# sashashura/h2o-3

Hardware: AMD Instinct MI355X
Metric: gbm_trees_per_sec (higher is better)
Workload: dtype fp32; 1 GPU; model=GBM binomial 100Mx100 ntrees=500 max_depth=8, rows=100000000, cols=100, max_depth=8, histogram_type=QuantilesGlobal, nbins=255, global_batch=100000000, parallelism=dp1

## Files before the change

h2o3_amd/models/tree/devtree.py:

```python
from __future__ import annotations

import ctypes
import os

import numpy as np
import torch

from ...ops import tree_ops
from ...ops.tree_ops import _ptr, _stream
from ...parallel import cloud
from ...parallel import collectives as coll
from ...utils import graphs
from .engine import _TreeBuf

RS = 16
(GAIN, FEAT, T, OPT, L0, L1, R0, R1, T0, T1, OK, NL, NAW, ST, CT, VAL) = range(16)
MAX_DEPTH = 11
_cv, _ci, _cll, _cd, _cf = ctypes.c_void_p, ctypes.c_int, ctypes.c_longlong, ctypes.c_double, ctypes.c_float


def _libs():
    from ...ops import _native
    lh = tree_ops._lib()
    ls = _native.get_lib("tree_split")
    if not getattr(lh, "_typed_dt", False):
        lh.h2o_dt_items.argtypes = [_ci, _cv, _ci, _ci, _ci, _ci, _ci, _cv, _cv, _cv, _cv]
        lh.h2o_dt_offsets.argtypes = [_cv, _cv, _cv, _cv, _ci, _cv, _cv, _cv, _cv]
        lh.h2o_dt_sibling.argtypes = [_cv, _cv, _cv, _ci, _ci, _ci, _ci, _ci, _ci, _cv, _cv, _cv, _cv, _cv]
        lh.h2o_dt_leaf_vals.argtypes = [_cv, _cv, _ci, _ci, _cv, _cd, _cv, _cv]
        lh.h2o_dt_root.argtypes = [_cv, _cll, _cv]
        lh.h2o_part_flags_dev.argtypes = [_cv, _ci, _cll, _cll, _cv, _cv, _cv, _ci, _cv, _cv, _ci, _cv, _cv, _cv, _cv]
        lh.h2o_part_compact_dev.argtypes = [_cv, _cv, _cv, _ci, _cv, _cv, _cv, _cv, _cv, _cv, _cv, _cv]
        lh.h2o_leaf_pos_dev.argtypes = [_cv, _cv, _ci, _ci, _cv, _cv, _cv]
        lh.h2o_leaf_scatter_dev.argtypes = [_cv, _cv, _ci, _cv, _cv, _cv, _cv]
        lh.h2o_hist_bm.argtypes = [_cv, _ci, _cv, _cv, _cv, _cv, _ci, _ci, _ci, _ci, _cf, _cf, _cv, _ci, _ci, _cv,
                                   _ci, _cll, _ci, _cv, _cv, _cv, _cv]
        lh.h2o_gbm_grad.argtypes = [_cv, _cv, _cv, _ci, _cll, _cv, _cv, _cv]
        lh.h2o_iota_i32.argtypes = [_cv, _cll, _cv]
        lh.h2o_dt_colmask.argtypes = [_ci, _cv, _cv, _cv, _cv, _cv, _ci, _ci, _cv, _cv]
        lh.h2o_dt_items2.argtypes = [_ci, _cv, _ci, _ci, _ci, _ci, _ci, _cv, _cv, _cv, _cv, _cv]
        lh.h2o_leaf_flag_sums_dev.argtypes = [_cv, _cv, _cv, _ci, _cv, _cv, _ci, _ci, _cv, _cv, _cv]
        lh.h2o_leaf_gather_lds.argtypes = [_ci, _ci]
        lh.h2o_leaf_gather_items.argtypes = [_cll, _ci]
        lh.h2o_leaf_gather_dev.argtypes = [_cv, _ci, _ci, _ci, _cv, _cv, _cv, _cv, _cll, _ci, _ci, _cv, _cv, _cv, _cv,
                                           _cv, _cv]
        lh._typed_dt = True
    if not getattr(ls, "_typed_dt", False):
        ls.h2o_split_find_b.argtypes = [_cv, _ci, _ci, _ci, _cv, _cv, _cv] + [_cd] * 5 + [_ci, _cv, _cv, _ci, _cv]
        ls.h2o_split_select2.argtypes = [_cv, _cv, _ci, _ci, _ci, _ci, _cd, _ci, _cv, _cv, _cv, _cv]
        ls._typed_dt = True
    return lh, ls


def _ck(rc, what):
    if rc != 0:
        raise RuntimeError(f"{what} failed: error {rc}")


def supported(drv) -> str | None:
    if os.environ.get("H2O3_DEV_TREE", "1") != "1":
        return "disabled (H2O3_DEV_TREE=0)"
    bd, gp, p = drv.bd, drv.gp, drv.est._parms
    if drv.dev.type != "cuda":
        return "no GPU"
    if drv.K != 1 or drv.dist.family not in ("bernoulli", "gaussian") or drv.dist.link not in ("logit", "identity"):
        return "distribution"
    if drv.mono_on or drv.noise_bw != 0 or gp.interaction_sets:
        return "constraints / prediction noise"
    if not drv._base_unit:
        return "row weights other than 0/1"
    if any(bd.is_cat) or bd.code_bytes != 1 or bd.Bs > 256 or bd.Bs % 4 or bd.Fp % 16:
        return "categorical features / wide codes"
    if getattr(bd, "hist_type", "auto") in ("uniformadaptive", "random", "roundrobin"):
        return "adaptive histogram type"
    if gp.max_depth > MAX_DEPTH or gp.max_depth < 1:
        return "max_depth"
    if (gp.mtries or -1) > 0:
        return "mtries"
    if gp.max_leaves:
        return "max_leaves"
    if tree_ops.bm_groups(bd.F, bd.Fp, bd.Bs, True) is None:
        return "histogram layout"
    if drv.offset is not None or getattr(drv.dist, "huber_delta", None) is not None:
        return "offset"
    if not drv.grower.pos_payload_ok():
        return "payload path"
    return None


def gather_rows(n):
    ev = tree_ops.env("H2O3_LEAF_GATHER_R")
    return int(ev) if ev else 8192


class LeafGather:

    def __init__(self, lh, N, D, dev, R=None):
        self.lh, self.N, self.D = lh, int(N), int(D)
        self.nh = (1 << (D + 1)) - 1
        self.R = int(R) if R else gather_rows(N)
        self.scap = 1 << D
        nb = -(-self.N // self.R)
        self.segs = torch.zeros(self.scap * 4, dtype=torch.int32, device=dev)
        self.items = torch.zeros(2 * lh.h2o_leaf_gather_items(self.N, self.scap), dtype=torch.int32, device=dev)
        self.nseg = torch.zeros(2, dtype=torch.int32, device=dev)
        self.T = torch.zeros((nb + 1) * self.scap, dtype=torch.int32, device=dev)

    def run(self, rec, ridx, vals, dbuf, flags=None, slot_wb=None):
        last = 0 if slot_wb is None else 1
        _ck(self.lh.h2o_leaf_gather_dev(_ptr(rec), self.nh, self.D, last, _ptr(slot_wb), _ptr(ridx), _ptr(flags),
                                        _ptr(vals), self.N, self.R, self.scap, _ptr(self.segs), _ptr(self.items),
                                        _ptr(self.nseg), _ptr(self.T), _ptr(dbuf), _stream()), "leaf_gather_dev")


class DevTreeGBM:

    def __init__(self, drv):
        self.drv = drv
        bd, gp = drv.bd, drv.gp
        self.bd, self.gp = bd, gp
        self.lh, self.ls = _libs()
        g = drv.grower
        self.W, self.rank = g.W, g.rank
        self.F, self.Fl, self.Fpad, self.f0 = bd.F, g.Fl, g.Fpad, g.f0
        self.N = N = bd.nrows_local
        self.D = D = int(gp.max_depth)
        self.nh = (1 << (D + 1)) - 1
        self.Bs = Bs = bd.Bs
        self.C = C = 2
        self.bern = drv.dist.family == "bernoulli"
        self.maxabs = float(drv.est._parms.get("max_abs_leafnode_pred", 1.79e308))
        dev = drv.dev
        self.dev = dev
        self.pack = tree_ops.env("H2O3_HIST_PACK", "1") == "1"
        n_fg, G = tree_ops.bm_groups(bd.F, bd.Fp, Bs, self.pack)
        self.n_fg, self.G = n_fg, G
        self.chunk_r = tree_ops.hist_chunk(N, n_fg)
        self.chunk_c = tree_ops.hist_chunk((N + 1) // 2, n_fg)
        if self.pack and max(self.chunk_r, self.chunk_c) >= (1 << 23):
            raise RuntimeError("devtree: histogram chunk too large for the packed path")
        self.chunk_p = tree_ops._part_chunk(N)
        self.chunk_l = 65536
        self.vmax = [1.0, 1.0]
        self._scales()
        n_lvl_max = 1 << (D - 1) if D >= 1 else 1
        self.cap_r = 1 + N // self.chunk_r + 1
        self.cap_c = n_lvl_max + ((N + 1) // 2) // self.chunk_c + 2
        self.cap_p = (1 << D) + N // self.chunk_p + 1
        self.cap_l = self.nh + N // self.chunk_l + 1
        cap_h = max(self.cap_r, self.cap_c)
        i32, f64 = torch.int32, torch.float64
        self.rec = torch.zeros(self.nh * RS, dtype=f64, device=dev)
        self.sums = torch.zeros(self.nh * 2, dtype=f64, device=dev)
        self.vals = torch.zeros(self.nh, dtype=torch.float32, device=dev)
        self.lr_t = torch.zeros(1, dtype=torch.float32, device=dev)
        self.ridx = [g.ridx, g.ridx2]
        self.pos = [torch.empty(N, dtype=torch.float32, device=dev) for _ in range(2)]
        self.dbuf = torch.zeros(N, dtype=torch.float32, device=dev)
        lvl = self.Fl * n_lvl_max * Bs * C
        self.Hbuf = [torch.zeros(lvl, dtype=f64, device=dev) for _ in range(2)]
        self.wyybuf = [torch.zeros(n_lvl_max, dtype=f64, device=dev) for _ in range(2)]
        npar_max = max(1, n_lvl_max // 2)
        self.Hb = torch.zeros(bd.F * npar_max * Bs * C + npar_max, dtype=f64, device=dev)
        self.Hroot = torch.zeros(bd.F * Bs * C + 1, dtype=f64, device=dev)
        self.hwork = torch.zeros(cap_h * 4, dtype=i32, device=dev)
        self.pwork = torch.zeros(self.cap_p * 4, dtype=i32, device=dev)
        self.fbase = torch.zeros(self.cap_p, dtype=i32, device=dev)
        self.lwork = torch.zeros(self.cap_l * 4, dtype=i32, device=dev)
        self.counts = torch.zeros(2, dtype=i32, device=dev)
        self.cnt = torch.zeros(self.cap_p, dtype=i32, device=dev)
        self.loff = torch.zeros(self.cap_p, dtype=i32, device=dev)
        self.roff = torch.zeros(self.cap_p, dtype=i32, device=dev)
        self.flags = torch.zeros(N // 64 + self.cap_p + 1, dtype=torch.int64, device=dev)
        self.part = tree_ops.bm_part(cap_h, n_fg, Bs, G, self.pack, dev)
        self.split_out = torch.zeros(n_lvl_max * max(self.Fl, 1) * 4, dtype=f64, device=dev)
        self.mask = torch.zeros(n_lvl_max * Bs, dtype=torch.uint8, device=dev)
        self.feat_i = torch.zeros(n_lvl_max, dtype=i32, device=dev)
        self.okm = torch.ones((n_lvl_max, max(self.Fl, 1)), dtype=torch.uint8, device=dev)
        if self.f0 + self.Fl > self.F:
            self.okm[:, max(0, self.F - self.f0):] = 0
        self._okm_col = None
        self.mono = torch.zeros(max(self.Fl, 1), dtype=torch.float32, device=dev)
        if bd.codes_col is not None:
            self.pcodes, self.prs, self.pfs = bd.codes_col, 1, bd.nrows_local
        else:
            self.pcodes, self.prs, self.pfs = bd.codes, bd.Fp, 1
        self.cutmat = g._cut_matrix()
        self.sampled = not drv._unit_weights
        self.wbuf = torch.ones(N, dtype=torch.float32, device=dev) if self.sampled else None
        self.colsamp = gp.col_sample_rate < 1.0 or gp.col_sample_rate_change_per_level != 1.0
        if self.colsamp:
            self.cs_elig = torch.zeros(max(self.F, 1), dtype=torch.int64, device=dev)
            self.cs_m = torch.zeros(1, dtype=torch.int32, device=dev)
            self.cs_k = torch.zeros(max(D, 1), dtype=torch.int32, device=dev)
            self.cs_seed = torch.zeros(max(D, 1), dtype=torch.int64, device=dev)
        self.gather = os.environ.get("H2O3_LEAF_GATHER", "1") != "0" and N > 0
        self.last_level = self.gather and os.environ.get("H2O3_DEV_LAST_LEVEL", "1") != "0"
        self.lg = LeafGather(self.lh, N, D, dev) if self.gather else None
        self.slot_wb = torch.zeros(n_lvl_max, dtype=i32, device=dev)
        self.graph = None
        self._hv = [None, None]
        self._k = 0

    def _scales(self):
        vm = self.vmax
        self.s_r = [tree_ops.fixed_point_scale(m, self.chunk_r) for m in vm]
        self.s_c = [tree_ops.fixed_point_scale(m, self.chunk_c) for m in vm]
        self.bq_r = self.bq_c = -1
        if self.pack:
            self.s_r[1], self.bq_r = tree_ops._pack_scale(vm[1], self.chunk_r)
            self.s_c[1], self.bq_c = tree_ops._pack_scale(vm[1], self.chunk_c)

    def set_tree_cols(self, mask):
        key = None if mask is None else mask.tobytes()
        if key == self._okm_col:
            return
        self._okm_col = key
        m = np.ones(self.Fpad, dtype=np.uint8)
        if mask is not None:
            m[:self.F] = np.asarray(mask, dtype=np.uint8)
        m[self.F:] = 0
        row = self._upload([m[self.f0:self.f0 + self.Fl].copy()])[0]
        self.okm.copy_(row.view(1, -1).expand_as(self.okm))

    def _upload(self, arrays):
        offs, n = [], 0
        for a in arrays:
            offs.append(n)
            n += (a.nbytes + 7) & ~7
        n = max(n, 8)
        if getattr(self, "_stg", None) is None or self._stg[0].numel() < n:
            self._stg = [torch.empty(n, dtype=torch.uint8, pin_memory=True) for _ in range(2)]
            self._stg_ev = [None, None]
            self._dstg = torch.empty(n, dtype=torch.uint8, device=self.dev)
            self._stg_i = 0
        i = self._stg_i
        self._stg_i ^= 1
        if self._stg_ev[i] is not None:
            self._stg_ev[i].synchronize()
        buf = self._stg[i].numpy()
        for a, o in zip(arrays, offs):
            buf[o:o + a.nbytes] = np.ascontiguousarray(a).view(np.uint8).reshape(-1)
        self._dstg[:n].copy_(self._stg[i][:n], non_blocking=True)
        ev = torch.cuda.Event()
        ev.record()
        self._stg_ev[i] = ev
        out = []
        for a, o in zip(arrays, offs):
            out.append(self._dstg[o:o + a.nbytes].view(torch.from_numpy(a[:0]).dtype)
                       if a.nbytes else torch.empty(0, dtype=torch.from_numpy(a[:0]).dtype, device=self.dev))
        return out

    def _rec_lvl(self, d):
        off = (1 << d) - 1
        return self.rec[off * RS:]

    def _hist(self, d, cur):
        lh = self.lh
        bd, Bs, C = self.bd, self.Bs, self.C
        n = 1 << d
        H = self.Hbuf[d % 2][:self.Fl * n * Bs * C]
        wyy = self.wyybuf[d % 2][:n]
        s = _stream()
        if d == 0:
            _ck(lh.h2o_dt_items(0, _ptr(self.rec), 1, self.D, 0, self.chunk_r, self.cap_r, _ptr(self.hwork), None,
                                _ptr(self.counts), s), "dt_items(root)")
            nh = bd.F * Bs * C
            buf = self.Hroot
            buf.zero_()
            _ck(lh.h2o_hist_bm(_ptr(bd.codes), bd.Fp, _ptr(self.ridx[cur]), _ptr(self.pos[cur]), None,
                               _ptr(self.hwork), self.cap_r, bd.F, 0, Bs, self.s_r[0], self.s_r[1], _ptr(buf), 1, 0,
                               _ptr(buf[nh:]), 1, self.bq_r, self.G, None, _ptr(self.counts), _ptr(self.part), s),
                "hist_bm(root)")
            Hl, wl = buf[:nh].view(bd.F, 1, Bs, C), buf[nh:]
            if self.W > 1:
                Hl, wl = self.drv.grower._rs_hist_wyy(Hl, wl)
            H.view(self.Fl, 1, Bs, C).copy_(Hl)
            wyy.copy_(wl)
            return H, wyy
        npar = n // 2
        rp = self._rec_lvl(d - 1)
        _ck(lh.h2o_dt_items(1, _ptr(rp), npar, self.D, 0, self.chunk_c, self.cap_c, _ptr(self.hwork), None,
                            _ptr(self.counts), s), "dt_items(child)")
        nhb = bd.F * npar * Bs * C
        buf = self.Hb[:nhb + npar]
        buf.zero_()
        _ck(lh.h2o_hist_bm(_ptr(bd.codes), bd.Fp, _ptr(self.ridx[cur]), _ptr(self.pos[cur]), None, _ptr(self.hwork),
                           self.cap_c, bd.F, 0, Bs, self.s_c[0], self.s_c[1], _ptr(buf), npar, 0, _ptr(buf[nhb:]), 1,
                           self.bq_c, self.G, None, _ptr(self.counts), _ptr(self.part), s), "hist_bm(child)")
        Hb, wb = buf[:nhb].view(bd.F, npar, Bs, C), buf[nhb:]
        if self.W > 1:
            Hb, wb = self.drv.grower._rs_hist_wyy(Hb, wb)
            Hb, wb = Hb.contiguous(), wb.contiguous()
        Hp = self.Hbuf[(d - 1) % 2]
        wp = self.wyybuf[(d - 1) % 2]
        _ck(lh.h2o_dt_sibling(_ptr(Hb), _ptr(Hp), _ptr(rp), npar, self.Fl, Bs * C, C, 0b1, 0, _ptr(H), _ptr(wb),
                              _ptr(wp), _ptr(wyy), _stream()), "dt_sibling")
        return H, wyy

    def _merge(self, recl, n):
        W, Bs = self.W, self.Bs
        rows = recl[:n * RS].view(n, RS)
        rb = 13 * 8
        buf = torch.cat([rows[:, :13].contiguous().view(torch.uint8).view(n, rb), self.mask[:n * Bs].view(n, Bs)], 1)
        g = coll.all_gather_dim0(buf).view(W, n, rb + Bs)
        gains = g[:, :, :8].contiguous().view(torch.float64).view(W, n)
        best = torch.argmax(gains, 0)
        win = g[best, torch.arange(n, device=buf.device)]
        pk = win[:, :rb].contiguous().view(torch.float64).view(n, 13)
        rows[:, :13].copy_(pk)
        self.mask[:n * Bs].view(n, Bs).copy_(win[:, rb:])
        okf = pk[:, OK] > 0
        self.feat_i[:n].copy_(torch.where(okf, pk[:, FEAT], torch.zeros_like(pk[:, FEAT])).to(torch.int32))

    def _level(self, d, cur):
        lh, ls, gp = self.lh, self.ls, self.gp
        n = 1 << d
        Bs = self.Bs
        H, wyy = self._hist(d, cur)
        recl = self._rec_lvl(d)
        s = _stream()
        if self.colsamp:
            rp = self._rec_lvl(d - 1) if d > 0 else None
            _ck(lh.h2o_dt_colmask(d, _ptr(rp), _ptr(self.cs_elig), _ptr(self.cs_m), _ptr(self.cs_k),
                                  _ptr(self.cs_seed), self.f0, self.Fl, _ptr(self.okm), s), "dt_colmask")
        _ck(ls.h2o_split_find_b(_ptr(H), self.Fl, n, Bs, _ptr(wyy), _ptr(self.okm), _ptr(self.mono),
                                float(gp.min_rows), float(gp.min_split_improvement), float(gp.reg_lambda),
                                float(gp.reg_alpha), float(gp.gamma), 0, _ptr(self.split_out), None, 0, s),
            "split_find")
        _ck(ls.h2o_split_select2(_ptr(self.split_out), _ptr(H), self.Fl, n, Bs, self.f0, 2.0 * float(gp.min_rows), RS,
                                 _ptr(recl), _ptr(self.mask), _ptr(self.feat_i), s), "split_select2")
        if self.W > 1:
            self._merge(recl, n)
        s = _stream()
        skip = self.last_level and d == self.D - 1
        _ck(lh.h2o_dt_items2(0, _ptr(recl), n, self.D, 0, self.chunk_p, self.cap_p, _ptr(self.pwork),
                             _ptr(self.fbase), _ptr(self.slot_wb) if skip else None, _ptr(self.counts), s),
            "dt_items(part)")
        _ck(lh.h2o_part_flags_dev(_ptr(self.pcodes), 1, self.prs, self.pfs, _ptr(self.ridx[cur]), _ptr(self.pwork),
                                  _ptr(self.fbase), self.cap_p, _ptr(self.feat_i), _ptr(self.mask), Bs,
                                  _ptr(self.flags), _ptr(self.cnt), _ptr(self.counts), s), "part_flags_dev")
        _ck(lh.h2o_dt_offsets(_ptr(self.cnt), _ptr(self.pwork), _ptr(self.counts), _ptr(recl), n,
                              _ptr(self._rec_lvl(d + 1)), _ptr(self.loff), _ptr(self.roff), s), "dt_offsets")
        if skip:
            _ck(lh.h2o_leaf_flag_sums_dev(_ptr(self.pos[cur]), _ptr(self.pwork), _ptr(self.fbase), self.cap_p,
                                          _ptr(self.flags), _ptr(recl), self.D, 1 if self.bern else 0,
                                          _ptr(self.sums), _ptr(self.counts), s), "leaf_flag_sums_dev")
            return cur
        nxt = cur ^ 1
        _ck(lh.h2o_part_compact_dev(_ptr(self.ridx[cur]), _ptr(self.pwork), _ptr(self.fbase), self.cap_p,
                                    _ptr(self.flags), _ptr(self.loff), _ptr(self.roff), _ptr(self.ridx[nxt]),
                                    _ptr(self.pos[cur]), _ptr(self.pos[nxt]), _ptr(self.counts), s),
            "part_compact_dev")
        return nxt

    def _sequence(self):
        lh, drv = self.lh, self.drv
        s = _stream()
        y = drv.yb if self.bern else torch.nan_to_num(drv.yf)
        if not hasattr(self, "_y"):
            self._y = y.contiguous().to(torch.float32)
        f = drv._f[:, 0]
        _ck(lh.h2o_gbm_grad(_ptr(self._y), _ptr(f), _ptr(self.wbuf) if self.sampled else None,
                            1 if self.bern else 0, self.N, _ptr(self.pos[0]), _ptr(self.dbuf), s), "gbm_grad")
        _ck(lh.h2o_iota_i32(_ptr(self.ridx[0]), self.N, s), "iota")
        self.rec.zero_()
        self.sums.zero_()
        _ck(lh.h2o_dt_root(_ptr(self.rec), self.N, _stream()), "dt_root")
        cur = 0
        for d in range(self.D):
            cur = self._level(d, cur)
        s = _stream()
        _ck(lh.h2o_dt_items(3 if self.last_level else 2, _ptr(self.rec), self.nh, self.D, 0, self.chunk_l, self.cap_l,
                            _ptr(self.lwork), None, _ptr(self.counts), s), "dt_items(leaf)")
        _ck(lh.h2o_leaf_pos_dev(_ptr(self.pos[cur]), _ptr(self.lwork), self.cap_l, 1 if self.bern else 0,
                                _ptr(self.sums), _ptr(self.counts), s), "leaf_pos_dev")
        if self.W > 1:
            coll.allreduce_(self.sums)
        s = _stream()
        _ck(lh.h2o_dt_leaf_vals(_ptr(self.rec), _ptr(self.sums), self.nh, self.D, _ptr(self.lr_t), self.maxabs,
                                _ptr(self.vals), s), "dt_leaf_vals")
        if self.gather:
            self.lg.run(self.rec, self.ridx[cur], self.vals, self.dbuf, self.flags if self.last_level else None,
                        self.slot_wb if self.last_level else None)
        else:
            _ck(lh.h2o_leaf_scatter_dev(_ptr(self.ridx[cur]), _ptr(self.lwork), self.cap_l, _ptr(self.vals),
                                        _ptr(self.dbuf), _ptr(self.counts), s), "leaf_scatter_dev")
        self.cur = cur

    def set_col_sampling(self, tree_mask):
        if not self.colsamp:
            return
        g, gp, F, D = self.drv.grower, self.gp, self.F, self.D
        base = np.ones(F, dtype=bool) if tree_mask is None else np.asarray(tree_mask, dtype=bool)
        elig = np.nonzero(base)[0]
        m = int(elig.size)
        ks = np.zeros(D, dtype=np.int32)
        seeds = np.zeros(D, dtype=np.int64)
        for d in range(D):
            rate = gp.col_sample_rate * (gp.col_sample_rate_change_per_level ** d)
            k = max(1, int(np.floor(rate * m + 0.5))) if rate < 1.0 else m
            if k >= m:
                ks[d] = m
            else:
                ks[d] = k
                seeds[d] = int(g.rng.randint(0, 2 ** 31 - 1))
        e = np.zeros(max(F, 1), dtype=np.int64)
        e[:m] = elig
        de, dm, dk, dsd = self._upload([e, np.array([m], dtype=np.int32), ks, seeds])
        self.cs_elig.copy_(de)
        self.cs_m.copy_(dm)
        self.cs_k.copy_(dk)
        self.cs_seed.copy_(dsd)

    def run(self, lr, pending, w=None):
        if not pending:
            self.dbuf.zero_()
        if self.sampled:
            self.wbuf.copy_(w)
        self.lr_t.fill_(float(lr))
        if not self.bern:
            f = self.drv._f[:, 0]
            z = (torch.nan_to_num(self.drv.yf) - (f + self.dbuf))
            self.vmax = [1.0, float(z.abs().max())]
            self._scales()
            self._sequence()
        elif self.W == 1 and os.environ.get("H2O3_DEV_TREE_GRAPH", "1") == "1":
            if self.graph is None:
                self._sequence()
                torch.cuda.synchronize()
                g = torch.cuda.CUDAGraph()
                with graphs.capture(g):
                    self._sequence()
                self.graph = g
            else:
                self.graph.replay()
        else:
            self._sequence()
        return self._copy_out()

    def _copy_out(self):
        k = self._k
        self._k ^= 1
        h = self._hv[k]
        if h is None:
            h = self._hv[k] = torch.empty(self.nh * RS, dtype=torch.float64, pin_memory=True)
        h.copy_(self.rec, non_blocking=True)
        ev = torch.cuda.Event()
        ev.record()
        return h, ev

    def decode(self, rec_h, criterion="se"):
        D, nh = self.D, self.nh
        R = np.asarray(rec_h, dtype=np.float64).reshape(nh, RS)
        lv = np.floor(np.log2(np.arange(nh) + 1)).astype(np.int64)
        ok = R[:, OK] > 0
        exists = np.zeros(nh, dtype=bool)
        exists[0] = True
        for d in range(1, D + 1):
            a, b = (1 << d) - 1, (1 << (d + 1)) - 1
            par = (np.arange(a, b) - 1) >> 1
            exists[a:b] = exists[par] & ok[par]
        split = exists & ok & (lv < D)
        ids = np.nonzero(exists)[0]
        bfs = np.full(nh, -1, dtype=np.int64)
        bfs[ids] = np.arange(ids.size)
        n = ids.size
        tb = _TreeBuf(cap=max(n, 1))
        tb.n = n
        par = np.maximum((ids - 1) >> 1, 0)
        is_left = (ids % 2) == 1
        w_own = R[ids, T0]
        w_par = np.where(is_left, R[par, L0], R[par, R0])
        tb.weight[:n] = np.where(lv[ids] < D, w_own, w_par)
        tb.depth[:n] = lv[ids]
        sp = split[ids]
        hs = ids[sp]
        bi = bfs[hs]
        f = R[hs, FEAT].astype(np.int64)
        t = R[hs, T].astype(np.int64)
        opt = R[hs, OPT].astype(np.int64)
        tb.feat[bi] = f
        tb.left[bi] = bfs[2 * hs + 1]
        tb.right[bi] = bfs[2 * hs + 2]
        tb.gain[bi] = R[hs, GAIN]
        tb.split_code[bi] = t
        cm = self.cutmat
        tb.thr[bi] = np.where(opt == 2, np.inf, cm[f, np.minimum(t, cm.shape[1] - 1)])
        na = opt == 1
        if criterion != "xgb":
            free = (R[hs, NAW] == 0) & (opt != 2)
            na = np.where(free, R[hs, L0] > R[hs, R0], na)
        tb.na_left[bi] = na
        lf = ~sp
        tb.value[bfs[ids[lf]]] = R[ids[lf], VAL]
        return tb.to_tree()
```

h2o3_amd/ops/csrc/tree_hist.hip:

```cpp
#include "common.h"
#include <stdlib.h>
#include <algorithm>

template <int MODE> struct Chan { static constexpr int C = MODE == 2 ? 1 : 2; };

template <typename CodeT, int MODE, bool HAS_VB, bool POSV, bool PACK = false>
__global__ __launch_bounds__(512) void hist_build_kernel(
    const CodeT* __restrict__ codes, int Fp, const int* __restrict__ ridx,
    const float* __restrict__ va, const float* __restrict__ vb,
    const int4* __restrict__ work, int F, int Bs, int FGL, float s0, float s1,
    double* __restrict__ hist, int n_slots, double* __restrict__ wyy_out, const uint8_t* __restrict__ need,
    long long bq = 0) {
  constexpr int C = Chan<MODE>::C;
  constexpr int CL = PACK ? 1 : C;
  const int RPW = 64 / FGL;
  extern __shared__ __attribute__((aligned(16))) unsigned long long ldsq[];
  const int4 wk = work[blockIdx.x];
  if (need != nullptr && need[(size_t)wk.x * gridDim.y + blockIdx.y] == 0) return;
  const int fg0 = blockIdx.y * FGL;
  const int nf = min(FGL, F - fg0);
  const int stride_f = Bs * CL;
  const int total = FGL * stride_f;
  for (int i = threadIdx.x; i < total; i += blockDim.x) ldsq[i] = 0ull;
  __syncthreads();
  const unsigned long long pk_off = (1ull << 40) + (unsigned long long)bq;

  const int lane = threadIdx.x & 63;
  const int fl = lane % FGL;
  const int rs = lane / FGL;
  const bool lane_ok = rs < RPW;
  const bool fok = fl < nf && lane_ok;
  const int nwaves = blockDim.x >> 6;
  const int wv = threadIdx.x >> 6;
  unsigned long long* hbase = ldsq + fl * stride_f;
  const bool do_wyy = (MODE == 0) && wyy_out != nullptr && blockIdx.y == 0 && fl == 0 && lane_ok;
  double wyy = 0.0;
  const int pend = wk.y + wk.z;
  const int step = nwaves * RPW;
  constexpr int U = 8;
  const int fcl = min(fl, max(nf - 1, 0));
  const CodeT* cbase = codes + fg0 + fcl;
  for (int p0 = wk.y + wv * RPW + (lane_ok ? rs : 0); p0 < pend; p0 += U * step) {
    int rr[U];
    float c0[U], c1[U], yv[U];
    int code[U];
#pragma unroll
    for (int u = 0; u < U; ++u) rr[u] = ridx[min(p0 + u * step, pend - 1)];
#pragma unroll
    for (int u = 0; u < U; ++u) {
      const int r = rr[u];
      const int vi = POSV ? min(p0 + u * step, pend - 1) : r;
      if (MODE == 0) {
        const float y = va[vi];
        const float w = HAS_VB ? vb[vi] : 1.f;
        c0[u] = w; c1[u] = w * y;
        yv[u] = y;
      } else if (MODE == 1) {
        c0[u] = va[vi]; c1[u] = vb[vi];
      } else {
        c0[u] = HAS_VB ? vb[vi] : 1.f; c1[u] = 0.f;
      }
      code[u] = (int)cbase[(size_t)r * Fp];
    }
#pragma unroll
    for (int u = 0; u < U; ++u) {
      const bool inr = p0 + u * step < pend;
      if (MODE == 0 && do_wyy && inr) wyy += (double)c1[u] * (double)yv[u];
      if (PACK) {
        if (fok && inr && c0[u] != 0.f)
          __hip_atomic_fetch_add(hbase + code[u], pk_off + (unsigned long long)__float2ll_rn(c1[u] * s1),
                                 __ATOMIC_RELAXED, __HIP_MEMORY_SCOPE_WORKGROUP);
        continue;
      }
      const bool ok = fok && inr && (c0[u] != 0.f || c1[u] != 0.f);
      if (ok) {
        unsigned long long* h = hbase + code[u] * C;
        __hip_atomic_fetch_add(h, (unsigned long long)__float2ll_rn(c0[u] * s0), __ATOMIC_RELAXED,
                               __HIP_MEMORY_SCOPE_WORKGROUP);
        if (C > 1)
          __hip_atomic_fetch_add(h + 1, (unsigned long long)__float2ll_rn(c1[u] * s1), __ATOMIC_RELAXED,
                                 __HIP_MEMORY_SCOPE_WORKGROUP);
      }
    }
  }
  __syncthreads();
  if (MODE == 0 && wyy_out != nullptr && blockIdx.y == 0) {
    wyy = wave_sum(wyy);
    if (lane == 0) gbl_add(wyy_out + wk.x, wyy);
  }
  const double inv0 = 1.0 / (double)s0, inv1 = 1.0 / (double)s1;
  if (PACK) {
    const int tot = nf * Bs;
    for (int i = threadIdx.x; i < tot; i += blockDim.x) {
      const unsigned long long v = ldsq[i];
      if (v != 0) {
        const int j = i / Bs, b = i - (i / Bs) * Bs;
        const long long cnt = (long long)(v >> 40);
        const long long low = (long long)(v & ((1ull << 40) - 1));
        double* o = hist + ((size_t)(fg0 + j) * n_slots + wk.x) * (Bs * 2) + 2 * b;
        gbl_add(o, (double)cnt);
        gbl_add(o + 1, (double)(low - cnt * bq) * inv1);
      }
    }
    return;
  }
  const int tot_real = nf * stride_f;
  for (int i = threadIdx.x; i < tot_real; i += blockDim.x) {
    const long long q = (long long)ldsq[i];
    if (q != 0) {
      const int j = i / stride_f;
      const int rem = i - j * stride_f;
      const double v = (double)q * ((C == 1 || (rem & 1) == 0) ? inv0 : inv1);
      gbl_add(hist + ((size_t)(fg0 + j) * n_slots + wk.x) * stride_f + rem, v);
    }
  }
}

template <int LW> struct CodeW { using T = unsigned int; };
template <> struct CodeW<2> { using T = uint2; };
__device__ __forceinline__ unsigned int code_at(unsigned int w, int hi, int sh) { return (w >> sh) & 0xffu; }
__device__ __forceinline__ unsigned int code_at(uint2 w, int hi, int sh) { return ((hi ? w.y : w.x) >> sh) & 0xffu; }

template <int MODE, bool HAS_VB, bool POSV, bool PACK, bool PIPE = true, int LW = 1>
__global__ __launch_bounds__(1024) void hist_quad_kernel(
    const uint8_t* __restrict__ codes, int Fp, const int* __restrict__ ridx,
    const float* __restrict__ va, const float* __restrict__ vb,
    const int4* __restrict__ work, int n_work, int n_fg, int fgw, int F, int foff, int Bs, float s0, float s1,
    double* __restrict__ hist, int n_slots, double* __restrict__ wyy_out, long long bq,
    const uint8_t* __restrict__ need, const int* __restrict__ n_work_dev) {
  using CT = typename CodeW<LW>::T;
  constexpr int C = Chan<MODE>::C;
  constexpr int CL = PACK ? 1 : C;
  constexpr int NK = 4 * LW;
  constexpr int U = 4;
  extern __shared__ __attribute__((aligned(16))) unsigned long long ldsq[];
  const int nwg = n_work_dev != nullptr ? n_work_dev[1] * n_fg : n_work * n_fg;
  if ((int)blockIdx.x >= nwg) return;
  const int lb = xcd_remap(blockIdx.x, nwg);
  const int fgi = lb % n_fg;
  const int4 wk = work[lb / n_fg];
  if (need != nullptr && need[(size_t)wk.x * n_fg + fgi] == 0) return;
  const int fg0 = foff + fgi * fgw;
  const int nf = min(fgw, F - fg0);
  const int LPR = fgw / NK;
  const int RPW = 64 / LPR;
  const int stride_f = Bs * CL + CL;
  const int total = fgw * stride_f;
  for (int i = threadIdx.x; i < total; i += blockDim.x) ldsq[i] = 0ull;
  __syncthreads();
  const int lane = threadIdx.x & 63;
  const int q = lane % LPR;
  const int rs = lane / LPR;
  const bool lane_ok = rs < RPW;
  const int wv = threadIdx.x >> 6;
  const int nwaves = blockDim.x >> 6;
  const bool do_wyy = (MODE == 0) && wyy_out != nullptr && fgi == 0 && q == 0 && lane_ok;
  double wyy = 0.0;
  const int pend = wk.y + wk.z;
  const int step = nwaves * RPW;
  const uint8_t* cbase = codes + fg0 + NK * q;
  unsigned long long* hb[NK];
  bool fk[NK];
#pragma unroll
  for (int k = 0; k < NK; ++k) {
    hb[k] = ldsq + (NK * q + k) * stride_f;
    fk[k] = lane_ok && NK * q + k < nf;
  }
  const int p_first = wk.y + wv * RPW + (lane_ok ? rs : 0);
  int rA[U], rB[U];
  CT cwA[U];
  float xaA[U], xbA[U];
  auto load_r = [&](int p, int (&r)[U]) {
#pragma unroll
    for (int u = 0; u < U; ++u) r[u] = ridx[min(p + u * step, pend - 1)];
  };
  auto load_v = [&](int p, const int (&r)[U], CT (&cw)[U], float (&xa)[U], float (&xb)[U]) {
#pragma unroll
    for (int u = 0; u < U; ++u) {
      const int vi = POSV ? min(p + u * step, pend - 1) : r[u];
      xa[u] = (MODE == 2) ? 0.f : va[vi];
      xb[u] = (HAS_VB || MODE == 1) ? vb[vi] : 1.f;
      cw[u] = *reinterpret_cast<const CT*>(cbase + (size_t)r[u] * Fp);
    }
  };
  if (PIPE) {
    load_r(p_first, rA);
    load_v(p_first, rA, cwA, xaA, xbA);
    load_r(p_first + U * step, rB);
  }
  for (int p0 = p_first; p0 < pend; p0 += U * step) {
    CT cw[U];
    float c0[U], c1[U], yv[U], xa[U], xb[U];
    if (PIPE) {
#pragma unroll
      for (int u = 0; u < U; ++u) { cw[u] = cwA[u]; xa[u] = xaA[u]; xb[u] = xbA[u]; }
      load_v(p0 + U * step, rB, cwA, xaA, xbA);
      load_r(p0 + 2 * U * step, rB);
    } else {
      int rr[U];
      load_r(p0, rr);
      load_v(p0, rr, cw, xa, xb);
    }
#pragma unroll
    for (int u = 0; u < U; ++u) {
      if (MODE == 0) {
        const float y = xa[u];
        const float w = HAS_VB ? xb[u] : (y == y ? 1.f : 0.f);
        c0[u] = w; c1[u] = w != 0.f ? w * y : 0.f; yv[u] = w != 0.f ? y : 0.f;
      } else if (MODE == 1) {
        c0[u] = xa[u]; c1[u] = xb[u]; yv[u] = 0.f;
      } else {
        c0[u] = xb[u]; c1[u] = 0.f; yv[u] = 0.f;
      }
    }
#pragma unroll
    for (int u = 0; u < U; ++u) {
      const bool inr = p0 + u * step < pend;
      if (MODE == 0 && do_wyy && inr) wyy += (double)c1[u] * (double)yv[u];
      if (!inr || (c0[u] == 0.f && c1[u] == 0.f)) continue;
      if (PACK) {
        const unsigned long long a = (1ull << 40) + (unsigned long long)(__float2ll_rn(yv[u] * s1) + bq);
#pragma unroll
        for (int k = 0; k < NK; ++k) {
          if (!fk[k]) continue;
          __hip_atomic_fetch_add(hb[k] + code_at(cw[u], k >> 2, 8 * (k & 3)), a, __ATOMIC_RELAXED,
                                 __HIP_MEMORY_SCOPE_WORKGROUP);
        }
        continue;
      }
      const unsigned long long a0 = (unsigned long long)__float2ll_rn(c0[u] * s0);
      const unsigned long long a1 = (unsigned long long)__float2ll_rn(c1[u] * s1);
#pragma unroll
      for (int k = 0; k < NK; ++k) {
        if (!fk[k]) continue;
        unsigned long long* h = hb[k] + code_at(cw[u], k >> 2, 8 * (k & 3)) * CL;
        __hip_atomic_fetch_add(h, a0, __ATOMIC_RELAXED, __HIP_MEMORY_SCOPE_WORKGROUP);
        if (C > 1) __hip_atomic_fetch_add(h + 1, a1, __ATOMIC_RELAXED, __HIP_MEMORY_SCOPE_WORKGROUP);
      }
    }
  }
  __syncthreads();
  if (MODE == 0 && wyy_out != nullptr && fgi == 0) {
    wyy = wave_sum(wyy);
    if (lane == 0) gbl_add(wyy_out + wk.x, wyy);
  }
  const double inv0 = 1.0 / (double)s0, inv1 = 1.0 / (double)s1;
  const int per_f = Bs * C;
  if (PACK) {
    const int tot = nf * Bs;
    for (int i = threadIdx.x; i < tot; i += blockDim.x) {
      const int j = i / Bs;
      const int b = i - j * Bs;
      const unsigned long long v = ldsq[j * stride_f + b];
      if (v != 0) {
        const long long cnt = (long long)(v >> 40);
        const long long low = (long long)(v & ((1ull << 40) - 1));
        double* o = hist + ((size_t)(fg0 + j) * n_slots + wk.x) * per_f + 2 * b;
        gbl_add(o, (double)cnt);
        gbl_add(o + 1, (double)(low - cnt * bq) * inv1);
      }
    }
    return;
  }
  const int tot_real = nf * per_f;
  for (int i = threadIdx.x; i < tot_real; i += blockDim.x) {
    const int j = i / per_f;
    const int rem = i - j * per_f;
    const long long v = (long long)ldsq[j * stride_f + rem];
    if (v != 0) {
      const double d = (double)v * ((C == 1 || (rem & 1) == 0) ? inv0 : inv1);
      gbl_add(hist + ((size_t)(fg0 + j) * n_slots + wk.x) * per_f + rem, d);
    }
  }
}

struct QuadArgs {
  dim3 grid; int threads; size_t lds; hipStream_t s;
  const uint8_t* cc; int Fp; const int* ridx; const float* va; const float* vb; const int4* wk;
  int n_work, n_fg, fgw, F, foff, Bs; float s0, s1; double* hist; int n_slots; double* wyy; long long bq;
  const uint8_t* need; const int* n_work_dev; unsigned long long* part = nullptr;
};

template <int M, bool V, bool PV, bool PK, bool PIPE = true, int LW = 1>
static void lq(const QuadArgs& a) {
  hipLaunchKernelGGL((hist_quad_kernel<M, V, PV, PK, PIPE, LW>), a.grid, dim3(a.threads), a.lds, a.s, a.cc, a.Fp,
                     a.ridx, a.va, a.vb, a.wk, a.n_work, a.n_fg, a.fgw, a.F, a.foff, a.Bs, a.s0, a.s1, a.hist,
                     a.n_slots, a.wyy, a.bq, a.need, a.n_work_dev);
}

static int env_int(const char* k, int d) {
  const char* v = getenv(k);
  return v ? atoi(v) : d;
}

template <int M, bool V, bool PV, bool PK>
static void lq_var(int lw, const QuadArgs& a) {
  static const int pipe = env_int("H2O3_HIST_PIPE", 1);
  if (!pipe) lq<M, V, PV, PK, false>(a);
  else if (lw == 2) lq<M, V, PV, PK, true, 2>(a);
  else lq<M, V, PV, PK>(a);
}

template <int M, bool V>
static void lq_pv(int posv, int pack, int lw, const QuadArgs& a) {
  if (pack) { if (posv) lq_var<M, V, true, true>(lw, a); else lq_var<M, V, false, true>(lw, a); }
  else { if (posv) lq_var<M, V, true, false>(lw, a); else lq_var<M, V, false, false>(lw, a); }
}

extern "C" int h2o_hist_quad4(const void* codes, int Fp, const int* ridx, const float* va, const float* vb,
                              const int* work, int n_work, int F, int foff, int Bs, float s0, float s1,
                              double* hist, int n_slots, int mode, int threads, double* wyy, int posv,
                              long long pack_bq, int fgw, const uint8_t* need, const int* n_work_dev,
                              hipStream_t s);
extern "C" int h2o_hist_quad3(const void* codes, int Fp, const int* ridx, const float* va, const float* vb,
                              const int* work, int n_work, int F, int foff, int Bs, float s0, float s1,
                              double* hist, int n_slots, int mode, int threads, double* wyy, int posv,
                              long long pack_bq, int fgw, const uint8_t* need, hipStream_t s) {
  return h2o_hist_quad4(codes, Fp, ridx, va, vb, work, n_work, F, foff, Bs, s0, s1, hist, n_slots, mode, threads,
                        wyy, posv, pack_bq, fgw, need, nullptr, s);
}

extern "C" int h2o_hist_quad4(const void* codes, int Fp, const int* ridx, const float* va, const float* vb,
                              const int* work, int n_work, int F, int foff, int Bs, float s0, float s1,
                              double* hist, int n_slots, int mode, int threads, double* wyy, int posv,
                              long long pack_bq, int fgw, const uint8_t* need, const int* n_work_dev,
                              hipStream_t s) {
  if (n_work <= 0 || foff >= F) return 0;
  if (Fp % 4 != 0 || foff % 4 != 0 || Bs > 256 || mode < 0 || mode > 2) return -1;
  if (fgw < 4 || fgw > 64 || fgw % 4 != 0) return -2;
  const bool pack = pack_bq >= 0 && mode == 0;
  const int n_fg = (F - foff + fgw - 1) / fgw;
  if (foff + n_fg * fgw > Fp) return -3;
  static const int lw_env = env_int("H2O3_HIST_LW", 1);
  const int lw = (lw_env == 2 && fgw % 8 == 0 && foff % 8 == 0 && Fp % 8 == 0) ? 2 : 1;
  const int C = mode == 2 ? 1 : 2;
  const int CL = pack ? 1 : C;
  QuadArgs a;
  a.grid = dim3(n_work * n_fg); a.threads = threads;
  a.lds = (size_t)fgw * (Bs * CL + CL) * sizeof(unsigned long long); a.s = s;
  if (a.lds > 160 * 1024) return -4;
  a.cc = (const uint8_t*)codes; a.Fp = Fp; a.ridx = ridx; a.va = va; a.vb = vb; a.wk = (const int4*)work;
  a.n_work = n_work; a.n_fg = n_fg; a.fgw = fgw; a.F = F; a.foff = foff; a.Bs = Bs; a.s0 = s0; a.s1 = s1;
  a.hist = hist; a.n_slots = n_slots; a.wyy = wyy; a.bq = pack_bq; a.need = need; a.n_work_dev = n_work_dev;
  switch (mode) {
    case 0: if (vb) lq_pv<0, true>(posv, pack, lw, a); else lq_pv<0, false>(posv, pack, lw, a); break;
    case 1: lq_pv<1, true>(posv, 0, lw, a); break;
    default: if (vb) lq_pv<2, true>(posv, 0, lw, a); else lq_pv<2, false>(posv, 0, lw, a); break;
  }
  return (int)hipGetLastError();
}

__device__ __forceinline__ unsigned long long fx_signed(float v, float s) {
  const double d = __fma_rn((double)v, (double)s, 6755399441055744.0);
  return (unsigned long long)(__double_as_longlong(d) - 0x4338000000000000LL);
}

template <int G, int CL, int MODE, bool HAS_VB, bool POSV, bool PACK, int LW = 2>
__global__ __launch_bounds__(1024) void hist_bm_kernel(
    const uint8_t* __restrict__ codes, int Fp, const int* __restrict__ ridx,
    const float* __restrict__ va, const float* __restrict__ vb,
    const int4* __restrict__ work, int n_work, int n_fg, int F, int foff, int Bs, float s0, float s1,
    double* __restrict__ hist, int n_slots, double* __restrict__ wyy_out, long long bq,
    const uint8_t* __restrict__ need, const int* __restrict__ n_work_dev, unsigned long long* __restrict__ part,
    int dbg) {
  constexpr int C = Chan<MODE>::C;
  constexpr int NK = 4 * LW;
  constexpr int LPR = G / NK;
  constexpr int RPW = 64 / LPR;
  constexpr int PITCH = G * CL;
  constexpr int U = 4;
  constexpr int PD = 2;
  using CT = typename CodeW<LW>::T;
  static_assert(CL == 1 || C == 2, "two LDS channels need a two-channel mode");
  static_assert(LPR >= 1, "group narrower than one lane's codes");
  extern __shared__ __attribute__((aligned(16))) unsigned long long ldsq[];
  const int nwg = n_work_dev != nullptr ? n_work_dev[1] * n_fg : n_work * n_fg;
  if ((int)blockIdx.x >= nwg) return;
  const int lb = xcd_remap(blockIdx.x, nwg);
  const int fgi = lb % n_fg;
  int4 wk = work[lb / n_fg];
  wk.x = __builtin_amdgcn_readfirstlane(wk.x);
  wk.y = __builtin_amdgcn_readfirstlane(wk.y);
  wk.z = __builtin_amdgcn_readfirstlane(wk.z);
  if (need != nullptr && need[(size_t)wk.x * n_fg + fgi] == 0) return;
  const int fg0 = foff + fgi * G;
  const int nf = min(G, F - fg0);
  {
    const int n2 = Bs * PITCH / 2;
    ulonglong2* z = reinterpret_cast<ulonglong2*>(ldsq);
    for (int i = threadIdx.x; i < n2; i += blockDim.x) z[i] = make_ulonglong2(0ull, 0ull);
  }
  __syncthreads();
  const int lane = threadIdx.x & 63;
  const int q = lane % LPR;
  const int rs = lane / LPR;
  const int wv = threadIdx.x >> 6;
  const int nwaves = __builtin_amdgcn_readfirstlane((int)(blockDim.x >> 6));
  unsigned sh[NK], sb[NK];
#pragma unroll
  for (int k = 0; k < NK; ++k) {
    const int kk = (k & ~3) | ((k + rs) & 3);
    sh[k] = 8u * kk;
    sb[k] = (unsigned)((kk * LPR + q) * 8);
  }
  const bool blk_wyy = MODE == 0 && wyy_out != nullptr && fgi == 0;
  double wyyd = 0.0;
  const int pend = wk.y + wk.z;
  const int step = nwaves * RPW;
  const uint8_t* cbase = codes + fg0 + NK * q;
  const int p_first = wk.y + wv * RPW + rs;
  const unsigned long long pk_off = (1ull << 40) + (unsigned long long)bq;
  const __amdgpu_buffer_rsrc_t rr = __builtin_amdgcn_make_buffer_rsrc((void*)ridx, (short)0, pend * 4, 0x00020000);
  const __amdgpu_buffer_rsrc_t ra = __builtin_amdgcn_make_buffer_rsrc((void*)va, (short)0, POSV ? pend * 4 : 0,
                                                                      0x00020000);
  const __amdgpu_buffer_rsrc_t rb = __builtin_amdgcn_make_buffer_rsrc((void*)vb, (short)0,
                                                                      (POSV && vb) ? pend * 4 : 0, 0x00020000);
  int R[PD][U];
  CT CW[PD][U];
  float XA[PD][U], XB[PD][U];
  auto load_r = [&](int p, int (&r)[U]) {
#pragma unroll
    for (int u = 0; u < U; ++u) r[u] = __builtin_amdgcn_raw_buffer_load_b32(rr, p * 4, u * step * 4, 0);
  };
  auto load_v = [&](int p, const int (&r)[U], CT (&cw)[U], float (&xa)[U], float (&xb)[U]) {
#pragma unroll
    for (int u = 0; u < U; ++u) {
      if (POSV) {
        xa[u] = (MODE == 2) ? 0.f : __int_as_float(__builtin_amdgcn_raw_buffer_load_b32(ra, p * 4, u * step * 4, 0));
        xb[u] = (HAS_VB || MODE == 1) ? __int_as_float(__builtin_amdgcn_raw_buffer_load_b32(rb, p * 4, u * step * 4, 0))
                                      : 1.f;
      } else {
        xa[u] = (MODE == 2) ? 0.f : va[r[u]];
        xb[u] = (HAS_VB || MODE == 1) ? vb[r[u]] : 1.f;
      }
      cw[u] = *reinterpret_cast<const CT*>(cbase + (size_t)(unsigned)r[u] * (unsigned)Fp);
    }
  };
  const int IT = U * step;
#pragma unroll
  for (int d = 0; d < PD; ++d) load_r(p_first + d * IT, R[d]);
#pragma unroll
  for (int d = 0; d < PD; ++d) {
    load_v(p_first + d * IT, R[d], CW[d], XA[d], XB[d]);
    load_r(p_first + (PD + d) * IT, R[d]);
  }
  for (int p0r = p_first; p0r < pend; p0r += PD * IT) {
#pragma unroll
    for (int d = 0; d < PD; ++d) {
      const int p0 = p0r + d * IT;
#pragma unroll
      for (int u = 0; u < U; ++u) {
        const bool inr = p0 + u * step < pend;
        float c0, c1, yv = 0.f;
        if (MODE == 0) {
          const float y = XA[d][u];
          const float w = HAS_VB ? XB[d][u] : (y == y ? 1.f : 0.f);
          c0 = w;
          c1 = w != 0.f ? w * y : 0.f;
          yv = w != 0.f ? y : 0.f;
          if (blk_wyy && inr) wyyd += (double)c1 * (double)yv;
        } else if (MODE == 1) {
          c0 = XA[d][u]; c1 = XB[d][u];
        } else {
          c0 = XB[d][u]; c1 = 0.f;
        }
        if (!inr || (c0 == 0.f && c1 == 0.f) || (dbg & 2)) continue;
        unsigned long long a0, a1 = 0ull;
        if (PACK) {
          a0 = fx_signed(yv, s1) + pk_off;
        } else {
          a0 = fx_signed(c0, s0);
          if (CL == 2) a1 = fx_signed(c1, s1);
        }
#pragma unroll
        for (int k = 0; k < NK; ++k) {
          unsigned word;
          if constexpr (LW == 2) word = (k & 4) ? CW[d][u].y : CW[d][u].x;
          else word = CW[d][u];
          const unsigned code = __builtin_amdgcn_ubfe(word, sh[k] & 31u, 8);
          unsigned long long* h = reinterpret_cast<unsigned long long*>(
              reinterpret_cast<char*>(ldsq) + code * (unsigned)(PITCH * 8) + sb[k]);
          __hip_atomic_fetch_add(h, a0, __ATOMIC_RELAXED, __HIP_MEMORY_SCOPE_WORKGROUP);
          if (CL == 2) __hip_atomic_fetch_add(h + G, a1, __ATOMIC_RELAXED, __HIP_MEMORY_SCOPE_WORKGROUP);
        }
      }
      load_v(p0 + PD * IT, R[d], CW[d], XA[d], XB[d]);
      load_r(p0 + 2 * PD * IT, R[d]);
    }
  }
  __syncthreads();
  if (blk_wyy) {
    double v = q == 0 ? wyyd : 0.0;
    v = wave_sum(v);
    if (lane == 0) gbl_add(wyy_out + wk.x, v);
  }
  if (part != nullptr) {
    if (dbg & 1) return;
    const int n2 = Bs * PITCH / 2;
    const ulonglong2* src = reinterpret_cast<const ulonglong2*>(ldsq);
    ulonglong2* dst = reinterpret_cast<ulonglong2*>(part + ((size_t)(lb / n_fg) * n_fg + fgi) * (size_t)(Bs * PITCH));
    for (int i2 = threadIdx.x; i2 < n2; i2 += blockDim.x) dst[i2] = src[i2];
    return;
  }
  const double inv0 = 1.0 / (double)s0, inv1 = 1.0 / (double)s1;
  const int si = lane & 15, bi = lane >> 4;
  constexpr int NSG = G / 16;
  const int nbq = (dbg & 1) ? 0 : (Bs + 3) >> 2;
  for (int e = wv; e < nbq * NSG; e += nwaves) {
    const int b = (e / NSG) * 4 + bi;
    const int slot = (e % NSG) * 16 + si;
    const int fl = NK * (slot % LPR) + slot / LPR;
    if (b >= Bs || fl >= nf) continue;
    double* o = hist + ((size_t)(fg0 + fl) * n_slots + wk.x) * (size_t)(Bs * C) + (size_t)b * C;
    const unsigned long long v = ldsq[b * PITCH + slot];
    if (PACK) {
      if (v != 0ull) {
        const long long cnt = (long long)(v >> 40);
        const long long low = (long long)(v & ((1ull << 40) - 1));
        if (dbg & 4) {
          unsigned long long* ou = reinterpret_cast<unsigned long long*>(o);
          __hip_atomic_fetch_add(ou, (unsigned long long)cnt, __ATOMIC_RELAXED, __HIP_MEMORY_SCOPE_AGENT);
          __hip_atomic_fetch_add(ou + 1, (unsigned long long)(low - cnt * bq), __ATOMIC_RELAXED,
                                 __HIP_MEMORY_SCOPE_AGENT);
        } else {
          gbl_add(o, (double)cnt);
          gbl_add(o + 1, (double)(low - cnt * bq) * inv1);
        }
      }
    } else {
      if (v != 0ull) gbl_add(o, (double)(long long)v * inv0);
      if (CL == 2) {
        const unsigned long long v1 = ldsq[b * PITCH + G + slot];
        if (v1 != 0ull) gbl_add(o + 1, (double)(long long)v1 * inv1);
      }
    }
  }
}

static int g_bm_dbg = 0;
extern "C" void h2o_hist_bm_set_debug(int flags) { g_bm_dbg = flags; }

template <int G, int CL, int M, bool V, bool PV, bool PK, int LW>
static int lbm_u(const QuadArgs& a) {
  auto kern = hist_bm_kernel<G, CL, M, V, PV, PK, LW>;
  static bool attr = false;
  if (!attr) {
    hipError_t e = hipFuncSetAttribute((const void*)kern, hipFuncAttributeMaxDynamicSharedMemorySize, 160 * 1024);
    if (e != hipSuccess) return (int)e;
    attr = true;
  }
  hipLaunchKernelGGL(kern, a.grid, dim3(a.threads), a.lds, a.s, a.cc, a.Fp, a.ridx, a.va, a.vb, a.wk, a.n_work,
                     a.n_fg, a.F, a.foff, a.Bs, a.s0, a.s1, a.hist, a.n_slots, a.wyy, a.bq, a.need, a.n_work_dev,
                     a.part, g_bm_dbg);
  return (int)hipGetLastError();
}

template <int G, int CL, int M, bool V, bool PV, bool PK>
static int lbm(const QuadArgs& a) {
  static const int lw = env_int("H2O3_HIST_BM_LW", 2);
  return (lw == 1 || G == 16) ? lbm_u<G, CL, M, V, PV, PK, 1>(a) : lbm_u<G, CL, M, V, PV, PK, 2>(a);
}

template <int G, int CL, int M, bool PK>
static int lbm_v(bool vb, bool posv, const QuadArgs& a) {
  if (M == 1) return posv ? lbm<G, CL, M, true, true, PK>(a) : lbm<G, CL, M, true, false, PK>(a);
  if (vb) return posv ? lbm<G, CL, M, true, true, PK>(a) : lbm<G, CL, M, true, false, PK>(a);
  return posv ? lbm<G, CL, M, false, true, PK>(a) : lbm<G, CL, M, false, false, PK>(a);
}

template <int G>
static int lbm_g(int mode, bool pack, bool vb, bool posv, const QuadArgs& a) {
  if (pack) return lbm_v<G, 1, 0, true>(vb, posv, a);
  if (mode == 2) return lbm_v<G, 1, 2, false>(vb, posv, a);
  if constexpr (G <= 32) {
    if (mode == 0) return lbm_v<G, 2, 0, false>(vb, posv, a);
    return lbm_v<G, 2, 1, false>(vb, posv, a);
  }
  return (int)hipErrorInvalidValue;
}

#define BM_RED 32
__global__ __launch_bounds__(256) void hist_bm_reduce_kernel(
    const unsigned long long* __restrict__ part, const int4* __restrict__ work, int n_work,
    const int* __restrict__ n_work_dev, int n_fg, int F, int foff, int G, int CL, int lpr, int nk, int Bs, int C,
    int pack, long long bq, float s0, float s1, const uint8_t* __restrict__ need, double* __restrict__ hist,
    int n_slots) {
  const int nw = n_work_dev != nullptr ? n_work_dev[1] : n_work;
  const int i0 = blockIdx.z * BM_RED;
  if (i0 >= nw) return;
  const int i1 = min(nw, i0 + BM_RED);
  const int g = blockIdx.y;
  const int PITCH = G * CL;
  const int nbt = (Bs + 15) / 16;
  const int b = (blockIdx.x % nbt) * 16 + (threadIdx.x >> 4);
  if (b >= Bs) return;
  const int sl = (blockIdx.x / nbt) * 16 + (threadIdx.x & 15);
  const int ch = sl / G, slot = sl - ch * G;
  const int fg0 = foff + g * G;
  const int fl = nk * (slot % lpr) + slot / lpr;
  const bool live = fl < min(G, F - fg0);
  const double inv0 = 1.0 / (double)s0, inv1 = 1.0 / (double)s1;
  const size_t E = (size_t)Bs * PITCH;
  const size_t eoff = (size_t)b * PITCH + sl;
  long long a0 = 0, a1 = 0;
  int cur = -1;
  auto flush = [&]() {
    if (cur < 0 || !live || (a0 == 0 && a1 == 0)) return;
    double* o = hist + ((size_t)(fg0 + fl) * n_slots + cur) * (size_t)(Bs * C) + (size_t)b * C;
    if (pack) {
      gbl_add(o, (double)a0);
      gbl_add(o + 1, (double)a1 * inv1);
    } else {
      gbl_add(o + ch, (double)a0 * (ch == 0 ? inv0 : inv1));
    }
  };
  for (int i = i0; i < i1; ++i) {
    const int s = work[i].x;
    if (need != nullptr && need[(size_t)s * n_fg + g] == 0) continue;
    if (s != cur) {
      flush();
      cur = s; a0 = 0; a1 = 0;
    }
    const unsigned long long v = part[((size_t)i * n_fg + g) * E + eoff];
    if (pack) {
      const long long cnt = (long long)(v >> 40);
      a0 += cnt;
      a1 += (long long)(v & ((1ull << 40) - 1)) - cnt * bq;
    } else {
      a0 += (long long)v;
    }
  }
  flush();
}

extern "C" int h2o_hist_bm(const void* codes, int Fp, const int* ridx, const float* va, const float* vb,
                           const int* work, int n_work, int F, int foff, int Bs, float s0, float s1,
                           double* hist, int n_slots, int mode, double* wyy, int posv, long long pack_bq, int G,
                           const uint8_t* need, const int* n_work_dev, unsigned long long* part, hipStream_t s) {
  if (n_work <= 0 || foff >= F) return 0;
  if (Fp % 4 != 0 || foff % 4 != 0 || Bs > 256 || Bs % 4 != 0 || mode < 0 || mode > 2) return -1;
  const bool pack = pack_bq >= 0 && mode == 0;
  const int CL = (pack || mode == 2) ? 1 : 2;
  if (!(G == 16 || G == 32 || G == 64) || (CL == 2 && G == 64)) return -2;
  const int n_fg = (F - foff + G - 1) / G;
  if (foff + n_fg * G > Fp) return -3;
  QuadArgs a;
  a.grid = dim3(n_work * n_fg); a.threads = 1024;
  a.lds = (size_t)Bs * G * CL * sizeof(unsigned long long); a.s = s;
  if (a.lds > 160 * 1024) return -4;
  a.cc = (const uint8_t*)codes; a.Fp = Fp; a.ridx = ridx; a.va = va; a.vb = vb; a.wk = (const int4*)work;
  a.n_work = n_work; a.n_fg = n_fg; a.fgw = G; a.F = F; a.foff = foff; a.Bs = Bs; a.s0 = s0; a.s1 = s1;
  a.hist = hist; a.n_slots = n_slots; a.wyy = wyy; a.bq = pack_bq; a.need = need; a.n_work_dev = n_work_dev;
  a.part = part;
  const int rc = G == 64 ? lbm_g<64>(mode, pack, vb != nullptr, posv != 0, a)
               : G == 32 ? lbm_g<32>(mode, pack, vb != nullptr, posv != 0, a)
                         : lbm_g<16>(mode, pack, vb != nullptr, posv != 0, a);
  if (rc != 0 || part == nullptr || (g_bm_dbg & 1)) return rc;
  static const int lw_env = env_int("H2O3_HIST_BM_LW", 2);
  const int lw = (lw_env == 1 || G == 16) ? 1 : 2;
  const int nk = 4 * lw, lpr = G / nk;
  const int C = mode == 2 ? 1 : 2;
  dim3 rg(((Bs + 15) / 16) * (G * CL / 16), n_fg, (n_work + BM_RED - 1) / BM_RED);
  hipLaunchKernelGGL(hist_bm_reduce_kernel, rg, dim3(256), 0, s, part, (const int4*)work, n_work, n_work_dev, n_fg,
                     F, foff, G, CL, lpr, nk, Bs, C, pack ? 1 : 0, pack_bq, s0, s1, need, hist, n_slots);
  return (int)hipGetLastError();
}

template <typename CodeT>
static int launch_hist(const void* codes, int Fp, const int* ridx, const float* va, const float* vb,
                       const int4* work, int n_work, int F, int FG, int Bs, float s0, float s1, double* hist,
                       int n_slots, int mode, int threads, double* wyy, int posv, const uint8_t* need,
                       hipStream_t s, long long pack_bq = -1) {
  const int n_fg = (F + FG - 1) / FG;
  dim3 grid(n_work, n_fg);
  const int C = mode == 2 ? 1 : 2;
  const CodeT* cc = (const CodeT*)codes;
  if (pack_bq >= 0 && mode == 0) {
    const size_t lds = (size_t)FG * Bs * sizeof(unsigned long long);
    if (lds > 160 * 1024) return (int)hipErrorInvalidValue;
#define H2O_PK(V, PV)                                                                                        \
  {                                                                                                          \
    auto kern = hist_build_kernel<CodeT, 0, V, PV, true>;                                                    \
    if (hipFuncSetAttribute((const void*)kern, hipFuncAttributeMaxDynamicSharedMemorySize, (int)lds) !=      \
        hipSuccess)                                                                                          \
      return (int)hipErrorInvalidValue;                                                                      \
    hipLaunchKernelGGL(kern, grid, dim3(threads), lds, s, cc, Fp, ridx, va, vb, work, F, Bs, FG, s0, s1,     \
                       hist, n_slots, wyy, need, pack_bq);                                                   \
  }
    if (vb) {
      if (posv) H2O_PK(true, true) else H2O_PK(true, false)
    } else {
      if (posv) H2O_PK(false, true) else H2O_PK(false, false)
    }
#undef H2O_PK
    return (int)hipGetLastError();
  }
  size_t lds = (size_t)FG * Bs * C * sizeof(unsigned long long);
  switch (mode) {
#define H2O_LH(M, V) if (posv) H2O_LH2(M, V, true); else H2O_LH2(M, V, false)
#define H2O_LH2(M, V, PV) hipLaunchKernelGGL((hist_build_kernel<CodeT, M, V, PV>), grid, dim3(threads), lds, s, cc, Fp, ridx, va, vb, work, F, Bs, FG, s0, s1, hist, n_slots, wyy, need)
    case 0: if (vb) H2O_LH(0, true); else H2O_LH(0, false); break;
    case 1: H2O_LH(1, true); break;
    default: if (vb) H2O_LH(2, true); else H2O_LH(2, false); break;
#undef H2O_LH
#undef H2O_LH2
  }
  return (int)hipGetLastError();
}

template <typename CodeT>
__device__ __forceinline__ void load_items(const CodeT* __restrict__ codes, long long rs, long long fs, int f,
                                           const int* __restrict__ ridx, int p0, int end, int (&r)[16],
                                           int (&c)[16]) {
  if (p0 + 16 <= end && (p0 & 3) == 0) {
    const int4* v = reinterpret_cast<const int4*>(ridx + p0);
#pragma unroll
    for (int q = 0; q < 4; ++q) {
      const int4 x = v[q];
      r[4 * q] = x.x; r[4 * q + 1] = x.y; r[4 * q + 2] = x.z; r[4 * q + 3] = x.w;
    }
  } else {
#pragma unroll
    for (int k = 0; k < 16; ++k) r[k] = ridx[min(p0 + k, end - 1)];
  }
#pragma unroll
  for (int k = 0; k < 16; ++k) c[k] = (int)codes[(size_t)r[k] * rs + (size_t)f * fs];
}

template <typename CodeT>
__global__ __launch_bounds__(256) void part_count_kernel(
    const CodeT* __restrict__ codes, long long rs, long long fs, const int* __restrict__ ridx,
    const int4* __restrict__ work, const int* __restrict__ feat, const uint8_t* __restrict__ masks,
    int Bs, int* __restrict__ cnt) {
  __shared__ uint8_t m[4096];
  __shared__ int red[4];
  const int4 wk = work[blockIdx.x];
  const int f = feat[wk.x];
  for (int i = threadIdx.x; i < Bs; i += blockDim.x) m[i] = masks[(size_t)wk.x * Bs + i];
  __syncthreads();
  const int end = wk.y + wk.z;
  int local = 0;
  for (int base = wk.y; base < end; base += 256 * 16) {
    const int p0 = base + threadIdx.x * 16;
    if (p0 >= end) continue;
    int r[16], c[16];
    load_items<CodeT>(codes, rs, fs, f, ridx, p0, end, r, c);
#pragma unroll
    for (int k = 0; k < 16; ++k) local += (p0 + k < end && m[c[k]]) ? 1 : 0;
  }
  for (int o = 32; o > 0; o >>= 1) local += __shfl_xor(local, o, 64);
  if (lane_id() == 0) red[wave_id()] = local;
  __syncthreads();
  if (threadIdx.x == 0) cnt[blockIdx.x] = red[0] + red[1] + red[2] + red[3];
}

template <typename CodeT>
__global__ __launch_bounds__(256) void part_scatter_kernel(
    const CodeT* __restrict__ codes, long long rs, long long fs, const int* __restrict__ ridx,
    const int4* __restrict__ work, const int* __restrict__ feat, const uint8_t* __restrict__ masks,
    int Bs, const int* __restrict__ loff, const int* __restrict__ roff, int* __restrict__ out,
    const float* __restrict__ pa, const float* __restrict__ pb, float* __restrict__ pa_out,
    float* __restrict__ pb_out) {
  __shared__ uint8_t m[4096];
  __shared__ int wsum[4];
  const int4 wk = work[blockIdx.x];
  const int f = feat[wk.x];
  for (int i = threadIdx.x; i < Bs; i += blockDim.x) m[i] = masks[(size_t)wk.x * Bs + i];
  __syncthreads();
  int lbase = loff[blockIdx.x], rbase = roff[blockIdx.x];
  const int end = wk.y + wk.z;
  const int lane = lane_id(), wv = wave_id();
  for (int base = wk.y; base < end; base += 256 * 16) {
    const int p0 = base + threadIdx.x * 16;
    int r[16], c[16];
    unsigned bits = 0;
    int nl = 0, nv = 0;
    if (p0 < end) {
      load_items<CodeT>(codes, rs, fs, f, ridx, p0, end, r, c);
#pragma unroll
      for (int k = 0; k < 16; ++k) {
        const bool v = p0 + k < end;
        const bool L = v && m[c[k]];
        bits |= (L ? 1u : 0u) << k;
        nl += L ? 1 : 0;
        nv += v ? 1 : 0;
      }
    }
    int incl = nl;
#pragma unroll
    for (int d = 1; d < 64; d <<= 1) {
      const int u = __shfl_up(incl, d, 64);
      if (lane >= d) incl += u;
    }
    if (lane == 63) wsum[wv] = incl;
    __syncthreads();
    int wpre = 0, tot = 0;
#pragma unroll
    for (int w = 0; w < 4; ++w) {
      const int s = wsum[w];
      wpre += (w < wv) ? s : 0;
      tot += s;
    }
    const int lpre = wpre + incl - nl;
    const int tile_first = base;
    const int pos_before = max(0, min(p0, end) - tile_first);
    int li = lbase + lpre;
    int ri = rbase + (pos_before - lpre);
    if (p0 < end) {
#pragma unroll
      for (int k = 0; k < 16; ++k) {
        if (p0 + k < end) {
          const int dst = ((bits >> k) & 1u) ? li++ : ri++;
          out[dst] = r[k];
          if (pa) { pa_out[dst] = pa[p0 + k]; pb_out[dst] = pb[p0 + k]; }
        }
      }
    }
    const int tile_n = min(256 * 16, end - base);
    lbase += tot;
    rbase += tile_n - tot;
    __syncthreads();
  }
}
template <typename CodeT>
__global__ __launch_bounds__(256) void part_flags_kernel(
    const CodeT* __restrict__ codes, long long rs, long long fs, const int* __restrict__ ridx,
    const int4* __restrict__ work, const int* __restrict__ fbase, const int* __restrict__ feat,
    const uint8_t* __restrict__ masks, int Bs, unsigned long long* __restrict__ flags, int* __restrict__ cnt,
    const int* __restrict__ nw_dev) {
  __shared__ uint8_t m[4096];
  __shared__ int red[4];
  if (nw_dev != nullptr && (int)blockIdx.x >= nw_dev[1]) return;
  const int4 wk = work[blockIdx.x];
  const int f = feat[wk.x];
  for (int i = threadIdx.x; i < Bs; i += blockDim.x) m[i] = masks[(size_t)wk.x * Bs + i];
  __syncthreads();
  const int lane = threadIdx.x & 63, wv = threadIdx.x >> 6;
  const int end = wk.y + wk.z;
  const int fb = fbase[blockIdx.x];
  int local = 0;
  constexpr int U = 8;
  for (int base = wk.y; base < end; base += 256 * U) {
    int r[U], c[U];
#pragma unroll
    for (int u = 0; u < U; ++u) r[u] = ridx[min(base + u * 256 + (int)threadIdx.x, end - 1)];
#pragma unroll
    for (int u = 0; u < U; ++u) c[u] = (int)codes[(size_t)r[u] * rs + (size_t)f * fs];
#pragma unroll
    for (int u = 0; u < U; ++u) {
      const int p = base + u * 256 + (int)threadIdx.x;
      const bool L = p < end && m[c[u]];
      const unsigned long long bal = __ballot(L);
      const int w0 = base + u * 256 + wv * 64;
      if (lane == 0 && w0 < end) flags[fb + (w0 - wk.y) / 64] = bal;
      local += L ? 1 : 0;
    }
  }
  local = (int)wave_sum((float)local);
  if (lane == 0) red[wv] = local;
  __syncthreads();
  if (threadIdx.x == 0) cnt[blockIdx.x] = red[0] + red[1] + red[2] + red[3];
}

template <int U>
__global__ __launch_bounds__(256) void part_compact_kernel(
    const int* __restrict__ ridx, const int4* __restrict__ work, const int* __restrict__ fbase,
    const unsigned long long* __restrict__ flags, const int* __restrict__ loff, const int* __restrict__ roff,
    int* __restrict__ out, const float* __restrict__ pa, float* __restrict__ pa_out, const int* __restrict__ nw_dev) {
  __shared__ int wl[U][4], wr_[U][4];
  if (nw_dev != nullptr && (int)blockIdx.x >= nw_dev[1]) return;
  const int4 wk = work[blockIdx.x];
  const int lane = threadIdx.x & 63, wv = threadIdx.x >> 6;
  const int end = wk.y + wk.z;
  const int fb = fbase[blockIdx.x];
  int lbase = loff[blockIdx.x], rbase = roff[blockIdx.x];
  const unsigned long long below = (lane == 0) ? 0ull : (~0ull >> (64 - lane));
  for (int base = wk.y; base < end; base += 256 * U) {
    int r[U];
    float a[U];
    unsigned long long bal[U], valid[U];
#pragma unroll
    for (int u = 0; u < U; ++u) {
      const int p = base + u * 256 + (int)threadIdx.x;
      const int pc = min(p, end - 1);
      r[u] = ridx[pc];
      a[u] = pa ? pa[pc] : 0.f;
      const int w0 = base + u * 256 + wv * 64;
      bal[u] = (w0 < end) ? flags[fb + (w0 - wk.y) / 64] : 0ull;
    }
#pragma unroll
    for (int u = 0; u < U; ++u) {
      valid[u] = __ballot(base + u * 256 + (int)threadIdx.x < end);
      const int nl_w = __popcll(bal[u] & valid[u]);
      if (lane == 0) { wl[u][wv] = nl_w; wr_[u][wv] = __popcll(valid[u]) - nl_w; }
    }
    __syncthreads();
    int lrun = 0, rrun = 0;
#pragma unroll
    for (int u = 0; u < U; ++u) {
      int lpre = lrun, rpre = rrun;
#pragma unroll
      for (int w = 0; w < 4; ++w) {
        lpre += (w < wv) ? wl[u][w] : 0;
        rpre += (w < wv) ? wr_[u][w] : 0;
        lrun += wl[u][w];
        rrun += wr_[u][w];
      }
      if ((valid[u] >> lane) & 1ull) {
        const bool L = (bal[u] >> lane) & 1ull;
        const int dst = L ? (lbase + lpre + __popcll(bal[u] & valid[u] & below))
                          : (rbase + rpre + __popcll(~bal[u] & valid[u] & below));
        out[dst] = r[u];
        if (pa) pa_out[dst] = a[u];
      }
    }
    lbase += lrun;
    rbase += rrun;
    __syncthreads();
  }
}


__global__ __launch_bounds__(256) void hist_sibling_kernel(const double* __restrict__ Hb,
                                                           const double* __restrict__ Hp,
                                                           const int* __restrict__ slots, int nb, int np, int nf,
                                                           int BsC, int C, int clamp_mask,
                                                           double* __restrict__ H, const double* __restrict__ wyy_b,
                                                           const double* __restrict__ wyy_p,
                                                           double* __restrict__ wyy_out,
                                                           const int* __restrict__ nb_dev) {
  const int j = blockIdx.x;
  if (nb_dev != nullptr && j >= nb_dev[0]) return;
  const int f = blockIdx.y;
  const int bs = slots[j], ds = slots[nb + j], ps = slots[2 * nb + j];
  const double* hb = Hb + ((size_t)f * nb + j) * BsC;
  const double* hp = Hp + ((size_t)f * np + ps) * BsC;
  double* ob = H + ((size_t)f * nf + bs) * BsC;
  double* od = H + ((size_t)f * nf + ds) * BsC;
  for (int i = threadIdx.x; i < BsC; i += blockDim.x) {
    const double b = hb[i];
    double d = hp[i] - b;
    if ((clamp_mask >> (i % C)) & 1) d = fmax(d, 0.0);
    ob[i] = b;
    od[i] = d;
  }
  if (wyy_b != nullptr && f == 0 && threadIdx.x == 0) {
    wyy_out[bs] = wyy_b[j];
    wyy_out[ds] = wyy_p[ps] - wyy_b[j];
  }
}

__global__ __launch_bounds__(1024) void part_offsets_kernel(const int* __restrict__ cnt,
                                                            const long long* __restrict__ meta, int nw, int n,
                                                            int* __restrict__ loff, int* __restrict__ roff,
                                                            long long* __restrict__ nleft, double* __restrict__ pk,
                                                            int stride, int col) {
  __shared__ long long carry;
  const long long* slot = meta;
  const long long* first = meta + nw;
  const long long* st = meta + 2 * (long long)nw;
  const long long* pos = meta + 3 * (long long)nw;
  for (int s = threadIdx.x; s < n; s += blockDim.x) nleft[s] = 0;
  if (threadIdx.x == 0) carry = 0;
  __syncthreads();
  __shared__ long long wtot[16];
  const int lane = threadIdx.x & 63, wv = threadIdx.x >> 6, nwv = blockDim.x >> 6;
  for (int base = 0; base < nw; base += blockDim.x) {
    const int i = base + threadIdx.x;
    const long long v = i < nw ? (long long)cnt[i] : 0;
    long long x = v;
#pragma unroll
    for (int o = 1; o < 64; o <<= 1) {
      const long long t = __shfl_up(x, o, 64);
      if (lane >= o) x += t;
    }
    if (lane == 63) wtot[wv] = x;
    __syncthreads();
    if (wv == 0) {
      long long w = lane < nwv ? wtot[lane] : 0;
#pragma unroll
      for (int o = 1; o < 16; o <<= 1) {
        const long long t = __shfl_up(w, o, 64);
        if (lane >= o) w += t;
      }
      if (lane < nwv) wtot[lane] = w;
    }
    __syncthreads();
    const long long before = (wv > 0 ? wtot[wv - 1] : 0) + carry;
    if (i < nw) loff[i] = (int)(before + x - v);
    __syncthreads();
    if (threadIdx.x == 0) carry += wtot[nwv - 1];
    __syncthreads();
  }
  __syncthreads();
  for (int i = threadIdx.x; i < nw; i += blockDim.x)
    if (i == nw - 1 || first[i + 1] != first[i])
      nleft[slot[i]] = (long long)loff[i] + cnt[i] - (long long)loff[first[i]];
  for (int i = threadIdx.x; i < nw; i += blockDim.x) roff[i] = loff[first[i]];
  __syncthreads();
  for (int i = threadIdx.x; i < nw; i += blockDim.x) {
    const long long lpre = (long long)loff[i] - (long long)roff[i];
    const long long s = slot[i];
    loff[i] = (int)(st[i] + lpre);
    roff[i] = (int)(st[i] + nleft[s] + pos[i] - lpre);
  }
  __syncthreads();
  if (pk != nullptr)
    for (int s = threadIdx.x; s < n; s += blockDim.x) pk[(size_t)s * stride + col] = (double)nleft[s];
}


__global__ __launch_bounds__(256) void leaf_pos_kernel(const float* __restrict__ zp, const int4* __restrict__ work,
                                                       int mode, double* __restrict__ out,
                                                       const int* __restrict__ nw_dev) {
  if (nw_dev != nullptr && (int)blockIdx.x >= nw_dev[1]) return;
  const int4 wk = work[blockIdx.x];
  double sa = 0.0, sb = 0.0;
  const int end = wk.y + wk.z;
  for (int p = wk.y + threadIdx.x; p < end; p += 256) {
    const float z = zp[p];
    if (z == z) {
      sa += (double)z;
      if (mode == 1) {
        const double az = fabs((double)z);
        sb += az * (1.0 - az);
      } else {
        sb += 1.0;
      }
    }
  }
  sa = wave_sum(sa);
  sb = wave_sum(sb);
  __shared__ double red[2][4];
  if (lane_id() == 0) { red[0][wave_id()] = sa; red[1][wave_id()] = sb; }
  __syncthreads();
  if (threadIdx.x == 0) {
    gbl_add(out + 2 * wk.x, red[0][0] + red[0][1] + red[0][2] + red[0][3]);
    gbl_add(out + 2 * wk.x + 1, red[1][0] + red[1][1] + red[1][2] + red[1][3]);
  }
}

__global__ __launch_bounds__(256) void leaf_update_kernel(const int* __restrict__ ridx, const int4* __restrict__ work,
                                                          const float* __restrict__ val, float* __restrict__ f) {
  const int4 wk = work[blockIdx.x];
  const float v = val[wk.x];
  for (int p = wk.y + threadIdx.x; p < wk.y + wk.z; p += 256) f[ridx[p]] += v;
}

__global__ __launch_bounds__(256) void leaf_scatter_kernel(const int* __restrict__ ridx, const int4* __restrict__ work,
                                                           const float* __restrict__ val, float* __restrict__ d,
                                                           const int* __restrict__ nw_dev) {
  if (nw_dev != nullptr && (int)blockIdx.x >= nw_dev[1]) return;
  const int4 wk = work[blockIdx.x];
  const float v = val[wk.x];
  const int end = wk.y + wk.z;
  int p = wk.y + threadIdx.x;
  for (; p + 3 * 256 < end; p += 4 * 256) {
    const int r0 = ridx[p], r1 = ridx[p + 256], r2 = ridx[p + 512], r3 = ridx[p + 768];
    d[r0] = v; d[r1] = v; d[r2] = v; d[r3] = v;
  }
  for (; p < end; p += 256) d[ridx[p]] = v;
}

__device__ __forceinline__ unsigned long long smix64(unsigned long long x) {
  x += 0x9E3779B97F4A7C15ull;
  x = (x ^ (x >> 30)) * 0xBF58476D1CE4E5B9ull;
  x = (x ^ (x >> 27)) * 0x94D049BB133111EBull;
  return x ^ (x >> 31);
}

__global__ __launch_bounds__(256) void col_sample_kernel(int n, int m, const long long* __restrict__ elig, int k,
                                                         unsigned long long seed, long long* __restrict__ out) {
  const int node = blockIdx.x * blockDim.x + threadIdx.x;
  if (node >= n) return;
  const unsigned long long base = smix64(seed ^ ((unsigned long long)node * 0xD1B54A32D192ED03ull));
  long long* o = out + (size_t)node * k;
  int taken = 0;
  for (int j = 0; j < m && taken < k; ++j) {
    const double u = (double)(smix64(base + (unsigned long long)j) >> 11) * (1.0 / 9007199254740992.0);
    if (u * (double)(m - j) < (double)(k - taken)) o[taken++] = elig[j];
  }
}

__global__ __launch_bounds__(256) void fill_nid_kernel(const int* __restrict__ ridx, const int4* __restrict__ work,
                                                       int* __restrict__ nid) {
  const int4 wk = work[blockIdx.x];
  for (int p = wk.y + threadIdx.x; p < wk.y + wk.z; p += blockDim.x) nid[ridx[p]] = wk.x;
}

__global__ __launch_bounds__(256) void iota_i32_kernel(int* __restrict__ out, long long n) {
  const long long n4 = n >> 2;
  const long long stride = (long long)gridDim.x * blockDim.x;
  for (long long i = (long long)blockIdx.x * blockDim.x + threadIdx.x; i < n4; i += stride) {
    const int b = (int)(4 * i);
    reinterpret_cast<int4*>(out)[i] = make_int4(b, b + 1, b + 2, b + 3);
  }
  for (long long i = 4 * n4 + (long long)blockIdx.x * blockDim.x + threadIdx.x; i < n; i += stride) out[i] = (int)i;
}

extern "C" {

int h2o_iota_i32(int* out, long long n, hipStream_t s) {
  if (n <= 0) return 0;
  if (((uintptr_t)out & 15) != 0) return -1;
  const long long blocks = std::min<long long>((n / 4 + 255) / 256 + 1, 4096);
  hipLaunchKernelGGL(iota_i32_kernel, dim3((unsigned)blocks), dim3(256), 0, s, out, n);
  return (int)hipGetLastError();
}

int h2o_hist_build(const void* codes, int code_bytes, int Fp, const int* ridx, const float* va,
                   const float* vb, const int* work, int n_work, int F, int FG, int Bs, float s0, float s1,
                   double* hist, int n_slots, int mode, int threads, double* wyy, int posv, const uint8_t* need,
                   hipStream_t s) {
  if (n_work <= 0) return 0;
  if (code_bytes == 1)
    return launch_hist<uint8_t>(codes, Fp, ridx, va, vb, (const int4*)work, n_work, F, FG, Bs, s0, s1, hist, n_slots, mode, threads, wyy, posv, need, s);
  return launch_hist<uint16_t>(codes, Fp, ridx, va, vb, (const int4*)work, n_work, F, FG, Bs, s0, s1, hist, n_slots, mode, threads, wyy, posv, need, s);
}

int h2o_hist_build_pk(const void* codes, int code_bytes, int Fp, const int* ridx, const float* va,
                      const float* vb, const int* work, int n_work, int F, int FG, int Bs, float s1, long long bq,
                      double* hist, int n_slots, int threads, double* wyy, int posv, const uint8_t* need,
                      hipStream_t s) {
  if (n_work <= 0) return 0;
  if (bq < 0) return (int)hipErrorInvalidValue;
  if (code_bytes == 1)
    return launch_hist<uint8_t>(codes, Fp, ridx, va, vb, (const int4*)work, n_work, F, FG, Bs, 1.f, s1, hist, n_slots,
                                0, threads, wyy, posv, need, s, bq);
  return launch_hist<uint16_t>(codes, Fp, ridx, va, vb, (const int4*)work, n_work, F, FG, Bs, 1.f, s1, hist, n_slots,
                               0, threads, wyy, posv, need, s, bq);
}

int h2o_part_flags(const void* codes, int code_bytes, long long rs, long long fs, const int* ridx,
                   const int* work, const int* fbase, int n_work, const int* feat, const uint8_t* masks, int Bs,
                   unsigned long long* flags, int* cnt, hipStream_t s) {
  if (n_work <= 0) return 0;
  if (code_bytes == 1)
    hipLaunchKernelGGL(part_flags_kernel<uint8_t>, dim3(n_work), dim3(256), 0, s, (const uint8_t*)codes, rs, fs,
                       ridx, (const int4*)work, fbase, feat, masks, Bs, flags, cnt, nullptr);
  else
    hipLaunchKernelGGL(part_flags_kernel<uint16_t>, dim3(n_work), dim3(256), 0, s, (const uint16_t*)codes, rs, fs,
                       ridx, (const int4*)work, fbase, feat, masks, Bs, flags, cnt, nullptr);
  return (int)hipGetLastError();
}

int h2o_hist_sibling(const double* Hb, const double* Hp, const int* slots, int nb, int np, int nf, int F, int BsC,
                     int C, int clamp_mask, double* H, const double* wyy_b, const double* wyy_p, double* wyy_out,
                     hipStream_t s) {
  if (nb <= 0 || F <= 0) return 0;
  hipLaunchKernelGGL(hist_sibling_kernel, dim3(nb, F), dim3(256), 0, s, Hb, Hp, slots, nb, np, nf, BsC, C, clamp_mask,
                     H, wyy_b, wyy_p, wyy_out, nullptr);
  return (int)hipGetLastError();
}

int h2o_hist_sibling_dev(const double* Hb, const double* Hp, const int* slots, int nb, int np, int nf, int F,
                         int BsC, int C, int clamp_mask, double* H, const double* wyy_b, const double* wyy_p,
                         double* wyy_out, const int* counts, hipStream_t s) {
  if (nb <= 0 || F <= 0) return 0;
  hipLaunchKernelGGL(hist_sibling_kernel, dim3(nb, F), dim3(256), 0, s, Hb, Hp, slots, nb, np, nf, BsC, C, clamp_mask,
                     H, wyy_b, wyy_p, wyy_out, counts);
  return (int)hipGetLastError();
}

__global__ __launch_bounds__(1024) void child_work_kernel(const long long* __restrict__ st,
                                                          const long long* __restrict__ ct,
                                                          const double* __restrict__ rec, int stride, int ok_col,
                                                          int nl_col, int wl_col, int wr_col, int n, int chunk,
                                                          int cap, int4* __restrict__ work, int* __restrict__ slots,
                                                          int* __restrict__ counts) {
  __shared__ long long wtot[2][16];
  __shared__ long long carry[2];
  const int lane = threadIdx.x & 63, wv = threadIdx.x >> 6, nwv = blockDim.x >> 6;
  if (threadIdx.x == 0) carry[0] = carry[1] = 0;
  __syncthreads();
  for (int base = 0; base < n; base += blockDim.x) {
    const int i = base + threadIdx.x;
    long long sp = 0, nch = 0, start = 0, cnt = 0;
    bool bl = true;
    if (i < n && rec[(size_t)i * stride + ok_col] > 0) {
      const long long nl = (long long)rec[(size_t)i * stride + nl_col];
      bl = rec[(size_t)i * stride + wl_col] <= rec[(size_t)i * stride + wr_col];
      cnt = bl ? nl : ct[i] - nl;
      start = bl ? st[i] : st[i] + nl;
      sp = 1;
      nch = (cnt + chunk - 1) / chunk;
    }
    long long a = sp, b = nch;
#pragma unroll
// ... 441 lines not shown
}

template <typename CodeT, int MODE>
static void pair_hist_launch(bool has_vb, bool posv, int n_work, size_t lds, hipStream_t s, const void* codes_col,
                             long long ncol, const int* ridx, const float* va, const float* vb, const int4* work,
                             const int* pfeat, int Bs, float s0, float s1, double* Hp, double* pwyy) {
  const CodeT* cc = (const CodeT*)codes_col;
#define PHL(V, PV)                                                                                                \
  hipLaunchKernelGGL((pair_hist_kernel<CodeT, MODE, V, PV>), dim3(n_work), dim3(256), lds, s, cc, ncol, ridx, va, \
                     vb, work, pfeat, Bs, s0, s1, Hp, pwyy)
  if (has_vb) { if (posv) PHL(true, true); else PHL(true, false); }
  else { if (posv) PHL(false, true); else PHL(false, false); }
#undef PHL
}

extern "C" int h2o_pair_hist(const void* codes_col, int code_bytes, long long ncol, const int* ridx, const float* va,
                             const float* vb, const int* work, int n_work, const int* pfeat, int Bs, int mode,
                             int posv, float s0, float s1, double* Hp, double* pwyy, hipStream_t s) {
  if (n_work <= 0) return 0;
  if (Bs < 2 || Bs > 4096 || (mode != 0 && mode != 1) || (mode == 1 && vb == nullptr)) return -1;
  const size_t lds = (size_t)Bs * 2 * sizeof(unsigned long long);
  const int4* w = (const int4*)work;
  const bool hv = vb != nullptr;
  if (code_bytes == 1) {
    if (mode == 0) pair_hist_launch<uint8_t, 0>(hv, posv, n_work, lds, s, codes_col, ncol, ridx, va, vb, w, pfeat, Bs, s0, s1, Hp, pwyy);
    else pair_hist_launch<uint8_t, 1>(hv, posv, n_work, lds, s, codes_col, ncol, ridx, va, vb, w, pfeat, Bs, s0, s1, Hp, pwyy);
  } else {
    if (mode == 0) pair_hist_launch<uint16_t, 0>(hv, posv, n_work, lds, s, codes_col, ncol, ridx, va, vb, w, pfeat, Bs, s0, s1, Hp, pwyy);
    else pair_hist_launch<uint16_t, 1>(hv, posv, n_work, lds, s, codes_col, ncol, ridx, va, vb, w, pfeat, Bs, s0, s1, Hp, pwyy);
  }
  return (int)hipGetLastError();
}

__global__ __launch_bounds__(256) void gbm_grad_kernel(const float* __restrict__ y, float* __restrict__ f,
                                                       const float* __restrict__ w, int mode, long long n,
                                                       float* __restrict__ z, const float* __restrict__ d) {
  const long long stride = (long long)gridDim.x * 256;
  for (long long i = (long long)blockIdx.x * 256 + threadIdx.x; i < n; i += stride) {
    float fi = f[i];
    if (d != nullptr) {
      fi += d[i];
      f[i] = fi;
    }
    const float p = mode == 1 ? 1.f / (1.f + expf(-fi)) : fi;
    float v = y[i] - p;
    if (w != nullptr && !(w[i] > 0.f)) v = __builtin_nanf("");
    z[i] = v;
  }
}

extern "C" int h2o_gbm_grad(const float* y, float* f, const float* w, int mode, long long n, float* z,
                            const float* d, hipStream_t s) {
  if (n <= 0) return 0;
  const long long blocks = std::min<long long>((n + 255) / 256, 8192);
  hipLaunchKernelGGL(gbm_grad_kernel, dim3((unsigned)blocks), dim3(256), 0, s, y, f, w, mode, n, z, d);
  return (int)hipGetLastError();
}

__global__ __launch_bounds__(256) void part_items_kernel(const long long* __restrict__ seg, int n, int chunk, int nw,
                                                         int4* __restrict__ work, long long* __restrict__ meta,
                                                         int* __restrict__ fbase) {
  const long long* st = seg;
  const long long* ct = seg + n;
  const long long* cb = seg + 2 * (long long)n;
  const long long* wb = seg + 3 * (long long)n;
  for (int c = blockIdx.x * 256 + threadIdx.x; c < nw; c += gridDim.x * 256) {
    int lo = 0, hi = n - 1;
    while (lo < hi) {
      const int mid = (lo + hi + 1) >> 1;
      if (cb[mid] <= c) lo = mid;
      else hi = mid - 1;
    }
    const int s = lo;
    const long long k = c - cb[s];
    const long long start = st[s] + k * chunk;
    const long long cnt = min((long long)chunk, ct[s] - k * chunk);
    work[c] = make_int4(s, (int)start, (int)cnt, (int)k);
    meta[c] = s;
    meta[(long long)nw + c] = cb[s];
    meta[2 * (long long)nw + c] = st[s];
    meta[3 * (long long)nw + c] = k * chunk;
    fbase[c] = (int)(wb[s] + k * (chunk / 64));
  }
}

extern "C" int h2o_part_items(const long long* seg, int n, int chunk, int nw, int* work, long long* meta,
                              int* fbase, hipStream_t s) {
  if (nw <= 0) return 0;
  if (chunk % 64 != 0 || n <= 0) return -1;
  const int blocks = std::min((nw + 255) / 256, 1024);
  hipLaunchKernelGGL(part_items_kernel, dim3(blocks), dim3(256), 0, s, seg, n, chunk, nw, (int4*)work, meta, fbase);
  return (int)hipGetLastError();
}

#define DT_RS 16
enum {
  DT_GAIN = 0, DT_FEAT = 1, DT_T = 2, DT_OPT = 3, DT_L0 = 4, DT_L1 = 5, DT_R0 = 6, DT_R1 = 7, DT_T0 = 8, DT_T1 = 9,
  DT_OK = 10, DT_NL = 11, DT_NAW = 12, DT_ST = 13, DT_CT = 14, DT_VAL = 15
};
#define DT_MAXN 4096

__device__ __forceinline__ void dt_seg(int kind, const double* __restrict__ rec, int i, int D, int wch,
                                       long long& start, long long& cnt) {
  const double* r = rec + (size_t)i * DT_RS;
  start = 0;
  cnt = 0;
  const long long st = (long long)r[DT_ST], ct = (long long)r[DT_CT];
  if (kind == 0) {
    start = st; cnt = ct;
  } else if (kind == 1) {
    if (r[DT_OK] > 0.0) {
      const long long nl = (long long)r[DT_NL];
      const bool bl = r[DT_L0 + wch] <= r[DT_R0 + wch];
      cnt = bl ? nl : ct - nl;
      start = bl ? st : st + nl;
    }
  } else {
    const int lv = 31 - __clz(i + 1);
    if (ct > 0 && ((lv == D && kind == 2) || (lv < D && !(r[DT_OK] > 0.0)))) { start = st; cnt = ct; }
  }
}

__global__ __launch_bounds__(1024) void dt_items_kernel(int kind, const double* __restrict__ rec, int n, int D,
                                                        int wch, int chunk, int cap, int4* __restrict__ work,
                                                        int* __restrict__ fbase, int* __restrict__ slot_wb,
                                                        int* __restrict__ counts) {
  __shared__ int sb[DT_MAXN + 1];
  __shared__ int wb[DT_MAXN + 1];
  __shared__ long long wtot[2][16];
  __shared__ long long carry[2];
  const int lane = threadIdx.x & 63, wv = threadIdx.x >> 6, nwv = blockDim.x >> 6;
  if (threadIdx.x == 0) carry[0] = carry[1] = 0;
  __syncthreads();
  for (int base = 0; base < n; base += blockDim.x) {
    const int i = base + threadIdx.x;
    long long start = 0, cnt = 0;
    if (i < n) dt_seg(kind, rec, i, D, wch, start, cnt);
    const long long nch = cnt > 0 ? (cnt + chunk - 1) / chunk : 0;
    const long long nwd = cnt > 0 ? (cnt + 63) / 64 : 0;
    long long a = nch, b = nwd;
#pragma unroll
    for (int o = 1; o < 64; o <<= 1) {
      const long long ta = __shfl_up(a, o, 64), tb = __shfl_up(b, o, 64);
      if (lane >= o) { a += ta; b += tb; }
    }
    if (lane == 63) { wtot[0][wv] = a; wtot[1][wv] = b; }
    __syncthreads();
    if (wv == 0) {
      long long x = lane < nwv ? wtot[0][lane] : 0, y = lane < nwv ? wtot[1][lane] : 0;
#pragma unroll
      for (int o = 1; o < 16; o <<= 1) {
        const long long tx = __shfl_up(x, o, 64), ty = __shfl_up(y, o, 64);
        if (lane >= o) { x += tx; y += ty; }
      }
      if (lane < nwv) { wtot[0][lane] = x; wtot[1][lane] = y; }
    }
    __syncthreads();
    if (i < n) {
      sb[i] = (int)(carry[0] + (wv > 0 ? wtot[0][wv - 1] : 0) + a - nch);
      wb[i] = (int)(carry[1] + (wv > 0 ? wtot[1][wv - 1] : 0) + b - nwd);
    }
    __syncthreads();
    if (threadIdx.x == 0) { carry[0] += wtot[0][nwv - 1]; carry[1] += wtot[1][nwv - 1]; }
    __syncthreads();
  }
  const int total = (int)min(carry[0], (long long)cap);
  if (slot_wb != nullptr)
    for (int i = threadIdx.x; i < n; i += blockDim.x) slot_wb[i] = wb[i];
  for (int it = threadIdx.x; it < total; it += blockDim.x) {
    int lo = 0, hi = n - 1;
    while (lo < hi) {
      const int mid = (lo + hi + 1) >> 1;
      if (sb[mid] <= it) lo = mid; else hi = mid - 1;
    }
    long long start, cnt;
    dt_seg(kind, rec, lo, D, wch, start, cnt);
    const int k = it - sb[lo];
    const long long p = start + (long long)k * chunk;
    work[it] = make_int4(lo, (int)p, (int)min((long long)chunk, cnt - (long long)k * chunk), k);
    if (fbase != nullptr) fbase[it] = wb[lo] + k * (chunk / 64);
  }
  if (threadIdx.x == 0) { counts[0] = n; counts[1] = total; }
}

__global__ __launch_bounds__(1024) void dt_offsets_kernel(const int* __restrict__ cnt, const int4* __restrict__ work,
                                                          const int* __restrict__ counts, double* __restrict__ rec,
                                                          int n, double* __restrict__ rec_next,
                                                          int* __restrict__ loff, int* __restrict__ roff) {
  __shared__ long long nl_s[DT_MAXN];
  __shared__ long long wtot[16];
  __shared__ long long carry;
  const int nw = counts[1];
  const int lane = threadIdx.x & 63, wv = threadIdx.x >> 6, nwv = blockDim.x >> 6;
  for (int s = threadIdx.x; s < n; s += blockDim.x) nl_s[s] = 0;
  if (threadIdx.x == 0) carry = 0;
  __syncthreads();
  for (int base = 0; base < nw; base += blockDim.x) {
    const int i = base + threadIdx.x;
    const long long v = i < nw ? (long long)cnt[i] : 0;
    long long x = v;
#pragma unroll
    for (int o = 1; o < 64; o <<= 1) {
      const long long t = __shfl_up(x, o, 64);
      if (lane >= o) x += t;
    }
    if (lane == 63) wtot[wv] = x;
    __syncthreads();
    if (wv == 0) {
      long long w = lane < nwv ? wtot[lane] : 0;
#pragma unroll
      for (int o = 1; o < 16; o <<= 1) {
        const long long t = __shfl_up(w, o, 64);
        if (lane >= o) w += t;
      }
      if (lane < nwv) wtot[lane] = w;
    }
    __syncthreads();
    if (i < nw) loff[i] = (int)(carry + (wv > 0 ? wtot[wv - 1] : 0) + x - v);
    __syncthreads();
    if (threadIdx.x == 0) carry += wtot[nwv - 1];
    __syncthreads();
  }
  __syncthreads();
  for (int i = threadIdx.x; i < nw; i += blockDim.x) {
    const int4 wk = work[i];
    if (i == nw - 1 || work[i + 1].x != wk.x) nl_s[wk.x] = (long long)loff[i] + cnt[i] - (long long)loff[i - wk.w];
  }
  for (int i = threadIdx.x; i < nw; i += blockDim.x) roff[i] = loff[i - work[i].w];
  __syncthreads();
  for (int i = threadIdx.x; i < nw; i += blockDim.x) {
    const int4 wk = work[i];
    const long long st = (long long)rec[(size_t)wk.x * DT_RS + DT_ST];
    const long long lpre = (long long)loff[i] - (long long)roff[i];
    loff[i] = (int)(st + lpre);
    roff[i] = (int)(st + nl_s[wk.x] + ((long long)wk.y - st) - lpre);
  }
  for (int s = threadIdx.x; s < n; s += blockDim.x) {
    double* r = rec + (size_t)s * DT_RS;
    const long long nl = nl_s[s];
    r[DT_NL] = (double)nl;
    if (rec_next != nullptr) {
      double* c = rec_next + (size_t)(2 * s) * DT_RS;
      const bool ok = r[DT_OK] > 0.0;
      const double st = r[DT_ST], ct = r[DT_CT];
      c[DT_ST] = ok ? st : 0.0;
      c[DT_CT] = ok ? (double)nl : 0.0;
      c[DT_RS + DT_ST] = ok ? st + (double)nl : 0.0;
      c[DT_RS + DT_CT] = ok ? ct - (double)nl : 0.0;
    }
  }
}

__global__ __launch_bounds__(256) void dt_sibling_kernel(const double* __restrict__ Hb, const double* __restrict__ Hp,
                                                         const double* __restrict__ rec_par, int np, int BsC, int C,
                                                         int clamp_mask, int wch, double* __restrict__ H,
                                                         const double* __restrict__ wyy_b,
                                                         const double* __restrict__ wyy_p,
                                                         double* __restrict__ wyy_out) {
  const int i = blockIdx.x, f = blockIdx.y;
  const double* r = rec_par + (size_t)i * DT_RS;
  const bool ok = r[DT_OK] > 0.0;
  const bool bl = r[DT_L0 + wch] <= r[DT_R0 + wch];
  const int bs = 2 * i + (bl ? 0 : 1), ds = 2 * i + (bl ? 1 : 0);
  const double* hb = Hb + ((size_t)f * np + i) * BsC;
  const double* hp = Hp + ((size_t)f * np + i) * BsC;
  double* ob = H + ((size_t)f * 2 * np + bs) * BsC;
  double* od = H + ((size_t)f * 2 * np + ds) * BsC;
  for (int k = threadIdx.x; k < BsC; k += blockDim.x) {
    double b = 0.0, d = 0.0;
    if (ok) {
      b = hb[k];
      d = hp[k] - b;
      if ((clamp_mask >> (k % C)) & 1) d = fmax(d, 0.0);
    }
    ob[k] = b;
    od[k] = d;
  }
  if (wyy_out != nullptr && f == 0 && threadIdx.x == 0) {
    wyy_out[bs] = ok ? wyy_b[i] : 0.0;
    wyy_out[ds] = ok ? wyy_p[i] - wyy_b[i] : 0.0;
  }
}

__global__ __launch_bounds__(256) void dt_leaf_vals_kernel(double* __restrict__ rec, const double* __restrict__ sums,
                                                           int nh, int D, const float* __restrict__ lr, double maxabs,
                                                           float* __restrict__ vals) {
  const int h = blockIdx.x * blockDim.x + threadIdx.x;
  if (h >= nh) return;
  const int lv = 31 - __clz(h + 1);
  const bool exists = h == 0 || rec[(size_t)((h - 1) >> 1) * DT_RS + DT_OK] > 0.0;
  const bool leaf = exists && (lv == D || !(rec[(size_t)h * DT_RS + DT_OK] > 0.0));
  double v = 0.0;
  if (leaf) {
    const double den = sums[2 * h + 1];
    v = den != 0.0 ? sums[2 * h] / den : 0.0;
    v = fmin(fmax(v, -maxabs), maxabs) * (double)lr[0];
  }
  vals[h] = (float)v;
  rec[(size_t)h * DT_RS + DT_VAL] = v;
}

__global__ void dt_root_kernel(double* __restrict__ rec, long long N) {
  if (threadIdx.x == 0) { rec[DT_ST] = 0.0; rec[DT_CT] = (double)N; }
}

__global__ __launch_bounds__(256) void leaf_flag_sums_kernel(
    const float* __restrict__ zp, const int4* __restrict__ work, const int* __restrict__ fbase,
    const unsigned long long* __restrict__ flags, const double* __restrict__ rec_lvl, int heap0, int mode,
    double* __restrict__ out, const int* __restrict__ nw_dev) {
  if (nw_dev != nullptr && (int)blockIdx.x >= nw_dev[1]) return;
  const int4 wk = work[blockIdx.x];
  if (!(rec_lvl[(size_t)wk.x * DT_RS + DT_OK] > 0.0)) return;
  const int fb = fbase[blockIdx.x];
  const int end = wk.y + wk.z;
  double la = 0.0, lb = 0.0, ra = 0.0, rb = 0.0;
  constexpr int U = 4;
  for (int base = wk.y + (int)threadIdx.x; base < end; base += 256 * U) {
    float z[U];
    unsigned long long w[U];
#pragma unroll
    for (int u = 0; u < U; ++u) {
      const int pc = min(base + u * 256, end - 1);
      z[u] = zp[pc];
      w[u] = flags[fb + ((pc - wk.y) >> 6)];
    }
#pragma unroll
    for (int u = 0; u < U; ++u) {
      const int p = base + u * 256;
      const bool L = (w[u] >> ((p - wk.y) & 63)) & 1ull;
      if (p < end && z[u] == z[u]) {
        const double az = fabs((double)z[u]);
        const double b = mode == 1 ? az * (1.0 - az) : 1.0;
        if (L) { la += (double)z[u]; lb += b; } else { ra += (double)z[u]; rb += b; }
      }
    }
  }
  la = wave_sum(la); lb = wave_sum(lb); ra = wave_sum(ra); rb = wave_sum(rb);
  __shared__ double red[4][4];
  if (lane_id() == 0) { red[0][wave_id()] = la; red[1][wave_id()] = lb; red[2][wave_id()] = ra; red[3][wave_id()] = rb; }
  __syncthreads();
  if (threadIdx.x < 4) {
    const int c = threadIdx.x;
    double* o = out + 2 * (size_t)(2 * (heap0 + wk.x) + 1 + (c >> 1)) + (c & 1);
    gbl_add(o, red[c][0] + red[c][1] + red[c][2] + red[c][3]);
  }
}

#define LG_MAXSEG 2048
__global__ __launch_bounds__(1024) void lg_segs_kernel(const double* __restrict__ rec, int nh, int D, int last,
                                                       const int* __restrict__ slot_wb, int cap, long long N,
                                                       int chk, int icap, int4* __restrict__ segs,
                                                       int2* __restrict__ items, int* __restrict__ nseg) {
  __shared__ int wcnt[16];
  __shared__ int carry;
  const int lane = threadIdx.x & 63, wv = threadIdx.x >> 6, nwv = blockDim.x >> 6;
  const unsigned long long below = (lane == 0) ? 0ull : (~0ull >> (64 - lane));
  if (threadIdx.x == 0) carry = 0;
  __syncthreads();
  for (int base = 0; base < nh; base += blockDim.x) {
    const int i = base + threadIdx.x;
    bool is = false;
    int4 sg = make_int4(0, 0, 0, -1);
    if (i < nh) {
      const double* r = rec + (size_t)i * DT_RS;
      const int lv = 31 - __clz(i + 1);
      const long long st = min(max((long long)r[DT_ST], 0ll), N);
      const long long ct = min((long long)r[DT_CT], N - st);
      const bool ok = r[DT_OK] > 0.0;
      if (ct > 0) {
        if (last == 0) {
          is = lv == D || !ok;
        } else if (lv < D) {
          is = !ok || lv == D - 1;
          if (ok && lv == D - 1) sg.w = slot_wb[i - ((1 << (D - 1)) - 1)];
        }
      }
      sg.x = i; sg.y = (int)st; sg.z = (int)ct;
    }
    const unsigned long long bal = __ballot(is);
    if (lane == 0) wcnt[wv] = __popcll(bal);
    __syncthreads();
    int pre = carry, tot = 0;
    for (int w = 0; w < nwv; ++w) { pre += (w < wv) ? wcnt[w] : 0; tot += wcnt[w]; }
    const int pos = pre + __popcll(bal & below);
    if (is && pos < cap) segs[pos] = sg;
    __syncthreads();
    if (threadIdx.x == 0) carry += tot;
    __syncthreads();
  }
  const int S = min(carry, cap);
  __shared__ int ib[LG_MAXSEG + 1];
  __shared__ int icarry;
  if (threadIdx.x == 0) icarry = 0;
  __syncthreads();
  for (int base = 0; base < S; base += blockDim.x) {
    const int s = base + threadIdx.x;
    const int nch = s < S ? (segs[s].z + chk - 1) / chk : 0;
    int x = nch;
#pragma unroll
    for (int o = 1; o < 64; o <<= 1) {
      const int t = __shfl_up(x, o, 64);
      if (lane >= o) x += t;
    }
    if (lane == 63) wcnt[wv] = x;
    __syncthreads();
    int off = icarry, tot = 0;
    for (int w = 0; w < nwv; ++w) { off += (w < wv) ? wcnt[w] : 0; tot += wcnt[w]; }
    if (s < S) ib[s] = off + x - nch;
    __syncthreads();
    if (threadIdx.x == 0) icarry += tot;
    __syncthreads();
  }
  const int nit = min(icarry, icap);
  for (int it = threadIdx.x; it < nit; it += blockDim.x) {
    int a = 0, b = S - 1;
    while (a < b) {
      const int mid = (a + b + 1) >> 1;
      if (ib[mid] <= it) a = mid; else b = mid - 1;
    }
    items[it] = make_int2(a, it - ib[a]);
  }
  if (threadIdx.x == 0) { nseg[0] = S; nseg[1] = nit; }
}

__global__ __launch_bounds__(256) void lg_bounds_kernel(const int* __restrict__ ridx, const int4* __restrict__ segs,
                                                        const int* __restrict__ nseg, const int2* __restrict__ items,
                                                        int sh, int nb, int scap, int chk, int* __restrict__ T) {
  if ((int)blockIdx.x >= nseg[1]) return;
  const int2 it = items[blockIdx.x];
  const int s = it.x;
  const int4 sg = segs[s];
  const int send = sg.y + sg.z;
  const int beg = sg.y + it.y * chk, end = min(send, beg + chk);
  for (int p = beg + (int)threadIdx.x; p < end; p += 256) {
    const int bcur = min(ridx[p] >> sh, nb - 1);
    const int bprev = p > sg.y ? (ridx[p - 1] >> sh) : -1;
    for (int b = max(bprev + 1, 0); b <= bcur; ++b) T[(size_t)b * scap + s] = p;
    if (p == send - 1)
      for (int b = max(bcur + 1, 0); b <= nb; ++b) T[(size_t)b * scap + s] = send;
  }
}

#define LG_NONE 0xFFFFFFFFu
__global__ __launch_bounds__(1024) void lg_gather_kernel(const int* __restrict__ ridx, const int4* __restrict__ segs,
                                                        const int* __restrict__ nseg, const int* __restrict__ T,
                                                        int scap, const unsigned long long* __restrict__ flags,
                                                        const float* __restrict__ vals, long long N, int R,
                                                        float* __restrict__ d) {
  extern __shared__ __attribute__((aligned(16))) int lg_lds[];
  unsigned int* v = reinterpret_cast<unsigned int*>(lg_lds);
  int* pre = lg_lds + R;
  int* lo = pre + scap + 1;
  __shared__ int wtot[16];
  const int nt = blockDim.x, nwv = nt >> 6;
  const int S = nseg[0];
  const long long row0 = (long long)blockIdx.x * R;
  const int nrows = (int)min((long long)R, N - row0);
  const int lane = threadIdx.x & 63, wv = threadIdx.x >> 6;
  for (int i = threadIdx.x; i < R; i += nt) v[i] = LG_NONE;
  const int K = (S + nt - 1) / nt;
  const int s0 = threadIdx.x * K;
  const int* Ta = T + (size_t)blockIdx.x * scap;
  const int* Tb = Ta + scap;
  int sum = 0;
  for (int k = 0; k < K; ++k) {
    const int s = s0 + k;
    if (s < S) {
      const int a = Ta[s];
      lo[s] = a;
      pre[s] = sum;
      sum += max(Tb[s] - a, 0);
    }
  }
  int x = sum;
#pragma unroll
  for (int o = 1; o < 64; o <<= 1) {
    const int t = __shfl_up(x, o, 64);
    if (lane >= o) x += t;
  }
  if (lane == 63) wtot[wv] = x;
  __syncthreads();
  int off = x - sum;
  int total = 0;
  for (int w = 0; w < nwv; ++w) { off += (w < wv) ? wtot[w] : 0; total += wtot[w]; }
  for (int k = 0; k < K; ++k) {
    const int s = s0 + k;
    if (s < S) pre[s] += off;
  }
  if (threadIdx.x == 0) pre[S] = total;
  __syncthreads();
  constexpr int U = 4;
  for (int j0 = threadIdx.x; j0 < total; j0 += nt * U) {
    int sl[U], p[U], r[U];
#pragma unroll
    for (int u = 0; u < U; ++u) {
      const int j = min(j0 + u * nt, total - 1);
      int a = 0, b = S - 1;
      while (a < b) {
        const int mid = (a + b) >> 1;
        if (pre[mid + 1] > j) b = mid; else a = mid + 1;
      }
      sl[u] = a;
      p[u] = lo[a] + (j - pre[a]);
    }
#pragma unroll
    for (int u = 0; u < U; ++u) r[u] = ridx[p[u]];
#pragma unroll
    for (int u = 0; u < U; ++u) {
      const int4 sg = segs[sl[u]];
      int h = sg.x;
      if (sg.w >= 0) {
        const int q = p[u] - sg.y;
        h = 2 * h + (((flags[sg.w + (q >> 6)] >> (q & 63)) & 1ull) ? 1 : 2);
      }
      const long long li = (long long)r[u] - row0;
      if (j0 + u * nt < total && li >= 0 && li < nrows) v[li] = __float_as_uint(vals[h]);
    }
  }
  __syncthreads();
  float* dr = d + row0;
  for (int i = threadIdx.x * 4; i < nrows; i += nt * 4) {
    const uint4 q = *reinterpret_cast<const uint4*>(v + i);
    if (i + 3 < nrows && q.x != LG_NONE && q.y != LG_NONE && q.z != LG_NONE && q.w != LG_NONE) {
      *reinterpret_cast<uint4*>(dr + i) = q;
    } else {
      const unsigned int e[4] = {q.x, q.y, q.z, q.w};
#pragma unroll
      for (int k = 0; k < 4; ++k)
        if (i + k < nrows && e[k] != LG_NONE) dr[i + k] = __uint_as_float(e[k]);
    }
  }
}

extern "C" {

int h2o_dt_items2(int kind, const double* rec, int n, int D, int wch, int chunk, int cap, int* work, int* fbase,
                  int* slot_wb, int* counts, hipStream_t s) {
  if (n <= 0 || n > DT_MAXN || chunk <= 0 || (fbase != nullptr && chunk % 64 != 0)) return -1;
  hipLaunchKernelGGL(dt_items_kernel, dim3(1), dim3(1024), 0, s, kind, rec, n, D, wch, chunk, cap, (int4*)work, fbase,
                     slot_wb, counts);
  return (int)hipGetLastError();
}

int h2o_dt_items(int kind, const double* rec, int n, int D, int wch, int chunk, int cap, int* work, int* fbase,
                 int* counts, hipStream_t s) {
  return h2o_dt_items2(kind, rec, n, D, wch, chunk, cap, work, fbase, nullptr, counts, s);
}

int h2o_dt_offsets(const int* cnt, const int* work, const int* counts, double* rec, int n, double* rec_next, int* loff,
                   int* roff, hipStream_t s) {
  if (n <= 0 || n > DT_MAXN) return -1;
  hipLaunchKernelGGL(dt_offsets_kernel, dim3(1), dim3(1024), 0, s, cnt, (const int4*)work, counts, rec, n, rec_next,
                     loff, roff);
  return (int)hipGetLastError();
}

int h2o_dt_sibling(const double* Hb, const double* Hp, const double* rec_par, int np, int F, int BsC, int C,
                   int clamp_mask, int wch, double* H, const double* wyy_b, const double* wyy_p, double* wyy_out,
                   hipStream_t s) {
  if (np <= 0 || F <= 0) return 0;
  hipLaunchKernelGGL(dt_sibling_kernel, dim3(np, F), dim3(256), 0, s, Hb, Hp, rec_par, np, BsC, C, clamp_mask, wch, H,
                     wyy_b, wyy_p, wyy_out);
  return (int)hipGetLastError();
}

int h2o_dt_leaf_vals(double* rec, const double* sums, int nh, int D, const float* lr, double maxabs, float* vals,
                     hipStream_t s) {
  hipLaunchKernelGGL(dt_leaf_vals_kernel, dim3((nh + 255) / 256), dim3(256), 0, s, rec, sums, nh, D, lr, maxabs, vals);
  return (int)hipGetLastError();
}

int h2o_dt_root(double* rec, long long N, hipStream_t s) {
  hipLaunchKernelGGL(dt_root_kernel, dim3(1), dim3(64), 0, s, rec, N);
  return (int)hipGetLastError();
}

int h2o_part_flags_dev(const void* codes, int code_bytes, long long rs, long long fs, const int* ridx, const int* work,
                       const int* fbase, int n_cap, const int* feat, const uint8_t* masks, int Bs,
                       unsigned long long* flags, int* cnt, const int* counts, hipStream_t s) {
  if (n_cap <= 0) return 0;
  if (code_bytes == 1)
    hipLaunchKernelGGL(part_flags_kernel<uint8_t>, dim3(n_cap), dim3(256), 0, s, (const uint8_t*)codes, rs, fs, ridx,
                       (const int4*)work, fbase, feat, masks, Bs, flags, cnt, counts);
  else
    hipLaunchKernelGGL(part_flags_kernel<uint16_t>, dim3(n_cap), dim3(256), 0, s, (const uint16_t*)codes, rs, fs,
                       ridx, (const int4*)work, fbase, feat, masks, Bs, flags, cnt, counts);
  return (int)hipGetLastError();
}

int h2o_part_compact_dev(const int* ridx, const int* work, const int* fbase, int n_cap,
                         const unsigned long long* flags, const int* loff, const int* roff, int* out, const float* pa,
                         float* pa_out, const int* counts, hipStream_t s) {
  if (n_cap <= 0) return 0;
  hipLaunchKernelGGL(part_compact_kernel<4>, dim3(n_cap), dim3(256), 0, s, ridx, (const int4*)work, fbase, flags, loff,
                     roff, out, pa, pa_out, counts);
  return (int)hipGetLastError();
}

int h2o_leaf_pos_dev(const float* zp, const int* work, int n_cap, int mode, double* out, const int* counts,
                     hipStream_t s) {
  if (n_cap <= 0) return 0;
  hipLaunchKernelGGL(leaf_pos_kernel, dim3(n_cap), dim3(256), 0, s, zp, (const int4*)work, mode, out, counts);
  return (int)hipGetLastError();
}

int h2o_leaf_scatter_dev(const int* ridx, const int* work, int n_cap, const float* val, float* d, const int* counts,
                         hipStream_t s) {
  if (n_cap <= 0) return 0;
  hipLaunchKernelGGL(leaf_scatter_kernel, dim3(n_cap), dim3(256), 0, s, ridx, (const int4*)work, val, d, counts);
  return (int)hipGetLastError();
}

int h2o_leaf_flag_sums_dev(const float* zp, const int* work, const int* fbase, int n_cap,
                           const unsigned long long* flags, const double* rec_lvl, int D, int mode, double* out,
                           const int* counts, hipStream_t s) {
  if (n_cap <= 0) return 0;
  if (D < 1) return -1;
  hipLaunchKernelGGL(leaf_flag_sums_kernel, dim3(n_cap), dim3(256), 0, s, zp, (const int4*)work, fbase, flags, rec_lvl,
                     (1 << (D - 1)) - 1, mode, out, counts);
  return (int)hipGetLastError();
}

#define LG_CHK 8192
int h2o_leaf_gather_lds(int R, int scap) { return (R + 2 * scap + 1) * (int)sizeof(int); }
int h2o_leaf_gather_items(long long N, int scap) { return (int)(scap + N / LG_CHK + 1); }

int h2o_leaf_gather_dev(const double* rec, int nh, int D, int last, const int* slot_wb, const int* ridx,
                        const unsigned long long* flags, const float* vals, long long N, int R, int scap, int* segs,
                        int* items, int* nseg, int* T, float* d, hipStream_t s) {
  if (N <= 0) return 0;
  if (nh <= 0 || D < 1 || R < 256 || (R & (R - 1)) != 0 || scap < (1 << D) || scap > LG_MAXSEG ||
      N > (1ll << 31) - (1 << 24))
    return -1;
  if (last != 0 && (slot_wb == nullptr || flags == nullptr)) return -1;
  const int lds = h2o_leaf_gather_lds(R, scap);
  if (lds > 160 * 1024 - 256) return -1;
  static int lds_set = 0;
  if (lds > lds_set) {
    if (hipFuncSetAttribute((const void*)lg_gather_kernel, hipFuncAttributeMaxDynamicSharedMemorySize, lds) !=
        hipSuccess)
      return -2;
    lds_set = lds;
  }
  const int nb = (int)((N + R - 1) / R);
  const int icap = h2o_leaf_gather_items(N, scap);
  const int nt = min(1024, max(256, R / 16));
  hipLaunchKernelGGL(lg_segs_kernel, dim3(1), dim3(1024), 0, s, rec, nh, D, last, slot_wb, scap, N, LG_CHK, icap,
                     (int4*)segs, (int2*)items, nseg);
  hipLaunchKernelGGL(lg_bounds_kernel, dim3(icap), dim3(256), 0, s, ridx, (const int4*)segs, nseg,
                     (const int2*)items, 31 - __builtin_clz(R), nb, scap, LG_CHK, T);
  hipLaunchKernelGGL(lg_gather_kernel, dim3(nb), dim3(nt), lds, s, ridx, (const int4*)segs, nseg, T, scap, flags,
                     vals, N, R, d);
  return (int)hipGetLastError();
}

}

extern "C" __global__ __launch_bounds__(1024) void dt_colmask_kernel(
    int d, const double* __restrict__ rec_par, const long long* __restrict__ elig, const int* __restrict__ m_dev,
    const int* __restrict__ k_dev, const unsigned long long* __restrict__ seed_dev, int f0, int Fl,
    unsigned char* __restrict__ okm) {
  __shared__ int wsum[16];
  __shared__ int carry;
  const int n = 1 << d;
  const int m = m_dev[0], k = k_dev[d];
  const unsigned long long seed = seed_dev[d];
  const int lane = threadIdx.x & 63, wv = threadIdx.x >> 6, nwv = blockDim.x >> 6;
  if (threadIdx.x == 0) carry = 0;
  __syncthreads();
  for (int base = 0; base < n; base += blockDim.x) {
    const int i = base + threadIdx.x;
    int ex = 0;
    if (i < n) ex = d == 0 ? 1 : (rec_par[(size_t)(i >> 1) * DT_RS + DT_OK] > 0.0 ? 1 : 0);
    int a = ex;
#pragma unroll
    for (int o = 1; o < 64; o <<= 1) {
      const int t = __shfl_up(a, o, 64);
      if (lane >= o) a += t;
    }
    if (lane == 63) wsum[wv] = a;
    __syncthreads();
    if (wv == 0) {
      int x = lane < nwv ? wsum[lane] : 0;
#pragma unroll
      for (int o = 1; o < 16; o <<= 1) {
        const int t = __shfl_up(x, o, 64);
        if (lane >= o) x += t;
      }
      if (lane < nwv) wsum[lane] = x;
    }
    __syncthreads();
    const int rank = carry + (wv > 0 ? wsum[wv - 1] : 0) + a - ex;
    if (i < n) {
      unsigned char* row = okm + (size_t)i * Fl;
      for (int f = 0; f < Fl; ++f) row[f] = 0;
      if (ex) {
        const unsigned long long b0 = smix64(seed ^ ((unsigned long long)rank * 0xD1B54A32D192ED03ull));
        int taken = 0;
        for (int j = 0; j < m && taken < k; ++j) {
          const double u = (double)(smix64(b0 + (unsigned long long)j) >> 11) * (1.0 / 9007199254740992.0);
          if (u * (double)(m - j) < (double)(k - taken)) {
            ++taken;
            const long long f = elig[j] - f0;
            if (f >= 0 && f < Fl) row[f] = 1;
          }
        }
      }
    }
    __syncthreads();
    if (threadIdx.x == 0) carry += wsum[nwv - 1];
    __syncthreads();
  }
}

extern "C" int h2o_dt_colmask(int d, const double* rec_par, const long long* elig, const int* m_dev,
                              const int* k_dev, const unsigned long long* seed_dev, int f0, int Fl,
                              unsigned char* okm, hipStream_t s) {
  if (d < 0 || d > 12 || Fl <= 0) return (int)hipErrorInvalidValue;
  if (d > 0 && rec_par == nullptr) return (int)hipErrorInvalidValue;
  hipLaunchKernelGGL(dt_colmask_kernel, dim3(1), dim3(1024), 0, s, d, rec_par, elig, m_dev, k_dev, seed_dev, f0,
                     Fl, okm);
  return (int)hipGetLastError();
}
```

h2o3_amd/ops/tree_ops.py:

```python
from __future__ import annotations

import ctypes
import math
import os

import numpy as np
import torch

from . import _native

_LDS_BUDGET = 80 * 1024
_c_void = ctypes.c_void_p
_c_int = ctypes.c_int
_c_ll = ctypes.c_longlong



_upload_seq = 0
_synced_upto = 0


def upload_mark():
    return _upload_seq


def host_synced(mark=None):
    global _synced_upto
    m = _upload_seq if mark is None else mark
    if m > _synced_upto:
        _synced_upto = m


class _PinnedRing:

    def __init__(self, n=16):
        self.bufs = [None] * n
        self.dbufs = [None] * n
        self.seq = [-1] * n
        self.i = 0

    def upload(self, a: np.ndarray, dev):
        global _upload_seq
        k = self.i
        self.i = (self.i + 1) % len(self.bufs)
        if self.seq[k] >= _synced_upto:
            torch.cuda.current_stream(dev).synchronize()
            host_synced()
        nb = max(a.nbytes, 8)
        buf = self.bufs[k]
        if buf is None or buf.numel() < nb:
            cap = max(nb, 1 << 16)
            buf = self.bufs[k] = torch.empty(cap, dtype=torch.uint8, pin_memory=True)
            self.dbufs[k] = torch.empty(cap, dtype=torch.uint8, device=dev)
        dbuf = self.dbufs[k]
        if dbuf.device != torch.device(dev) if not isinstance(dev, torch.device) else dbuf.device != dev:
            dbuf = self.dbufs[k] = torch.empty(buf.numel(), dtype=torch.uint8, device=dev)
        tdt = torch.from_numpy(a[:0]).dtype
        stage = buf[:a.nbytes].view(tdt).view(a.shape)
        stage.numpy()[...] = a
        out = dbuf[:a.nbytes].view(tdt).view(a.shape)
        out.copy_(stage, non_blocking=True)
        self.seq[k] = _upload_seq
        _upload_seq += 1
        return out


_ring = None


def _h2d(a, dev):
    a = np.ascontiguousarray(a)
    if dev.type != "cuda":
        return torch.from_numpy(a)
    global _ring
    if _ring is None:
        _ring = _PinnedRing()
    return _ring.upload(a, dev)


def _ptr(t):
    return ctypes.c_void_p(t.data_ptr()) if t is not None else ctypes.c_void_p(0)


_ENV_CACHE = None


def env(key, default=None):
    c = _ENV_CACHE
    if c is None:
        return os.environ.get(key, default)
    k = (key, default)
    v = c.get(k, c)
    if v is c:
        v = c[k] = os.environ.get(key, default)
    return v


class env_scope:

    def __enter__(self):
        global _ENV_CACHE
        self._prev = _ENV_CACHE
        _ENV_CACHE = {}
        return self

    def __exit__(self, *exc):
        global _ENV_CACHE
        _ENV_CACHE = self._prev
        return False


_raw_stream = getattr(torch._C, "_cuda_getCurrentRawStream", None)
_get_device = getattr(torch._C, "_cuda_getDevice", None)


def _stream():
    if _raw_stream is not None and _get_device is not None:
        return ctypes.c_void_p(_raw_stream(_get_device()))
    return ctypes.c_void_p(torch.cuda.current_stream().cuda_stream)


def _lib():
    lib = _native.get_lib("tree_hist")
    if lib is not None and not getattr(lib, "_typed", False):
        lib.h2o_hist_build.argtypes = [_c_void, _c_int, _c_int, _c_void, _c_void, _c_void, _c_void, _c_int,
                                       _c_int, _c_int, _c_int, ctypes.c_float, ctypes.c_float, _c_void, _c_int, _c_int,
                                       _c_int, _c_void, _c_int, _c_void, _c_void]
        lib.h2o_hist_quad3.argtypes = [_c_void, _c_int, _c_void, _c_void, _c_void, _c_void, _c_int, _c_int, _c_int,
                                       _c_int, ctypes.c_float, ctypes.c_float, _c_void, _c_int, _c_int, _c_int,
                                       _c_void, _c_int, _c_ll, _c_int, _c_void, _c_void]
        lib.h2o_hist_bm.argtypes = [_c_void, _c_int, _c_void, _c_void, _c_void, _c_void, _c_int, _c_int, _c_int,
                                    _c_int, ctypes.c_float, ctypes.c_float, _c_void, _c_int, _c_int, _c_void, _c_int,
                                    _c_ll, _c_int, _c_void, _c_void, _c_void, _c_void]
        lib.h2o_hist_build_pk.argtypes = [_c_void, _c_int, _c_int, _c_void, _c_void, _c_void, _c_void, _c_int,
                                          _c_int, _c_int, _c_int, ctypes.c_float, _c_ll, _c_void, _c_int, _c_int,
                                          _c_void, _c_int, _c_void, _c_void]
        lib.h2o_part_flags.argtypes = [_c_void, _c_int, _c_ll, _c_ll, _c_void, _c_void, _c_void, _c_int, _c_void,
                                       _c_void, _c_int, _c_void, _c_void, _c_void]
        lib.h2o_part_compact.argtypes = [_c_void, _c_void, _c_void, _c_int, _c_void, _c_void, _c_void, _c_void,
                                         _c_void, _c_void, _c_void]
        lib.h2o_part_count.argtypes = [_c_void, _c_int, _c_ll, _c_ll, _c_void, _c_void, _c_int, _c_void,
                                       _c_void, _c_int, _c_void, _c_void]
        lib.h2o_part_scatter.argtypes = [_c_void, _c_int, _c_ll, _c_ll, _c_void, _c_void, _c_int, _c_void,
                                         _c_void, _c_int, _c_void, _c_void, _c_void, _c_void, _c_void, _c_void,
                                         _c_void, _c_void]
        lib.h2o_fill_nid.argtypes = [_c_void, _c_void, _c_int, _c_void, _c_void]
        lib._typed = True
    return lib


def channels(mode: int) -> int:
    return 1 if mode == 2 else (4 if mode == 3 else 2)


def feature_group(F: int, Bs: int, mode: int, budget: int = _LDS_BUDGET) -> int:
    import os
    if env("H2O3_HIST_FGL"):
        return max(1, min(64, int(os.environ["H2O3_HIST_FGL"]), F))
    C = channels(mode)
    fmax = max(1, min(64, budget // (Bs * C * 8)))
    best = None
    for ng in range(1, F + 1):
        fgl = -(-F // ng)
        if fgl > fmax:
            continue
        cost = ng / (64 // fgl) + 0.05 * ng
        key = (round(cost, 6), ng)
        if best is None or key < best[0]:
            best = (key, fgl)
        if fgl == 1:
            break
    return best[1] if best else 1


def quad_groups(F: int, Fp: int, Bs: int, pack: bool, budget: int = _LDS_BUDGET):
    CL = 1 if pack else 2
    fmax = max(4, min(64, (budget // ((Bs * CL + CL) * 8)) // 4 * 4))
    fmax = int(env("H2O3_HIST_FGW", fmax))
    n_fg = -(-F // fmax)
    while True:
        fgw = -(-(-(-F // n_fg)) // 4) * 4
        if n_fg * fgw <= Fp or fgw <= 4:
            return n_fg, fgw
        n_fg += 1


def bm_groups(F: int, Fp: int, Bs: int, one_channel: bool):
    if env("H2O3_HIST_BM", "1") != "1" or Bs > 256 or Bs % 4 or Fp % 4:
        return None
    cl = 1 if one_channel else 2
    best = None
    for G in (64, 32, 16):
        if cl == 2 and G == 64:
            continue
        n_fg = -(-F // G)
        if n_fg * G > Fp or Bs * G * cl * 8 > 160 * 1024:
            continue
        if best is None or n_fg < best[0]:
            best = (n_fg, G)
    return best


def bm_part(n_items, n_fg, Bs, G, one_channel, dev):
    if env("H2O3_HIST_BM_RED", "1") != "1":
        return None
    cl = 1 if one_channel else 2
    return torch.empty(int(n_items) * n_fg * Bs * G * cl, dtype=torch.int64, device=dev)


def make_work(starts, counts, slots, chunk):
    st = np.asarray(starts, dtype=np.int64).reshape(-1)
    ct = np.asarray(counts, dtype=np.int64).reshape(-1)
    sl = np.asarray(list(slots), dtype=np.int64).reshape(-1)
    m = ct > 0
    st, ct, sl = st[m], ct[m], sl[m]
    if st.size == 0:
        return np.zeros((0, 4), dtype=np.int32)
    nch = (ct + chunk - 1) // chunk
    rep = np.repeat(np.arange(st.size), nch)
    k = np.arange(int(nch.sum())) - np.repeat(np.cumsum(nch) - nch, nch)
    p = st[rep] + k * chunk
    c = np.minimum(chunk, st[rep] + ct[rep] - p)
    return np.stack([sl[rep], p, c, k], 1).astype(np.int32)


def channel_max(va, vb, mode):
    if mode == 3:
        a, b = channel_max(va, vb[0], 0), channel_max(va, vb[1], 0)
        return [max(a[0], b[0]), max(a[1], b[1])]
    if mode == 0:
        w = vb if vb is not None else None
        m1 = torch.nan_to_num(va.abs() * (w.abs() if w is not None else 1), nan=0.0).max() if va.numel() \
            else va.new_zeros(())
        m0 = w.abs().max() if (w is not None and w.numel()) else va.new_ones(())
    elif mode == 1:
        m0, m1 = va.abs().max(), vb.abs().max()
    else:
        m0 = vb.abs().max() if vb is not None else va.new_ones(())
        m1 = m0
    t = torch.stack([m0.float(), m1.float()]).cpu().tolist()
    return [x if x == x else 0.0 for x in t]


def fixed_point_scale(maxv, nmax):
    import math
    if not maxv or maxv <= 0 or not math.isfinite(maxv):
        return 1.0
    k = math.floor(math.log2(2.0 ** 62 / (maxv * max(nmax, 1))))
    return float(2.0 ** max(min(k, 100), -100))


def _pack_scale(vmax, chunk):
    vm = max(float(vmax), 1e-30)
    k = math.floor(math.log2((2.0 ** 40 - 2 * chunk) / (2.0 * chunk * vm * 1.0001)))
    s1 = 2.0 ** k
    return s1, int(math.ceil(vm * s1))


_PK_BUDGET = 152 * 1024
_HIST_CHUNK_ROWS = 131072
_HIST_MIN_BLOCKS = 512


def hist_chunk(total, n_fg, target_blocks=None):
    tb = env("H2O3_HIST_TB", target_blocks)
    if tb is not None:
        n_chunks = max(1, int(tb) // n_fg)
    else:
        rows = int(env("H2O3_HIST_CHUNK", _HIST_CHUNK_ROWS))
        n_chunks = max(-(-_HIST_MIN_BLOCKS // n_fg), -(-total // rows))
    return max(2048, -(-total // n_chunks))


def hist_build(bd, ridx, va, vb, mode, starts, counts, n_slots, use_native=None, target_blocks=None, vmax=None,
               want_wyy=False, posv=False, unit_w=False, need_mask=None):
    C = channels(mode)
    dev = ridx.device
    nh = bd.F * n_slots * bd.Bs * C
    if want_wyy and mode == 0:
        buf = torch.zeros(nh + n_slots, dtype=torch.float64, device=dev)
        hist = buf[:nh].view(bd.F, n_slots, bd.Bs, C)
        wyy = buf[nh:]
    else:
        hist = torch.zeros((bd.F, n_slots, bd.Bs, C), dtype=torch.float64, device=dev)
        wyy = None
    ret = (lambda: (hist, wyy)) if want_wyy else (lambda: hist)
    native = dev.type == "cuda" if use_native is None else use_native
    if native:
        lib = _lib()
        kern = env("H2O3_HIST_KERNEL", "quad")
        total = int(sum(counts))
        if total == 0:
            return ret()
        quad = bd.code_bytes == 1 and bd.Fp % 4 == 0 and bd.Bs <= 256 and kern == "quad" and mode in (0, 1, 2)
        pack = quad and mode == 0 and unit_w and env("H2O3_HIST_PACK", "1") == "1"
        big = env("H2O3_HIST_BIG", "0") == "1"
        qbudget = 156 * 1024 if big else _LDS_BUDGET
        bm = None
        if quad:
            bm = bm_groups(bd.F, bd.Fp, bd.Bs, pack or mode == 2)
            n_fg, fgw = bm if bm is not None else quad_groups(bd.F, bd.Fp, bd.Bs, pack, qbudget)
        pkw = False
        if not quad:
            pkw = mode == 0 and unit_w and bd.code_bytes == 2 and env("H2O3_HIST_PACK", "1") == "1"
            FG = feature_group(bd.F, bd.Bs, 2 if pkw else mode, budget=_PK_BUDGET if pkw else _LDS_BUDGET)
            n_fg = (bd.F + FG - 1) // FG
        chunk = hist_chunk(total, n_fg, target_blocks)
        if pkw and chunk >= (1 << 23):
            pkw = False
            FG = feature_group(bd.F, bd.Bs, mode)
            n_fg = (bd.F + FG - 1) // FG
        if pack and chunk >= (1 << 23):
            pack = False
            bm = bm_groups(bd.F, bd.Fp, bd.Bs, mode == 2)
            n_fg, fgw = bm if bm is not None else quad_groups(bd.F, bd.Fp, bd.Bs, False, qbudget)
        items = make_work(starts, counts, range(n_slots), chunk)
        if len(items) == 0:
            return ret()
        work = _h2d(items, dev)

        def _need(fg):
            if need_mask is None:
                return None
            m = need_mask[:, :bd.F].to(device=dev, dtype=torch.bool)
            ng = (bd.F + fg - 1) // fg
            if ng * fg > bd.F:
                m = torch.cat([m, torch.zeros((m.shape[0], ng * fg - bd.F), dtype=torch.bool, device=dev)], 1)
            return m.view(m.shape[0], ng, fg).any(2).to(torch.uint8).contiguous()
        threads = 512 if chunk >= 8192 else 256
        if vmax is None:
            vmax = channel_max(va, vb, mode)
        s0, s1 = (fixed_point_scale(m, chunk) for m in vmax)
        if quad:
            bq = -1
            if pack:
                s1, bq = _pack_scale(vmax[1] if vb is None else max(vmax[1], 0.0), chunk)
            need = _need(fgw)
            if bm is not None:
                part = bm_part(len(items), n_fg, bd.Bs, fgw, pack or mode == 2, dev)
                rc = lib.h2o_hist_bm(_ptr(bd.codes), bd.Fp, _ptr(ridx), _ptr(va), _ptr(vb), _ptr(work), len(items),
                                     bd.F, 0, bd.Bs, s0, s1, _ptr(hist), n_slots, mode, _ptr(wyy), 1 if posv else 0,
                                     bq, fgw, _ptr(need), None, _ptr(part), _stream())
                if rc != 0:
                    raise RuntimeError(f"h2o_hist_bm failed: error {rc} (F={bd.F}, Fp={bd.Fp}, G={fgw})")
                return ret()
            rc = lib.h2o_hist_quad3(_ptr(bd.codes), bd.Fp, _ptr(ridx), _ptr(va), _ptr(vb), _ptr(work), len(items),
                                    bd.F, 0, bd.Bs, s0, s1, _ptr(hist), n_slots, mode, 1024 if big else 512, _ptr(wyy),
                                    1 if posv else 0, bq, fgw, _ptr(need), _stream())
            if rc != 0:
                raise RuntimeError(f"h2o_hist_quad3 failed: error {rc} (F={bd.F}, Fp={bd.Fp}, fgw={fgw})")
            return ret()
        need = _need(FG)
        if pkw:
            s1p, bqp = _pack_scale(vmax[1] if vb is None else max(vmax[1], 0.0), chunk)
            rc = lib.h2o_hist_build_pk(_ptr(bd.codes), bd.code_bytes, bd.Fp, _ptr(ridx), _ptr(va), _ptr(vb),
                                       _ptr(work), len(items), bd.F, FG, bd.Bs, s1p, bqp, _ptr(hist), n_slots,
                                       threads, _ptr(wyy), 1 if posv else 0, _ptr(need), _stream())
            if rc != 0:
                raise RuntimeError(f"h2o_hist_build_pk failed: hip error {rc}")
            return ret()
        rc = lib.h2o_hist_build(_ptr(bd.codes), bd.code_bytes, bd.Fp, _ptr(ridx), _ptr(va), _ptr(vb), _ptr(work),
                                len(items), bd.F, FG, bd.Bs, s0, s1, _ptr(hist), n_slots, mode, threads, _ptr(wyy),
                                1 if posv else 0, _ptr(need), _stream())
        if rc != 0:
            raise RuntimeError(f"h2o_hist_build failed: hip error {rc}")
        return ret()
    if posv:
        va_r = torch.empty_like(va)
        va_r[ridx.long()] = va
        vb_r = None
        if vb is not None:
            vb_r = torch.empty_like(vb)
            vb_r[ridx.long()] = vb
        va, vb = va_r, vb_r
    _hist_build_torch(bd, ridx, va, vb, mode, starts, counts, hist)
    if wyy is not None:
        for slot, (st, ct) in enumerate(zip(starts, counts)):
            r = ridx[st: st + ct].long()
            w = vb[r].to(torch.float64) if vb is not None else torch.ones(r.numel(), dtype=torch.float64, device=dev)
            y = va[r].to(torch.float64)
            wyy[slot] = (w * y * y).sum()
    return ret()


def _hist_build_torch(bd, ridx, va, vb, mode, starts, counts, hist):
    F, Bs = bd.F, bd.Bs
    C = channels(mode)
    codes = bd.codes
    for slot, (st, ct) in enumerate(zip(starts, counts)):
        if ct <= 0:
            continue
        r = ridx[st: st + ct].long()
        a = va[r].to(torch.float32)
        if mode == 0:
            w = vb[r].to(torch.float32) if vb is not None else torch.ones_like(a)
            vals = torch.stack([w, w * a], 1)
        elif mode == 1:
            vals = torch.stack([a, vb[r].to(torch.float32)], 1)
        else:
            w = vb[r].to(torch.float32) if vb is not None else torch.ones_like(a)
            vals = w.reshape(-1, 1)
        cd = codes[r][:, :F].to(torch.int64)
        idx = (torch.arange(F, device=cd.device).reshape(1, F) * Bs + cd).reshape(-1)
        flat = torch.zeros((F * Bs, C), dtype=torch.float64, device=cd.device)
        v = vals.unsqueeze(1).expand(-1, F, C).reshape(-1, C).to(torch.float64)
        flat.index_add_(0, idx, v)
        hist[:, slot] = flat.reshape(F, Bs, C)
    return hist


_PAIR_CHUNK = 16384
_PAIR_KP = int(os.environ.get("H2O3_PAIR_KP", 4))


def pair_hist(bd, ridx, va, vb, mode, node_st, node_ct, pair_node, pair_feat, vmax=None, posv=False,
              want_wyy=False, use_native=None, chunk=_PAIR_CHUNK):
    assert mode in (0, 1)
    dev = ridx.device
    st = np.asarray(node_st, dtype=np.int64)
    ct = np.asarray(node_ct, dtype=np.int64)
    pn = np.asarray(pair_node, dtype=np.int64)
    pf = np.asarray(pair_feat, dtype=np.int64)
    P, n = pn.size, st.size
    Bs = bd.Bs
    first = np.ones(P, dtype=bool)
    first[1:] = pn[1:] != pn[:-1]
    wyy_n = torch.zeros(n, dtype=torch.float64, device=dev) if (want_wyy and mode == 0) else None
    native = (dev.type == "cuda" and bd.codes_col is not None) if use_native is None else use_native
    if P == 0:
        return torch.zeros((0, Bs, 2), dtype=torch.float64, device=dev), wyy_n
    if native:
        lib = _lib()
        if not getattr(lib, "_typed_pair", False):
            lib.h2o_pair_hist.argtypes = [_c_void, _c_int, _c_ll, _c_void, _c_void, _c_void, _c_void, _c_int,
                                          _c_void, _c_int, _c_int, _c_int, ctypes.c_float, ctypes.c_float, _c_void,
                                          _c_void, _c_void]
            lib._typed_pair = True
        pct = ct[pn]
        nch = np.maximum((pct + chunk - 1) // chunk, 0)
        live = pct > 0
        rep = np.repeat(np.arange(P), nch)
        k = np.arange(int(nch.sum())) - np.repeat(np.cumsum(nch) - nch, nch)
        start = st[pn][rep] + k * chunk
        cnt = np.minimum(chunk, pct[rep] - k * chunk)
        flags = (nch[rep] == 1).astype(np.int64) | first[rep].astype(np.int64) * 2
        items = np.stack([rep, start, cnt, flags], 1).astype(np.int32)
        Hp = torch.empty((P, Bs, 2), dtype=torch.float64, device=dev)
        multi = np.nonzero((nch > 1) | ~live)[0]
        if multi.size:
            Hp.index_fill_(0, _h2d(multi.astype(np.int64), dev), 0.0)
        pwyy = torch.zeros(P, dtype=torch.float64, device=dev) if wyy_n is not None else None
        if len(items):
            buf = _h2d(np.concatenate([items.reshape(-1), pf.astype(np.int32)]), dev)
            work, pfd = buf[:4 * len(items)], buf[4 * len(items):]
            if vmax is None:
                vmax = channel_max(va, vb, mode)
            s0, s1 = (fixed_point_scale(m, min(chunk, int(pct.max()))) for m in vmax)
            rc = lib.h2o_pair_hist(_ptr(bd.codes_col), bd.code_bytes, bd.codes_col.stride(0), _ptr(ridx), _ptr(va),
                                   _ptr(vb), _ptr(work), len(items), _ptr(pfd), Bs, mode, 1 if posv else 0, s0, s1,
                                   _ptr(Hp), _ptr(pwyy), _stream())
            if rc != 0:
                raise RuntimeError(f"h2o_pair_hist failed: {rc}")
        if wyy_n is not None:
            fi = np.nonzero(first)[0]
            wyy_n[_h2d(pn[fi], dev)] = pwyy[_h2d(fi.astype(np.int64), dev)]
        return Hp, wyy_n
    if posv:
        va_r = torch.empty_like(va)
        va_r[ridx.long()] = va
        vb_r = None
        if vb is not None:
            vb_r = torch.empty_like(vb)
            vb_r[ridx.long()] = vb
        va, vb = va_r, vb_r
    pct = torch.as_tensor(ct[pn], device=dev)
    tot = int(pct.sum())
    Hp = torch.zeros((P, Bs, 2), dtype=torch.float64, device=dev)
    if tot == 0:
        return Hp, wyy_n
    prep = torch.repeat_interleave(torch.arange(P, device=dev), pct)
    off = torch.arange(tot, device=dev) - torch.repeat_interleave(torch.cumsum(pct, 0) - pct, pct)
    pos = torch.as_tensor(st[pn], device=dev)[prep] + off
    rows = ridx[pos].long()
    feat = torch.as_tensor(pf, device=dev)[prep]
    code = bd.codes_col[feat, rows].to(torch.int64) if bd.codes_col is not None else \
        bd.codes[rows, feat].to(torch.int64)
    code = code & 0xFFFF if bd.code_bytes == 2 else code
    a = va[rows].to(torch.float64)
    if mode == 0:
        w = vb[rows].to(torch.float64) if vb is not None else (~torch.isnan(a)).to(torch.float64)
        a = torch.nan_to_num(a) if vb is None else a
        vals = torch.stack([w, w * a], 1)
    else:
        vals = torch.stack([a, vb[rows].to(torch.float64)], 1)
    Hp.view(-1, 2).index_add_(0, prep * Bs + code, vals)
    if wyy_n is not None:
        fp = torch.as_tensor(first, device=dev)[prep]
        nodes = torch.as_tensor(pn, device=dev)[prep]
        wyy_n.index_add_(0, nodes[fp], (vals[:, 1] * a)[fp])
    return Hp, wyy_n


def pair_hist_dev(bd, ridx, va, vb, mode, node_st, node_ct, sel, vmax, posv=False, chunk=_PAIR_CHUNK, fbins=None):
    dev = ridx.device
    lib = _lib()
    if not getattr(lib, "_typed_pair", False):
        lib.h2o_pair_hist.argtypes = [_c_void, _c_int, _c_ll, _c_void, _c_void, _c_void, _c_void, _c_int,
                                      _c_void, _c_int, _c_int, _c_int, ctypes.c_float, ctypes.c_float, _c_void,
                                      _c_void, _c_void]
        lib._typed_pair = True
    st = np.asarray(node_st, dtype=np.int64)
    ct = np.asarray(node_ct, dtype=np.int64)
    n, k = sel.shape
    P = n * k
    Bs = bd.Bs
    nch = (ct + chunk - 1) // chunk
    rep = np.repeat(np.arange(n), nch)
    c = np.arange(int(nch.sum())) - np.repeat(np.cumsum(nch) - nch, nch)
    tab = np.stack([rep, st[rep] + c * chunk, np.minimum(chunk, ct[rep] - c * chunk), (nch[rep] == 1)], 1)
    multi = np.nonzero((nch > 1) | (ct == 0))[0]
    tab_d = _h2d(np.concatenate([tab.astype(np.int32).reshape(-1), multi.astype(np.int32)]), dev)
    m = len(tab)
    kp = _PAIR_KP if k > 1 else 1
    if kp > 1:
        ng = -(-k // kp)
        items = tab_d[:4 * m].view(m, 1, 4).expand(m, ng, 4).clone()
        g = torch.arange(ng, dtype=torch.int32, device=dev).view(1, ng)
        items[:, :, 0] = items[:, :, 0] * k + g * kp
        items[:, :, 3] += (g == 0).to(torch.int32) * 2 + torch.clamp(k - g * kp, max=kp) * 256
        n_items = m * ng
    else:
        items = tab_d[:4 * m].view(m, 1, 4).expand(m, k, 4).clone()
        j = torch.arange(k, dtype=torch.int32, device=dev).view(1, k)
        items[:, :, 0] = items[:, :, 0] * k + j
        items[:, :, 3] += (j == 0).to(torch.int32) * 2
        n_items = m * k
    pfeat = sel.to(torch.int32).reshape(-1).contiguous()
    Hp = torch.empty((P, Bs, 2), dtype=torch.float64, device=dev)
    if multi.size:
        Hp.view(n, -1).index_fill_(0, tab_d[4 * m:].long(), 0.0)
    want_wyy = mode == 0
    pwyy = torch.zeros(P, dtype=torch.float64, device=dev) if want_wyy else None
    if m:
        s0, s1 = (fixed_point_scale(v, min(chunk, int(ct.max()))) for v in vmax)
        fn = lib.h2o_pair_hist4 if kp > 1 else lib.h2o_pair_hist
        if kp > 1 and not getattr(lib, "_typed_pair4", False):
            lib.h2o_pair_hist4.argtypes = lib.h2o_pair_hist.argtypes
            lib.h2o_pair_hist4b.argtypes = lib.h2o_pair_hist.argtypes + [_c_void]
            lib._typed_pair4 = True
        args = [_ptr(bd.codes_col), bd.code_bytes, bd.codes_col.stride(0), _ptr(ridx), _ptr(va), _ptr(vb),
                _ptr(items), n_items, _ptr(pfeat), Bs, mode, 1 if posv else 0, s0, s1, _ptr(Hp), _ptr(pwyy),
                _stream()]
        if kp > 1 and fbins is not None:
            rc = lib.h2o_pair_hist4b(*args, _ptr(fbins))
        else:
            rc = fn(*args)
        if rc != 0:
            raise RuntimeError(f"h2o_pair_hist failed: {rc}")
    return Hp, (pwyy.view(n, k)[:, 0].contiguous() if want_wyy else None), pfeat


def gbm_grad(y, f, w, family, out=None, d=None):
    mode = {"gaussian": 0, "bernoulli": 1}[family]
    n = y.numel()
    z = out if out is not None else torch.empty(n, dtype=torch.float32, device=y.device)
    if d is not None and (y.device.type != "cuda" or not f.is_contiguous() or f.dtype != torch.float32):
        f.add_(d.view_as(f))
        d = None
    if y.device.type != "cuda":
        p = f if mode == 0 else torch.sigmoid(f)
        v = (y - p).to(torch.float32)
        if w is not None:
            v = torch.where(w > 0, v, torch.full_like(v, float("nan")))
        z.copy_(v)
        return z
    lib = _lib()
    if not getattr(lib, "_typed_grad", False):
        lib.h2o_gbm_grad.argtypes = [_c_void, _c_void, _c_void, _c_int, _c_ll, _c_void, _c_void, _c_void]
        lib._typed_grad = True
    yc, fc = y.contiguous().to(torch.float32), f.contiguous().to(torch.float32)
    wc = w.contiguous().to(torch.float32) if w is not None else None
    rc = lib.h2o_gbm_grad(_ptr(yc), _ptr(fc), _ptr(wc), mode, n, _ptr(z), _ptr(d), _stream())
    if rc != 0:
        raise RuntimeError(f"h2o_gbm_grad failed: {rc}")
    return z


def partition(bd, ridx, ridx_out, feats, masks, starts, counts, use_native=None, chunk=16384, payload=None):
    dev = ridx.device
    n = len(starts)
    if n == 0:
        return []
    native = dev.type == "cuda" if use_native is None else use_native
    if native:
        lib = _lib()
        items = make_work(starts, counts, range(n), chunk)
        if len(items) == 0:
            return [0] * n
        work = _h2d(items, dev)
        nw = len(items)
        feat_t = _h2d(np.asarray(feats, dtype=np.int32), dev)
        masks = masks.to(torch.uint8).contiguous()
        cnt = torch.empty(nw, dtype=torch.int32, device=dev)
        if bd.codes_col is not None:
            codes, rs, fs = bd.codes_col, 1, bd.nrows_local
        else:
            codes, rs, fs = bd.codes, bd.Fp, 1
        ballot = env("H2O3_PART", "ballot") == "ballot" and (payload is None or payload[1] is None)
        if ballot:
            words = (items[:, 2].astype(np.int64) + 63) // 64
            fb_h = (np.cumsum(words) - words).astype(np.int32)
            fbase = _h2d(fb_h, dev)
            flags = torch.empty(int(words.sum()) + 1, dtype=torch.int64, device=dev)
            rc = lib.h2o_part_flags(_ptr(codes), bd.code_bytes, rs, fs, _ptr(ridx), _ptr(work), _ptr(fbase), nw,
                                    _ptr(feat_t), _ptr(masks), bd.Bs, _ptr(flags), _ptr(cnt), _stream())
        else:
            rc = lib.h2o_part_count(_ptr(codes), bd.code_bytes, rs, fs, _ptr(ridx), _ptr(work), nw, _ptr(feat_t),
                                    _ptr(masks), bd.Bs, _ptr(cnt), _stream())
        if rc != 0:
            raise RuntimeError(f"h2o_part_count failed: {rc}")
        cnt_h = cnt.cpu().numpy().astype(np.int64)
        slot = items[:, 0].astype(np.int64)
        nleft = np.bincount(slot, weights=cnt_h, minlength=n).astype(np.int64)
        csum = np.cumsum(cnt_h) - cnt_h
        first = np.ones(len(items), dtype=bool)
        first[1:] = slot[1:] != slot[:-1]
        first_idx = np.maximum.accumulate(np.where(first, np.arange(len(items)), 0))
        lpre = csum - csum[first_idx]
        st_arr = np.asarray(starts, dtype=np.int64)[slot]
        rpre = (items[:, 1].astype(np.int64) - st_arr) - lpre
        loff = (st_arr + lpre).astype(np.int32)
        roff = (st_arr + nleft[slot] + rpre).astype(np.int32)
        loff_d = _h2d(loff, dev)
        roff_d = _h2d(roff, dev)
        pa, pb, pa_o, pb_o = payload if payload is not None else (None, None, None, None)
        if ballot:
            rc = lib.h2o_part_compact(_ptr(ridx), _ptr(work), _ptr(fbase), nw, _ptr(flags), _ptr(loff_d),
                                      _ptr(roff_d), _ptr(ridx_out), _ptr(pa), _ptr(pa_o), _stream())
            if rc != 0:
                raise RuntimeError(f"h2o_part_compact failed: {rc}")
            return nleft.tolist()
        rc = lib.h2o_part_scatter(_ptr(codes), bd.code_bytes, rs, fs, _ptr(ridx), _ptr(work), nw, _ptr(feat_t),
                                  _ptr(masks), bd.Bs, _ptr(loff_d), _ptr(roff_d), _ptr(ridx_out), _ptr(pa), _ptr(pb),
                                  _ptr(pa_o), _ptr(pb_o), _stream())
        if rc != 0:
            raise RuntimeError(f"h2o_part_scatter failed: {rc}")
        return nleft.tolist()
    out = []
    for i, (st, ct) in enumerate(zip(starts, counts)):
        seg = ridx[st: st + ct]
        if bd.codes_col is not None:
            c = bd.codes_col[feats[i]][seg.long()].to(torch.int64)
        else:
            c = bd.codes[seg.long(), feats[i]].to(torch.int64)
        left = masks[i].to(torch.bool)[c]
        l = seg[left]
        r = seg[~left]
        ridx_out[st: st + l.numel()] = l
        ridx_out[st + l.numel(): st + ct] = r
        if payload is not None:
            pa, pb, pa_o, pb_o = payload
            for src, dst in ((pa, pa_o), (pb, pb_o)):
                v = src[st: st + ct]
                dst[st: st + l.numel()] = v[left]
                dst[st + l.numel(): st + ct] = v[~left]
        out.append(int(l.numel()))
    return out


def _part_chunk(total):
    ev = env("H2O3_PART_CHUNK")
    if ev:
        return int(ev)
    return int(max(4096, min(16384, -(-int(total) // 2048 // 64) * 64)))


def iota_i32(out) -> bool:
    lib = _lib()
    if lib is None or out.dtype != torch.int32 or not out.is_cuda or out.data_ptr() % 16:
        return False
    if not getattr(lib, "_typed_iota", False):
        lib.h2o_iota_i32.argtypes = [_c_void, ctypes.c_longlong, _c_void]
        lib._typed_iota = True
    return lib.h2o_iota_i32(_ptr(out), out.numel(), _stream()) == 0


def partition_async(bd, ridx, ridx_out, feat_d, masks, starts, counts, chunk=None, payload=None, pk=None,
                    pk_col=0):
    dev = ridx.device
    n = len(starts)
    lib = _lib()
    if not getattr(lib, "_typed_async", False):
        lib.h2o_part_offsets.argtypes = [_c_void, _c_void, _c_int, _c_int, _c_void, _c_void, _c_void, _c_void,
                                         _c_int, _c_int, _c_void]
        lib._typed_async = True
    if chunk is None:
        chunk = _part_chunk(sum(counts))
    nleft = torch.empty(n, dtype=torch.int64, device=dev)
    st = np.asarray(starts, dtype=np.int64).reshape(-1)
    ct = np.asarray(counts, dtype=np.int64).reshape(-1)
    nch = (ct + chunk - 1) // chunk
    nw = int(nch.sum())
    if nw == 0:
        nleft.zero_()
        if pk is not None:
            pk[:, pk_col] = 0.0
        return nleft
    wd = (ct + 63) // 64
    total_words = int(wd.sum())
    buf = torch.empty(13 * nw, dtype=torch.int32, device=dev)
    meta = buf[: 8 * nw].view(torch.int64)
    work = buf[8 * nw: 12 * nw]
    fbase = buf[12 * nw:]
    if chunk % 64 == 0 and env("H2O3_PART_ITEMS", "dev") == "dev":
        if not getattr(lib, "_typed_items", False):
            lib.h2o_part_items.argtypes = [_c_void, _c_int, _c_int, _c_int, _c_void, _c_void, _c_void, _c_void]
            lib._typed_items = True
        seg = _h2d(np.concatenate([st, ct, np.cumsum(nch) - nch, np.cumsum(wd) - wd]), dev)
        rc = lib.h2o_part_items(_ptr(seg), n, chunk, nw, _ptr(work), _ptr(meta), _ptr(fbase), _stream())
        if rc != 0:
            raise RuntimeError(f"h2o_part_items failed: {rc}")
    else:
        items = make_work(starts, counts, range(n), chunk)
        words = (items[:, 2].astype(np.int64) + 63) // 64
        fb_h = (np.cumsum(words) - words).astype(np.int64)
        slot = items[:, 0].astype(np.int64)
        first = np.ones(nw, dtype=bool)
        first[1:] = slot[1:] != slot[:-1]
        first_idx = np.maximum.accumulate(np.where(first, np.arange(nw), 0))
        st_arr = st[slot]
        pos = items[:, 1].astype(np.int64) - st_arr
        buf.copy_(_h2d(np.concatenate([np.stack([slot, first_idx, st_arr, pos], 0).reshape(-1).view(np.int32),
                                       items.reshape(-1), fb_h.astype(np.int32)]), dev))
    feat_t = feat_d if feat_d.dtype == torch.int32 else feat_d.to(torch.int32)
    masks = masks if masks.dtype == torch.uint8 else masks.to(torch.uint8)
    cnt = torch.empty(nw, dtype=torch.int32, device=dev)
    if bd.codes_col is not None:
        codes, rs, fs = bd.codes_col, 1, bd.nrows_local
    else:
        codes, rs, fs = bd.codes, bd.Fp, 1
    flags = torch.empty(total_words + 1, dtype=torch.int64, device=dev)
    rc = lib.h2o_part_flags(_ptr(codes), bd.code_bytes, rs, fs, _ptr(ridx), _ptr(work), _ptr(fbase), nw,
                            _ptr(feat_t), _ptr(masks), bd.Bs, _ptr(flags), _ptr(cnt), _stream())
    if rc != 0:
        raise RuntimeError(f"h2o_part_flags failed: {rc}")
    loff = torch.empty(nw, dtype=torch.int32, device=dev)
    roff = torch.empty(nw, dtype=torch.int32, device=dev)
    stride = pk.stride(0) if pk is not None else 0
    rc = lib.h2o_part_offsets(_ptr(cnt), _ptr(meta), nw, n, _ptr(loff), _ptr(roff), _ptr(nleft), _ptr(pk),
                              stride, pk_col, _stream())
    if rc != 0:
        raise RuntimeError(f"h2o_part_offsets failed: {rc}")
    pa, _, pa_o, _ = payload if payload is not None else (None, None, None, None)
    rc = lib.h2o_part_compact(_ptr(ridx), _ptr(work), _ptr(fbase), nw, _ptr(flags), _ptr(loff), _ptr(roff),
                              _ptr(ridx_out), _ptr(pa), _ptr(pa_o), _stream())
    if rc != 0:
        raise RuntimeError(f"h2o_part_compact failed: {rc}")
    return nleft


def hist_build_dev(bd, ridx, va, vb, mode, rec, rec_cols, starts, counts, vmax, posv=False, unit_w=False,
                   target_blocks=None):
    dev = ridx.device
    if dev.type != "cuda" or bd.code_bytes != 1 or bd.Fp % 4 != 0 or bd.Bs > 256 or mode not in (0, 1, 2) or \
            env("H2O3_HIST_KERNEL", "quad") != "quad":
        return None
    lib = _lib()
    if not getattr(lib, "_typed_dev", False):
        lib.h2o_child_work.argtypes = [_c_void, _c_void, _c_void] + [_c_int] * 8 + [_c_void, _c_void, _c_void,
                                                                                  _c_void]
        lib.h2o_hist_quad4.argtypes = [_c_void, _c_int, _c_void, _c_void, _c_void, _c_void, _c_int, _c_int, _c_int,
                                       _c_int, ctypes.c_float, ctypes.c_float, _c_void, _c_int, _c_int, _c_int,
                                       _c_void, _c_int, _c_ll, _c_int, _c_void, _c_void, _c_void]
        lib.h2o_hist_sibling_dev.argtypes = [_c_void, _c_void, _c_void, _c_int, _c_int, _c_int, _c_int, _c_int,
                                             _c_int, _c_int, _c_void, _c_void, _c_void, _c_void, _c_void, _c_void]
        lib._typed_dev = True
    n = len(starts)
    C = channels(mode)
    pack = mode == 0 and unit_w and env("H2O3_HIST_PACK", "1") == "1"
    bm = bm_groups(bd.F, bd.Fp, bd.Bs, pack or mode == 2)
    n_fg, fgw = bm if bm is not None else quad_groups(bd.F, bd.Fp, bd.Bs, pack)
    total = int(sum(counts))
    chunk = hist_chunk((total + 1) // 2, n_fg, target_blocks)
    if pack and chunk >= (1 << 23):
        pack = False
        bm = bm_groups(bd.F, bd.Fp, bd.Bs, mode == 2)
        n_fg, fgw = bm if bm is not None else quad_groups(bd.F, bd.Fp, bd.Bs, False)
    cap = n + total // chunk + 1
    stc = np.concatenate([np.asarray(starts, dtype=np.int64), np.asarray(counts, dtype=np.int64)])
    stc_d = _h2d(stc, dev)
    ibuf = torch.empty(4 * cap + 3 * n + 2, dtype=torch.int32, device=dev)
    work, slots, cnts = ibuf[:4 * cap], ibuf[4 * cap:4 * cap + 3 * n], ibuf[4 * cap + 3 * n:]
    ok_c, nl_c, wl_c, wr_c = rec_cols
    rc = lib.h2o_child_work(_ptr(stc_d), _ptr(stc_d[n:]), _ptr(rec), rec.stride(0), ok_c, nl_c, wl_c, wr_c, n, chunk,
                            cap, _ptr(work), _ptr(slots), _ptr(cnts), _stream())
    if rc != 0:
        raise RuntimeError(f"h2o_child_work failed: {rc}")
    nh = bd.F * n * bd.Bs * C
    want_wyy = mode == 0
    buf = torch.zeros(nh + (n if want_wyy else 0), dtype=torch.float64, device=dev)
    Hb = buf[:nh].view(bd.F, n, bd.Bs, C)
    wyy = buf[nh:] if want_wyy else None
    if vmax is None:
        vmax = channel_max(va, vb, mode)
    s0, s1 = (fixed_point_scale(m, chunk) for m in vmax)
    bq = -1
    if pack:
        s1, bq = _pack_scale(vmax[1] if vb is None else max(vmax[1], 0.0), chunk)
    if bm is not None:
        part = bm_part(cap, n_fg, bd.Bs, fgw, pack or mode == 2, dev)
        rc = lib.h2o_hist_bm(_ptr(bd.codes), bd.Fp, _ptr(ridx), _ptr(va), _ptr(vb), _ptr(work), cap, bd.F, 0, bd.Bs,
                             s0, s1, _ptr(Hb), n, mode, _ptr(wyy), 1 if posv else 0, bq, fgw, None, _ptr(cnts),
                             _ptr(part), _stream())
        if rc != 0:
            raise RuntimeError(f"h2o_hist_bm failed: {rc}")
        return Hb, wyy, slots, cnts
    rc = lib.h2o_hist_quad4(_ptr(bd.codes), bd.Fp, _ptr(ridx), _ptr(va), _ptr(vb), _ptr(work), cap, bd.F, 0, bd.Bs,
                            s0, s1, _ptr(Hb), n, mode, 512, _ptr(wyy), 1 if posv else 0, bq, fgw, None, _ptr(cnts),
                            _stream())
    if rc != 0:
        raise RuntimeError(f"h2o_hist_quad4 failed: {rc}")
    return Hb, wyy, slots, cnts


def hist_sibling_dev(Hb, H_prev, slots, cnts, clamp_mask, wyy_b=None, wyy_prev=None):
    lib = _lib()
    F, nb, Bs, C = Hb.shape
    H = torch.empty((F, 2 * nb, Bs, C), dtype=Hb.dtype, device=Hb.device)
    wyy = torch.empty(2 * nb, dtype=torch.float64, device=Hb.device) if wyy_b is not None else None
    Hp = H_prev.contiguous()
    rc = lib.h2o_hist_sibling_dev(_ptr(Hb), _ptr(Hp), _ptr(slots), nb, Hp.shape[1], 2 * nb, F, Bs * C, C, clamp_mask,
                                  _ptr(H), _ptr(wyy_b), _ptr(wyy_prev), _ptr(wyy), _ptr(cnts), _stream())
    if rc != 0:
        raise RuntimeError(f"h2o_hist_sibling_dev failed: {rc}")
    return H, wyy


def hist_sibling(Hb, H_prev, build_slots, der_slots, par_slots, n_front, clamp_mask, wyy_b=None, wyy_prev=None):
    lib = _lib()
    if not getattr(lib, "_typed_sib", False):
        lib.h2o_hist_sibling.argtypes = [_c_void, _c_void, _c_void, _c_int, _c_int, _c_int, _c_int, _c_int, _c_int,
                                         _c_int, _c_void, _c_void, _c_void, _c_void, _c_void]
        lib._typed_sib = True
    F, nb, Bs, C = Hb.shape
    H = torch.empty((F, n_front, Bs, C), dtype=Hb.dtype, device=Hb.device)
    slots = _h2d(np.asarray([build_slots, der_slots, par_slots], dtype=np.int32).reshape(-1), Hb.device)
    wyy = torch.empty(n_front, dtype=torch.float64, device=Hb.device) if wyy_b is not None else None
    Hb = Hb.contiguous()
    Hp = H_prev.contiguous()
    rc = lib.h2o_hist_sibling(_ptr(Hb), _ptr(Hp), _ptr(slots), nb, Hp.shape[1], n_front, F, Bs * C, C, clamp_mask,
                              _ptr(H), _ptr(wyy_b), _ptr(wyy_prev), _ptr(wyy), _stream())
    if rc != 0:
        raise RuntimeError(f"h2o_hist_sibling failed: {rc}")
    return H, wyy


def fill_nid(ridx, leaf_ids, starts, counts, nrows, use_native=None):
    dev = ridx.device
    if dev.type == "cuda" and use_native is None:
        nid = _fill_nid_tiled(ridx, leaf_ids, starts, counts, nrows)
        if nid is not None:
            return nid
    nid = torch.full((nrows,), -1, dtype=torch.int32, device=dev)
    native = dev.type == "cuda" if use_native is None else use_native
    if native:
        lib = _lib()
        items = make_work(starts, counts, leaf_ids, 65536)
        if len(items):
            work = _h2d(items, dev)
            rc = lib.h2o_fill_nid(_ptr(ridx), _ptr(work), len(items), _ptr(nid), _stream())
            if rc != 0:
                raise RuntimeError(f"h2o_fill_nid failed: {rc}")
        return nid
    for lid, st, ct in zip(leaf_ids, starts, counts):
        nid[ridx[st: st + ct].long()] = lid
    return nid


def _fill_nid_tiled(ridx, leaf_ids, starts, counts, nrows):
    st = np.asarray(starts, dtype=np.int64).reshape(-1)
    ct = np.asarray(counts, dtype=np.int64).reshape(-1)
    lid = np.asarray(leaf_ids, dtype=np.int64).reshape(-1)
    m = ct > 0
    st, ct, lid = st[m], ct[m], lid[m]
    if st.size == 0 or st.size != ct.size:
        return None
    o = np.argsort(st, kind="stable")
    st, ct, lid = st[o], ct[o], lid[o]
    if st[0] != 0 or st[-1] + ct[-1] != nrows or (st.size > 1 and not np.array_equal(st[1:], st[:-1] + ct[:-1])):
        return None
    dev = ridx.device
    bounds = _h2d(st, dev)
    lid_d = _h2d(lid.astype(np.int32), dev)
    pos = torch.arange(nrows, device=dev, dtype=torch.int64)
    seg = torch.searchsorted(bounds, pos, right=True) - 1
    nid = torch.empty(nrows, dtype=torch.int32, device=dev)
    nid[ridx[:nrows].long()] = lid_d[seg]
    return nid


def leaf_pass(ridx, z, w, leaf_ids, starts, counts, n_leaves, nrows, mode, chunk=65536, want_nid=True):
    dev = ridx.device
    lib = _lib()
    if not getattr(lib, "_typed_leaf", False):
        lib.h2o_leaf_pass.argtypes = [_c_void, _c_void, _c_void, _c_void, _c_int, _c_int, _c_void, _c_void, _c_void]
        lib._typed_leaf = True
    out = torch.zeros((n_leaves, 2), dtype=torch.float64, device=dev)
    nid = torch.zeros(nrows, dtype=torch.int32, device=dev) if want_nid else None
    items = make_work(starts, counts, leaf_ids, chunk)
    if len(items) == 0:
        return nid, out
    work = _h2d(items, dev)
    z = z.to(torch.float32).contiguous()
    w = None if w is None else w.to(torch.float32).contiguous()
    rc = lib.h2o_leaf_pass(_ptr(ridx), _ptr(z), _ptr(w), _ptr(work), len(items), int(mode), _ptr(nid), _ptr(out),
                           _stream())
    if rc != 0:
        raise RuntimeError(f"h2o_leaf_pass failed: {rc}")
    return nid, out


def leaf_pos_sums(zpos, leaf_ids, starts, counts, n_leaves, mode, chunk=65536):
    lib = _lib()
    if not getattr(lib, "_typed_lpos", False):
        lib.h2o_leaf_pos.argtypes = [_c_void, _c_void, _c_int, _c_int, _c_void, _c_void]
        lib.h2o_leaf_update.argtypes = [_c_void, _c_void, _c_int, _c_void, _c_void, _c_void]
        lib._typed_lpos = True
    out = torch.zeros((n_leaves, 2), dtype=torch.float64, device=zpos.device)
    items = make_work(starts, counts, leaf_ids, chunk)
    if len(items):
        work = _h2d(items, zpos.device)
        rc = lib.h2o_leaf_pos(_ptr(zpos), _ptr(work), len(items), int(mode), _ptr(out), _stream())
        if rc != 0:
            raise RuntimeError(f"h2o_leaf_pos failed: {rc}")
    return out


def col_sample(n, elig_d, k, seed):
    dev = elig_d.device
    out = torch.empty((n, k), dtype=torch.int64, device=dev)
    lib = _lib()
    if not getattr(lib, "_typed_csamp", False):
        lib.h2o_col_sample.argtypes = [_c_int, _c_int, _c_void, _c_int, ctypes.c_ulonglong, _c_void, _c_void]
        lib._typed_csamp = True
    rc = lib.h2o_col_sample(int(n), int(elig_d.numel()), _ptr(elig_d), int(k), int(seed) & ((1 << 64) - 1),
                            _ptr(out), _stream())
    if rc != 0:
        raise RuntimeError(f"h2o_col_sample failed: {rc}")
    return out


def leaf_scatter(ridx, d, vals, leaf_ids, starts, counts, chunk=65536):
    if d.device.type != "cuda":
        for lid, st, ct in zip(leaf_ids, starts, counts):
            d[ridx[st: st + ct].long()] = vals[lid]
        return d
    lib = _lib()
    if not getattr(lib, "_typed_lscat", False):
        lib.h2o_leaf_scatter.argtypes = [_c_void, _c_void, _c_int, _c_void, _c_void, _c_void]
        lib._typed_lscat = True
    items = make_work(starts, counts, leaf_ids, chunk)
    if len(items):
        work = _h2d(items, d.device)
        rc = lib.h2o_leaf_scatter(_ptr(ridx), _ptr(work), len(items), _ptr(vals), _ptr(d), _stream())
        if rc != 0:
            raise RuntimeError(f"h2o_leaf_scatter failed: {rc}")
    return d


def leaf_update(ridx, f, vals, leaf_ids, starts, counts, chunk=65536):
    lib = _lib()
    if not getattr(lib, "_typed_lpos", False):
        lib.h2o_leaf_pos.argtypes = [_c_void, _c_void, _c_int, _c_int, _c_void, _c_void]
        lib.h2o_leaf_update.argtypes = [_c_void, _c_void, _c_int, _c_void, _c_void, _c_void]
        lib._typed_lpos = True
    items = make_work(starts, counts, leaf_ids, chunk)
    if len(items):
        work = _h2d(items, f.device)
        rc = lib.h2o_leaf_update(_ptr(ridx), _ptr(work), len(items), _ptr(vals), _ptr(f), _stream())
        if rc != 0:
            raise RuntimeError(f"h2o_leaf_update failed: {rc}")


def seg_sum2(ridx, a, b, leaf_ids, starts, counts, n_leaves, use_native=None, chunk=65536):
    dev = ridx.device
    out = torch.zeros((n_leaves, 2), dtype=torch.float64, device=dev)
    native = dev.type == "cuda" if use_native is None else use_native
    if native:
        lib = _lib()
        if not getattr(lib, "_typed_seg", False):
            lib.h2o_seg_sum2.argtypes = [_c_void, _c_void, _c_void, _c_void, _c_int, _c_void, _c_void]
            lib._typed_seg = True
        items = make_work(starts, counts, leaf_ids, chunk)
        if len(items) == 0:
            return out
        work = _h2d(items, dev)
        a = a.to(torch.float32).contiguous()
        b = None if b is None else b.to(torch.float32).contiguous()
        rc = lib.h2o_seg_sum2(_ptr(ridx), _ptr(a), _ptr(b), _ptr(work), len(items), _ptr(out), _stream())
        if rc != 0:
            raise RuntimeError(f"h2o_seg_sum2 failed: {rc}")
        return out
    for lid, st, ct in zip(leaf_ids, starts, counts):
        r = ridx[st: st + ct].long()
        out[lid, 0] = a[r].to(torch.float64).sum()
        if b is not None:
            out[lid, 1] = b[r].to(torch.float64).sum()
    return out
```

Before: 68.57 trees/s.

## Skip root row-index array via identity indexing and add ragged tail histogram variant

When the root node covers all rows, the histogram and partition kernels now take a null row-index pointer and use the position itself as the row id. This avoids the iota fill and the gather reads of ridx at depth 0. The iota is deferred to a conditional kernel that runs only if the root becomes a leaf. A ragged-tail histogram variant is also added for the last feature group, but it is off by default behind an env flag. The kernel body is refactored into a templated device function, which adds template instantiations and some code complexity.

New measurement: 70.41 trees/s (median of 6 runs). 2.7% higher.

```diff
diff --git a/h2o3_amd/models/tree/devtree.py b/h2o3_amd/models/tree/devtree.py
--- a/h2o3_amd/models/tree/devtree.py
+++ b/h2o3_amd/models/tree/devtree.py
@@ -37,6 +37,7 @@
                                    _ci, _cll, _ci, _cv, _cv, _cv, _cv]
         lh.h2o_gbm_grad.argtypes = [_cv, _cv, _cv, _ci, _cll, _cv, _cv, _cv]
         lh.h2o_iota_i32.argtypes = [_cv, _cll, _cv]
+        lh.h2o_dt_root_leaf_iota.argtypes = [_cv, _cv, _cll, _cv]
         lh.h2o_dt_colmask.argtypes = [_ci, _cv, _cv, _cv, _cv, _cv, _ci, _ci, _cv, _cv]
         lh.h2o_dt_items2.argtypes = [_ci, _cv, _ci, _ci, _ci, _ci, _ci, _cv, _cv, _cv, _cv, _cv]
         lh.h2o_leaf_flag_sums_dev.argtypes = [_cv, _cv, _cv, _ci, _cv, _cv, _ci, _ci, _cv, _cv, _cv]
@@ -133,8 +134,11 @@
         dev = drv.dev
         self.dev = dev
         self.pack = tree_ops.env("H2O3_HIST_PACK", "1") == "1"
+        self.ragged = tree_ops.bm_ragged()
         n_fg, G = tree_ops.bm_groups(bd.F, bd.Fp, Bs, self.pack)
         self.n_fg, self.G = n_fg, G
+        self.root_ident = D >= 2 and tree_ops.env("H2O3_DEV_ROOT_IDENT", "1") != "0" and self.pack and G == 64 \
+            and tree_ops.env("H2O3_HIST_BM_LW", "2") != "1"
         self.chunk_r = tree_ops.hist_chunk(N, n_fg)
         self.chunk_c = tree_ops.hist_chunk((N + 1) // 2, n_fg)
         if self.pack and max(self.chunk_r, self.chunk_c) >= (1 << 23):
@@ -255,6 +259,9 @@
         off = (1 << d) - 1
         return self.rec[off * RS:]
 
+    def _ridx_ptr(self, d, cur):
+        return None if (d == 0 and self.root_ident) else _ptr(self.ridx[cur])
+
     def _hist(self, d, cur):
         lh = self.lh
         bd, Bs, C = self.bd, self.Bs, self.C
@@ -268,7 +275,8 @@
             nh = bd.F * Bs * C
             buf = self.Hroot
             buf.zero_()
-            _ck(lh.h2o_hist_bm(_ptr(bd.codes), bd.Fp, _ptr(self.ridx[cur]), _ptr(self.pos[cur]), None,
+            tree_ops.set_bm_ragged(lh, self.ragged)
+            _ck(lh.h2o_hist_bm(_ptr(bd.codes), bd.Fp, self._ridx_ptr(0, cur), _ptr(self.pos[cur]), None,
                                _ptr(self.hwork), self.cap_r, bd.F, 0, Bs, self.s_r[0], self.s_r[1], _ptr(buf), 1, 0,
                                _ptr(buf[nh:]), 1, self.bq_r, self.G, None, _ptr(self.counts), _ptr(self.part), s),
                 "hist_bm(root)")
@@ -285,6 +293,7 @@
         nhb = bd.F * npar * Bs * C
         buf = self.Hb[:nhb + npar]
         buf.zero_()
+        tree_ops.set_bm_ragged(lh, self.ragged)
         _ck(lh.h2o_hist_bm(_ptr(bd.codes), bd.Fp, _ptr(self.ridx[cur]), _ptr(self.pos[cur]), None, _ptr(self.hwork),
                            self.cap_c, bd.F, 0, Bs, self.s_c[0], self.s_c[1], _ptr(buf), npar, 0, _ptr(buf[nhb:]), 1,
                            self.bq_c, self.G, None, _ptr(self.counts), _ptr(self.part), s), "hist_bm(child)")
@@ -337,9 +346,9 @@
         _ck(lh.h2o_dt_items2(0, _ptr(recl), n, self.D, 0, self.chunk_p, self.cap_p, _ptr(self.pwork),
                              _ptr(self.fbase), _ptr(self.slot_wb) if skip else None, _ptr(self.counts), s),
             "dt_items(part)")
-        _ck(lh.h2o_part_flags_dev(_ptr(self.pcodes), 1, self.prs, self.pfs, _ptr(self.ridx[cur]), _ptr(self.pwork),
-                                  _ptr(self.fbase), self.cap_p, _ptr(self.feat_i), _ptr(self.mask), Bs,
-                                  _ptr(self.flags), _ptr(self.cnt), _ptr(self.counts), s), "part_flags_dev")
+        _ck(lh.h2o_part_flags_dev(_ptr(self.pcodes), 1, self.prs, self.pfs, self._ridx_ptr(d, cur),
+                                  _ptr(self.pwork), _ptr(self.fbase), self.cap_p, _ptr(self.feat_i), _ptr(self.mask),
+                                  Bs, _ptr(self.flags), _ptr(self.cnt), _ptr(self.counts), s), "part_flags_dev")
         _ck(lh.h2o_dt_offsets(_ptr(self.cnt), _ptr(self.pwork), _ptr(self.counts), _ptr(recl), n,
                               _ptr(self._rec_lvl(d + 1)), _ptr(self.loff), _ptr(self.roff), s), "dt_offsets")
         if skip:
@@ -348,7 +357,9 @@
                                           _ptr(self.sums), _ptr(self.counts), s), "leaf_flag_sums_dev")
             return cur
         nxt = cur ^ 1
-        _ck(lh.h2o_part_compact_dev(_ptr(self.ridx[cur]), _ptr(self.pwork), _ptr(self.fbase), self.cap_p,
+        if d == 0 and self.root_ident:
+            _ck(lh.h2o_dt_root_leaf_iota(_ptr(recl), _ptr(self.ridx[0]), self.N, s), "dt_root_leaf_iota")
+        _ck(lh.h2o_part_compact_dev(self._ridx_ptr(d, cur), _ptr(self.pwork), _ptr(self.fbase), self.cap_p,
                                     _ptr(self.flags), _ptr(self.loff), _ptr(self.roff), _ptr(self.ridx[nxt]),
                                     _ptr(self.pos[cur]), _ptr(self.pos[nxt]), _ptr(self.counts), s),
             "part_compact_dev")
@@ -363,7 +374,8 @@
         f = drv._f[:, 0]
         _ck(lh.h2o_gbm_grad(_ptr(self._y), _ptr(f), _ptr(self.wbuf) if self.sampled else None,
                             1 if self.bern else 0, self.N, _ptr(self.pos[0]), _ptr(self.dbuf), s), "gbm_grad")
-        _ck(lh.h2o_iota_i32(_ptr(self.ridx[0]), self.N, s), "iota")
+        if not self.root_ident:
+            _ck(lh.h2o_iota_i32(_ptr(self.ridx[0]), self.N, s), "iota")
         self.rec.zero_()
         self.sums.zero_()
         _ck(lh.h2o_dt_root(_ptr(self.rec), self.N, _stream()), "dt_root")
diff --git a/h2o3_amd/ops/csrc/tree_hist.hip b/h2o3_amd/ops/csrc/tree_hist.hip
--- a/h2o3_amd/ops/csrc/tree_hist.hip
+++ b/h2o3_amd/ops/csrc/tree_hist.hip
@@ -279,6 +279,7 @@
   const uint8_t* cc; int Fp; const int* ridx; const float* va; const float* vb; const int4* wk;
   int n_work, n_fg, fgw, F, foff, Bs; float s0, s1; double* hist; int n_slots; double* wyy; long long bq;
   const uint8_t* need; const int* n_work_dev; unsigned long long* part = nullptr;
+  int t_lw = 0, t_lpr = 0, t_ss = 0;
 };
 
 template <int M, bool V, bool PV, bool PK, bool PIPE = true, int LW = 1>
@@ -355,24 +356,185 @@
   return (unsigned long long)(__double_as_longlong(d) - 0x4338000000000000LL);
 }
 
-template <int G, int CL, int MODE, bool HAS_VB, bool POSV, bool PACK, int LW = 2>
+template <int G, int CL, int MODE, bool HAS_VB, bool POSV, bool PACK, int LW, bool IDENT, bool RAG, bool MASK = false>
+__device__ __forceinline__ void hist_bm_body(
+    const uint8_t* __restrict__ codes, int Fp, const int* __restrict__ ridx,
+    const float* __restrict__ va, const float* __restrict__ vb, int4 wk, int lb, int fgi, int n_fg, int fg0, int nf,
+    int Bs, float s0, float s1, double* __restrict__ hist, int n_slots, double* __restrict__ wyy_out, long long bq,
+    unsigned long long* __restrict__ part, int dbg, int t_lpr, int t_ss) {
+  constexpr int C = Chan<MODE>::C;
+  constexpr int NK = 4 * LW;
+  const int LPR = RAG ? t_lpr : G / NK;
+  const int SS = RAG ? t_ss : G / NK;
+  const int RPW = 64 / LPR;
+  constexpr int PITCH = G * CL;
+  constexpr int U = 4;
+  constexpr int PD = 2;
+  using CT = typename CodeW<LW>::T;
+  static_assert(CL == 1 || C == 2, "two LDS channels need a two-channel mode");
+  static_assert(G / NK >= 1, "group narrower than one lane's codes");
+  extern __shared__ __attribute__((aligned(16))) unsigned long long ldsq[];
+  const int lane = threadIdx.x & 63;
+  const int q = lane % LPR;
+  const int rs = lane / LPR;
+  const int wv = threadIdx.x >> 6;
+  const int nwaves = __builtin_amdgcn_readfirstlane((int)(blockDim.x >> 6));
+  unsigned sh[NK], sb[NK], vm = 0;
+#pragma unroll
+  for (int k = 0; k < NK; ++k) {
+    const int kk = (k & ~3) | ((k + rs) & 3);
+    sh[k] = 8u * kk;
+    sb[k] = (unsigned)((kk * SS + q) * 8);
+    if (MASK && NK * q + kk < nf) vm |= 1u << k;
+  }
+  const bool blk_wyy = MODE == 0 && wyy_out != nullptr && fgi == 0;
+  double wyyd = 0.0;
+  const int pend = wk.y + wk.z;
+  const int step = nwaves * RPW;
+  const uint8_t* cbase = codes + fg0 + NK * q;
+  const int p_first = (RAG && rs >= RPW) ? pend : wk.y + wv * RPW + rs;
+  const unsigned long long pk_off = (1ull << 40) + (unsigned long long)bq;
+  const __amdgpu_buffer_rsrc_t rr = __builtin_amdgcn_make_buffer_rsrc((void*)ridx, (short)0, pend * 4, 0x00020000);
+  const __amdgpu_buffer_rsrc_t ra = __builtin_amdgcn_make_buffer_rsrc((void*)va, (short)0, POSV ? pend * 4 : 0,
+                                                                      0x00020000);
+  const __amdgpu_buffer_rsrc_t rb = __builtin_amdgcn_make_buffer_rsrc((void*)vb, (short)0,
+                                                                      (POSV && vb) ? pend * 4 : 0, 0x00020000);
+  int R[PD][U];
+  CT CW[PD][U];
+  float XA[PD][U], XB[PD][U];
+  auto load_r = [&](int p, int (&r)[U]) {
+#pragma unroll
+    for (int u = 0; u < U; ++u) {
+      if constexpr (IDENT) r[u] = p + u * step < pend ? p + u * step : 0;
+      else r[u] = __builtin_amdgcn_raw_buffer_load_b32(rr, p * 4, u * step * 4, 0);
+    }
+  };
+  auto load_v = [&](int p, const int (&r)[U], CT (&cw)[U], float (&xa)[U], float (&xb)[U]) {
+#pragma unroll
+    for (int u = 0; u < U; ++u) {
+      if (POSV) {
+        xa[u] = (MODE == 2) ? 0.f : __int_as_float(__builtin_amdgcn_raw_buffer_load_b32(ra, p * 4, u * step * 4, 0));
+        xb[u] = (HAS_VB || MODE == 1) ? __int_as_float(__builtin_amdgcn_raw_buffer_load_b32(rb, p * 4, u * step * 4, 0))
+                                      : 1.f;
+      } else {
+        xa[u] = (MODE == 2) ? 0.f : va[r[u]];
+        xb[u] = (HAS_VB || MODE == 1) ? vb[r[u]] : 1.f;
+      }
+      cw[u] = *reinterpret_cast<const CT*>(cbase + (size_t)(unsigned)r[u] * (unsigned)Fp);
+    }
+  };
+  const int IT = U * step;
+#pragma unroll
+  for (int d = 0; d < PD; ++d) load_r(p_first + d * IT, R[d]);
+#pragma unroll
+  for (int d = 0; d < PD; ++d) {
+    load_v(p_first + d * IT, R[d], CW[d], XA[d], XB[d]);
+    load_r(p_first + (PD + d) * IT, R[d]);
+  }
+  for (int p0r = p_first; p0r < pend; p0r += PD * IT) {
+#pragma unroll
+    for (int d = 0; d < PD; ++d) {
+      const int p0 = p0r + d * IT;
+#pragma unroll
+      for (int u = 0; u < U; ++u) {
+        const bool inr = p0 + u * step < pend;
+        float c0, c1, yv = 0.f;
+        if (MODE == 0) {
+          const float y = XA[d][u];
+          const float w = HAS_VB ? XB[d][u] : (y == y ? 1.f : 0.f);
+          c0 = w;
+          c1 = w != 0.f ? w * y : 0.f;
+          yv = w != 0.f ? y : 0.f;
+          if (blk_wyy && inr) wyyd += (double)c1 * (double)yv;
+        } else if (MODE == 1) {
+          c0 = XA[d][u]; c1 = XB[d][u];
+        } else {
+          c0 = XB[d][u]; c1 = 0.f;
+        }
+        if (!inr || (c0 == 0.f && c1 == 0.f) || (dbg & 2) || (MASK && vm == 0)) continue;
+        unsigned long long a0, a1 = 0ull;
+        if (PACK) {
+          a0 = fx_signed(yv, s1) + pk_off;
+        } else {
+          a0 = fx_signed(c0, s0);
+          if (CL == 2) a1 = fx_signed(c1, s1);
+        }
+#pragma unroll
+        for (int k = 0; k < NK; ++k) {
+          if (MASK && !((vm >> k) & 1u)) continue;
+          unsigned word;
+          if constexpr (LW == 2) word = (k & 4) ? CW[d][u].y : CW[d][u].x;
+          else word = CW[d][u];
+          const unsigned code = __builtin_amdgcn_ubfe(word, sh[k] & 31u, 8);
+          unsigned long long* h = reinterpret_cast<unsigned long long*>(
+              reinterpret_cast<char*>(ldsq) + code * (unsigned)(PITCH * 8) + sb[k]);
+          __hip_atomic_fetch_add(h, a0, __ATOMIC_RELAXED, __HIP_MEMORY_SCOPE_WORKGROUP);
+          if (CL == 2) __hip_atomic_fetch_add(h + G, a1, __ATOMIC_RELAXED, __HIP_MEMORY_SCOPE_WORKGROUP);
+        }
+      }
+      load_v(p0 + PD * IT, R[d], CW[d], XA[d], XB[d]);
+      load_r(p0 + 2 * PD * IT, R[d]);
+    }
+  }
+  __syncthreads();
+  if (blk_wyy) {
+    double v = q == 0 ? wyyd : 0.0;
+    v = wave_sum(v);
+    if (lane == 0) gbl_add(wyy_out + wk.x, v);
+  }
+  if (part != nullptr) {
+    if (dbg & 1) return;
+    const int n2 = Bs * PITCH / 2;
+    const ulonglong2* src = reinterpret_cast<const ulonglong2*>(ldsq);
+    ulonglong2* dst = reinterpret_cast<ulonglong2*>(part + ((size_t)(lb / n_fg) * n_fg + fgi) * (size_t)(Bs * PITCH));
+    for (int i2 = threadIdx.x; i2 < n2; i2 += blockDim.x) dst[i2] = src[i2];
+    return;
+  }
+  const double inv0 = 1.0 / (double)s0, inv1 = 1.0 / (double)s1;
+  const int si = lane & 15, bi = lane >> 4;
+  constexpr int NSG = G / 16;
+  const int nbq = (dbg & 1) ? 0 : (Bs + 3) >> 2;
+  for (int e = wv; e < nbq * NSG; e += nwaves) {
+    const int b = (e / NSG) * 4 + bi;
+    const int slot = (e % NSG) * 16 + si;
+    const int sq = slot % SS, sk = slot / SS;
+    const int fl = NK * sq + sk;
+    if (b >= Bs || sq >= LPR || sk >= NK || fl >= nf) continue;
+    double* o = hist + ((size_t)(fg0 + fl) * n_slots + wk.x) * (size_t)(Bs * C) + (size_t)b * C;
+    const unsigned long long v = ldsq[b * PITCH + slot];
+    if (PACK) {
+      if (v != 0ull) {
+        const long long cnt = (long long)(v >> 40);
+        const long long low = (long long)(v & ((1ull << 40) - 1));
+        if (dbg & 4) {
+          unsigned long long* ou = reinterpret_cast<unsigned long long*>(o);
+          __hip_atomic_fetch_add(ou, (unsigned long long)cnt, __ATOMIC_RELAXED, __HIP_MEMORY_SCOPE_AGENT);
+          __hip_atomic_fetch_add(ou + 1, (unsigned long long)(low - cnt * bq), __ATOMIC_RELAXED,
+                                 __HIP_MEMORY_SCOPE_AGENT);
+        } else {
+          gbl_add(o, (double)cnt);
+          gbl_add(o + 1, (double)(low - cnt * bq) * inv1);
+        }
+      }
+    } else {
+      if (v != 0ull) gbl_add(o, (double)(long long)v * inv0);
+      if (CL == 2) {
+        const unsigned long long v1 = ldsq[b * PITCH + G + slot];
+        if (v1 != 0ull) gbl_add(o + 1, (double)(long long)v1 * inv1);
+      }
+    }
+  }
+}
+
+template <int G, int CL, int MODE, bool HAS_VB, bool POSV, bool PACK, int LW = 2, int TLW = 0, bool IDENT = false>
 __global__ __launch_bounds__(1024) void hist_bm_kernel(
     const uint8_t* __restrict__ codes, int Fp, const int* __restrict__ ridx,
     const float* __restrict__ va, const float* __restrict__ vb,
     const int4* __restrict__ work, int n_work, int n_fg, int F, int foff, int Bs, float s0, float s1,
     double* __restrict__ hist, int n_slots, double* __restrict__ wyy_out, long long bq,
     const uint8_t* __restrict__ need, const int* __restrict__ n_work_dev, unsigned long long* __restrict__ part,
-    int dbg) {
-  constexpr int C = Chan<MODE>::C;
-  constexpr int NK = 4 * LW;
-  constexpr int LPR = G / NK;
-  constexpr int RPW = 64 / LPR;
+    int dbg, int t_lpr, int t_ss) {
   constexpr int PITCH = G * CL;
-  constexpr int U = 4;
-  constexpr int PD = 2;
-  using CT = typename CodeW<LW>::T;
-  static_assert(CL == 1 || C == 2, "two LDS channels need a two-channel mode");
-  static_assert(LPR >= 1, "group narrower than one lane's codes");
   extern __shared__ __attribute__((aligned(16))) unsigned long long ldsq[];
   const int nwg = n_work_dev != nullptr ? n_work_dev[1] * n_fg : n_work * n_fg;
   if ((int)blockIdx.x >= nwg) return;
@@ -391,158 +553,49 @@
     for (int i = threadIdx.x; i < n2; i += blockDim.x) z[i] = make_ulonglong2(0ull, 0ull);
   }
   __syncthreads();
-  const int lane = threadIdx.x & 63;
-  const int q = lane % LPR;
-  const int rs = lane / LPR;
-  const int wv = threadIdx.x >> 6;
-  const int nwaves = __builtin_amdgcn_readfirstlane((int)(blockDim.x >> 6));
-  unsigned sh[NK], sb[NK];
-#pragma unroll
-  for (int k = 0; k < NK; ++k) {
-    const int kk = (k & ~3) | ((k + rs) & 3);
-    sh[k] = 8u * kk;
-    sb[k] = (unsigned)((kk * LPR + q) * 8);
-  }
-  const bool blk_wyy = MODE == 0 && wyy_out != nullptr && fgi == 0;
-  double wyyd = 0.0;
-  const int pend = wk.y + wk.z;
-  const int step = nwaves * RPW;
-  const uint8_t* cbase = codes + fg0 + NK * q;
-  const int p_first = wk.y + wv * RPW + rs;
-  const unsigned long long pk_off = (1ull << 40) + (unsigned long long)bq;
-  const __amdgpu_buffer_rsrc_t rr = __builtin_amdgcn_make_buffer_rsrc((void*)ridx, (short)0, pend * 4, 0x00020000);
-  const __amdgpu_buffer_rsrc_t ra = __builtin_amdgcn_make_buffer_rsrc((void*)va, (short)0, POSV ? pend * 4 : 0,
-                                                                      0x00020000);
-  const __amdgpu_buffer_rsrc_t rb = __builtin_amdgcn_make_buffer_rsrc((void*)vb, (short)0,
-                                                                      (POSV && vb) ? pend * 4 : 0, 0x00020000);
-  int R[PD][U];
-  CT CW[PD][U];
-  float XA[PD][U], XB[PD][U];
-  auto load_r = [&](int p, int (&r)[U]) {
-#pragma unroll
-    for (int u = 0; u < U; ++u) r[u] = __builtin_amdgcn_raw_buffer_load_b32(rr, p * 4, u * step * 4, 0);
-  };
-  auto load_v = [&](int p, const int (&r)[U], CT (&cw)[U], float (&xa)[U], float (&xb)[U]) {
-#pragma unroll
-    for (int u = 0; u < U; ++u) {
-      if (POSV) {
-        xa[u] = (MODE == 2) ? 0.f : __int_as_float(__builtin_amdgcn_raw_buffer_load_b32(ra, p * 4, u * step * 4, 0));
-        xb[u] = (HAS_VB || MODE == 1) ? __int_as_float(__builtin_amdgcn_raw_buffer_load_b32(rb, p * 4, u * step * 4, 0))
-                                      : 1.f;
-      } else {
-        xa[u] = (MODE == 2) ? 0.f : va[r[u]];
-        xb[u] = (HAS_VB || MODE == 1) ? vb[r[u]] : 1.f;
-      }
-      cw[u] = *reinterpret_cast<const CT*>(cbase + (size_t)(unsigned)r[u] * (unsigned)Fp);
-    }
-  };
-  const int IT = U * step;
-#pragma unroll
-  for (int d = 0; d < PD; ++d) load_r(p_first + d * IT, R[d]);
-#pragma unroll
-  for (int d = 0; d < PD; ++d) {
-    load_v(p_first + d * IT, R[d], CW[d], XA[d], XB[d]);
-    load_r(p_first + (PD + d) * IT, R[d]);
-  }
-  for (int p0r = p_first; p0r < pend; p0r += PD * IT) {
-#pragma unroll
-    for (int d = 0; d < PD; ++d) {
-      const int p0 = p0r + d * IT;
-#pragma unroll
-      for (int u = 0; u < U; ++u) {
-        const bool inr = p0 + u * step < pend;
-        float c0, c1, yv = 0.f;
-        if (MODE == 0) {
-          const float y = XA[d][u];
-          const float w = HAS_VB ? XB[d][u] : (y == y ? 1.f : 0.f);
-          c0 = w;
-          c1 = w != 0.f ? w * y : 0.f;
-          yv = w != 0.f ? y : 0.f;
-          if (blk_wyy && inr) wyyd += (double)c1 * (double)yv;
-        } else if (MODE == 1) {
-          c0 = XA[d][u]; c1 = XB[d][u];
-        } else {
-          c0 = XB[d][u]; c1 = 0.f;
-        }
-        if (!inr || (c0 == 0.f && c1 == 0.f) || (dbg & 2)) continue;
-        unsigned long long a0, a1 = 0ull;
-        if (PACK) {
-          a0 = fx_signed(yv, s1) + pk_off;
-        } else {
-          a0 = fx_signed(c0, s0);
-          if (CL == 2) a1 = fx_signed(c1, s1);
-        }
-#pragma unroll
-        for (int k = 0; k < NK; ++k) {
-          unsigned word;
-          if constexpr (LW == 2) word = (k & 4) ? CW[d][u].y : CW[d][u].x;
-          else word = CW[d][u];
-          const unsigned code = __builtin_amdgcn_ubfe(word, sh[k] & 31u, 8);
-          unsigned long long* h = reinterpret_cast<unsigned long long*>(
-              reinterpret_cast<char*>(ldsq) + code * (unsigned)(PITCH * 8) + sb[k]);
-          __hip_atomic_fetch_add(h, a0, __ATOMIC_RELAXED, __HIP_MEMORY_SCOPE_WORKGROUP);
-          if (CL == 2) __hip_atomic_fetch_add(h + G, a1, __ATOMIC_RELAXED, __HIP_MEMORY_SCOPE_WORKGROUP);
-        }
-      }
-      load_v(p0 + PD * IT, R[d], CW[d], XA[d], XB[d]);
-      load_r(p0 + 2 * PD * IT, R[d]);
-    }
-  }
-  __syncthreads();
-  if (blk_wyy) {
-    double v = q == 0 ? wyyd : 0.0;
-    v = wave_sum(v);
-    if (lane == 0) gbl_add(wyy_out + wk.x, v);
-  }
-  if (part != nullptr) {
-    if (dbg & 1) return;
-    const int n2 = Bs * PITCH / 2;
-    const ulonglong2* src = reinterpret_cast<const ulonglong2*>(ldsq);
-    ulonglong2* dst = reinterpret_cast<ulonglong2*>(part + ((size_t)(lb / n_fg) * n_fg + fgi) * (size_t)(Bs * PITCH));
-    for (int i2 = threadIdx.x; i2 < n2; i2 += blockDim.x) dst[i2] = src[i2];
-    return;
-  }
-  const double inv0 = 1.0 / (double)s0, inv1 = 1.0 / (double)s1;
-  const int si = lane & 15, bi = lane >> 4;
-  constexpr int NSG = G / 16;
-  const int nbq = (dbg & 1) ? 0 : (Bs + 3) >> 2;
-  for (int e = wv; e < nbq * NSG; e += nwaves) {
-    const int b = (e / NSG) * 4 + bi;
-    const int slot = (e % NSG) * 16 + si;
-    const int fl = NK * (slot % LPR) + slot / LPR;
-    if (b >= Bs || fl >= nf) continue;
-    double* o = hist + ((size_t)(fg0 + fl) * n_slots + wk.x) * (size_t)(Bs * C) + (size_t)b * C;
-    const unsigned long long v = ldsq[b * PITCH + slot];
-    if (PACK) {
-      if (v != 0ull) {
-        const long long cnt = (long long)(v >> 40);
-        const long long low = (long long)(v & ((1ull << 40) - 1));
-        if (dbg & 4) {
-          unsigned long long* ou = reinterpret_cast<unsigned long long*>(o);
-          __hip_atomic_fetch_add(ou, (unsigned long long)cnt, __ATOMIC_RELAXED, __HIP_MEMORY_SCOPE_AGENT);
-          __hip_atomic_fetch_add(ou + 1, (unsigned long long)(low - cnt * bq), __ATOMIC_RELAXED,
-                                 __HIP_MEMORY_SCOPE_AGENT);
-        } else {
-          gbl_add(o, (double)cnt);
-          gbl_add(o + 1, (double)(low - cnt * bq) * inv1);
-        }
-      }
-    } else {
-      if (v != 0ull) gbl_add(o, (double)(long long)v * inv0);
-      if (CL == 2) {
-        const unsigned long long v1 = ldsq[b * PITCH + G + slot];
-        if (v1 != 0ull) gbl_add(o + 1, (double)(long long)v1 * inv1);
-      }
-    }
-  }
+  if constexpr (TLW == 3) {
+    if (fgi == n_fg - 1) {
+      hist_bm_body<G, CL, MODE, HAS_VB, POSV, PACK, LW, IDENT, false, true>(codes, Fp, ridx, va, vb, wk, lb, fgi, n_fg,
+                                                                     fg0, nf, Bs, s0, s1, hist, n_slots, wyy_out, bq,
+                                                                     part, dbg, 0, 0);
+      return;
+    }
+  } else if constexpr (TLW != 0) {
+    if (t_lpr > 0 && fgi == n_fg - 1) {
+      hist_bm_body<G, CL, MODE, HAS_VB, POSV, PACK, TLW, IDENT, true>(codes, Fp, ridx, va, vb, wk, lb, fgi, n_fg, fg0,
+                                                               nf, Bs, s0, s1, hist, n_slots, wyy_out, bq, part, dbg,
+                                                               t_lpr, t_ss);
+      return;
+    }
+  }
+  hist_bm_body<G, CL, MODE, HAS_VB, POSV, PACK, LW, IDENT, false>(codes, Fp, ridx, va, vb, wk, lb, fgi, n_fg, fg0, nf,
+                                                           Bs, s0, s1, hist, n_slots, wyy_out, bq, part, dbg, 0, 0);
 }
 
 static int g_bm_dbg = 0;
 extern "C" void h2o_hist_bm_set_debug(int flags) { g_bm_dbg = flags; }
 
-template <int G, int CL, int M, bool V, bool PV, bool PK, int LW>
+static int g_bm_ragged = 0;
+extern "C" void h2o_hist_bm_set_ragged(int mode) { g_bm_ragged = mode; }
+
+struct BmTail { int lw, lpr, ss; };
+static BmTail bm_tail(int F, int foff, int Fp, int G, int CL, int n_fg) {
+  BmTail t{0, 0, 0};
+  const int fg0 = foff + (n_fg - 1) * G, nf = F - fg0;
+  if (g_bm_ragged <= 0 || g_bm_ragged > 4 || G != 64 || CL != 1 || nf >= G) return t;
+  if (g_bm_ragged == 4) return BmTail{3, 0, 0};
+  if (g_bm_ragged == 3) {
+    const int l = (nf + 7) / 8;
+    if (l <= 7 && fg0 + 8 * l <= Fp) return BmTail{2, l, 8};
+  }
+  const int l = (nf + 3) / 4;
+  if (l > 12) return t;
+  return BmTail{1, l, g_bm_ragged == 2 ? l : 16};
+}
+
+template <int G, int CL, int M, bool V, bool PV, bool PK, int LW, int TLW = 0, bool ID = false>
 static int lbm_u(const QuadArgs& a) {
-  auto kern = hist_bm_kernel<G, CL, M, V, PV, PK, LW>;
+  auto kern = hist_bm_kernel<G, CL, M, V, PV, PK, LW, TLW, ID>;
   static bool attr = false;
   if (!attr) {
     hipError_t e = hipFuncSetAttribute((const void*)kern, hipFuncAttributeMaxDynamicSharedMemorySize, 160 * 1024);
@@ -551,14 +604,29 @@
   }
   hipLaunchKernelGGL(kern, a.grid, dim3(a.threads), a.lds, a.s, a.cc, a.Fp, a.ridx, a.va, a.vb, a.wk, a.n_work,
                      a.n_fg, a.F, a.foff, a.Bs, a.s0, a.s1, a.hist, a.n_slots, a.wyy, a.bq, a.need, a.n_work_dev,
-                     a.part, g_bm_dbg);
-  return (int)hipGetLastError();
+                     a.part, g_bm_dbg, a.t_lpr, a.t_ss);
+  return (int)hipGetLastError();
+}
+
+template <int G, int CL, int M, bool V, bool PV, bool PK, bool ID>
+static int lbm_t(const QuadArgs& a) {
+  static const int lw = env_int("H2O3_HIST_BM_LW", 2);
+  if constexpr (G == 64 && CL == 1) {
+    if (a.t_lw == 1) return lbm_u<G, CL, M, V, PV, PK, 2, 1, ID>(a);
+    if (a.t_lw == 2) return lbm_u<G, CL, M, V, PV, PK, 2, 2, ID>(a);
+    if (a.t_lw == 3) return lbm_u<G, CL, M, V, PV, PK, 2, 3, ID>(a);
+  }
+  if constexpr (ID) return lbm_u<G, CL, M, V, PV, PK, 2, 0, true>(a);
+  return (lw == 1 || G == 16) ? lbm_u<G, CL, M, V, PV, PK, 1>(a) : lbm_u<G, CL, M, V, PV, PK, 2>(a);
 }
 
 template <int G, int CL, int M, bool V, bool PV, bool PK>
 static int lbm(const QuadArgs& a) {
-  static const int lw = env_int("H2O3_HIST_BM_LW", 2);
-  return (lw == 1 || G == 16) ? lbm_u<G, CL, M, V, PV, PK, 1>(a) : lbm_u<G, CL, M, V, PV, PK, 2>(a);
+  if (a.ridx == nullptr) {
+    if constexpr (G == 64 && CL == 1 && PV) return lbm_t<G, CL, M, V, PV, PK, true>(a);
+    return (int)hipErrorInvalidValue;
+  }
+  return lbm_t<G, CL, M, V, PV, PK, false>(a);
 }
 
 template <int G, int CL, int M, bool PK>
@@ -584,7 +652,7 @@
     const unsigned long long* __restrict__ part, const int4* __restrict__ work, int n_work,
     const int* __restrict__ n_work_dev, int n_fg, int F, int foff, int G, int CL, int lpr, int nk, int Bs, int C,
     int pack, long long bq, float s0, float s1, const uint8_t* __restrict__ need, double* __restrict__ hist,
-    int n_slots) {
+    int n_slots, int t_lpr, int t_nk, int t_ss) {
   const int nw = n_work_dev != nullptr ? n_work_dev[1] : n_work;
   const int i0 = blockIdx.z * BM_RED;
   if (i0 >= nw) return;
@@ -597,8 +665,11 @@
   const int sl = (blockIdx.x / nbt) * 16 + (threadIdx.x & 15);
   const int ch = sl / G, slot = sl - ch * G;
   const int fg0 = foff + g * G;
-  const int fl = nk * (slot % lpr) + slot / lpr;
-  const bool live = fl < min(G, F - fg0);
+  int ss = lpr;
+  if (t_lpr > 0 && g == n_fg - 1) { lpr = t_lpr; nk = t_nk; ss = t_ss; }
+  const int sq = slot % ss, sk = slot / ss;
+  const int fl = nk * sq + sk;
+  const bool live = sq < lpr && sk < nk && fl < min(G, F - fg0);
   const double inv0 = 1.0 / (double)s0, inv1 = 1.0 / (double)s1;
   const size_t E = (size_t)Bs * PITCH;
   const size_t eoff = (size_t)b * PITCH + sl;
@@ -652,17 +723,21 @@
   a.n_work = n_work; a.n_fg = n_fg; a.fgw = G; a.F = F; a.foff = foff; a.Bs = Bs; a.s0 = s0; a.s1 = s1;
   a.hist = hist; a.n_slots = n_slots; a.wyy = wyy; a.bq = pack_bq; a.need = need; a.n_work_dev = n_work_dev;
   a.part = part;
+  static const int lw_env = env_int("H2O3_HIST_BM_LW", 2);
+  const int lw = (lw_env == 1 || G == 16) ? 1 : 2;
+  const BmTail tail = lw == 2 ? bm_tail(F, foff, Fp, G, CL, n_fg) : BmTail{0, 0, 0};
+  if (ridx == nullptr && !(G == 64 && CL == 1 && posv != 0 && lw == 2)) return -5;
+  a.t_lw = tail.lw; a.t_lpr = tail.lpr; a.t_ss = tail.ss;
   const int rc = G == 64 ? lbm_g<64>(mode, pack, vb != nullptr, posv != 0, a)
                : G == 32 ? lbm_g<32>(mode, pack, vb != nullptr, posv != 0, a)
                          : lbm_g<16>(mode, pack, vb != nullptr, posv != 0, a);
   if (rc != 0 || part == nullptr || (g_bm_dbg & 1)) return rc;
-  static const int lw_env = env_int("H2O3_HIST_BM_LW", 2);
-  const int lw = (lw_env == 1 || G == 16) ? 1 : 2;
   const int nk = 4 * lw, lpr = G / nk;
   const int C = mode == 2 ? 1 : 2;
   dim3 rg(((Bs + 15) / 16) * (G * CL / 16), n_fg, (n_work + BM_RED - 1) / BM_RED);
   hipLaunchKernelGGL(hist_bm_reduce_kernel, rg, dim3(256), 0, s, part, (const int4*)work, n_work, n_work_dev, n_fg,
-                     F, foff, G, CL, lpr, nk, Bs, C, pack ? 1 : 0, pack_bq, s0, s1, need, hist, n_slots);
+                     F, foff, G, CL, lpr, nk, Bs, C, pack ? 1 : 0, pack_bq, s0, s1, need, hist, n_slots,
+                     tail.lpr, 4 * tail.lw, tail.ss);
   return (int)hipGetLastError();
 }
 
@@ -843,7 +918,10 @@
   for (int base = wk.y; base < end; base += 256 * U) {
     int r[U], c[U];
 #pragma unroll
-    for (int u = 0; u < U; ++u) r[u] = ridx[min(base + u * 256 + (int)threadIdx.x, end - 1)];
+    for (int u = 0; u < U; ++u) {
+      const int pc = min(base + u * 256 + (int)threadIdx.x, end - 1);
+      r[u] = ridx != nullptr ? ridx[pc] : pc;
+    }
 #pragma unroll
     for (int u = 0; u < U; ++u) c[u] = (int)codes[(size_t)r[u] * rs + (size_t)f * fs];
 #pragma unroll
@@ -883,7 +961,7 @@
     for (int u = 0; u < U; ++u) {
       const int p = base + u * 256 + (int)threadIdx.x;
       const int pc = min(p, end - 1);
-      r[u] = ridx[pc];
+      r[u] = ridx != nullptr ? ridx[pc] : pc;
       a[u] = pa ? pa[pc] : 0.f;
       const int w0 = base + u * 256 + wv * 64;
       bal[u] = (w0 < end) ? flags[fb + (w0 - wk.y) / 64] : 0ull;
@@ -1931,6 +2009,13 @@
 
 __global__ void dt_root_kernel(double* __restrict__ rec, long long N) {
   if (threadIdx.x == 0) { rec[DT_ST] = 0.0; rec[DT_CT] = (double)N; }
+}
+
+__global__ __launch_bounds__(256) void dt_root_leaf_iota_kernel(const double* __restrict__ rec,
+                                                                int* __restrict__ ridx0, long long n) {
+  if (rec[DT_OK] > 0.0) return;
+  for (long long i = (long long)blockIdx.x * 256 + threadIdx.x; i < n; i += (long long)gridDim.x * 256)
+    ridx0[i] = (int)i;
 }
 
 __global__ __launch_bounds__(256) void leaf_flag_sums_kernel(
@@ -2204,6 +2289,13 @@
   return (int)hipGetLastError();
 }
 
+int h2o_dt_root_leaf_iota(const double* rec, int* ridx0, long long n, hipStream_t s) {
+  if (n <= 0) return 0;
+  const long long blocks = std::min<long long>((n + 255) / 256, 2048);
+  hipLaunchKernelGGL(dt_root_leaf_iota_kernel, dim3((unsigned)blocks), dim3(256), 0, s, rec, ridx0, n);
+  return (int)hipGetLastError();
+}
+
 int h2o_part_flags_dev(const void* codes, int code_bytes, long long rs, long long fs, const int* ridx, const int* work,
                        const int* fbase, int n_cap, const int* feat, const uint8_t* masks, int Bs,
                        unsigned long long* flags, int* cnt, const int* counts, hipStream_t s) {
diff --git a/h2o3_amd/ops/tree_ops.py b/h2o3_amd/ops/tree_ops.py
--- a/h2o3_amd/ops/tree_ops.py
+++ b/h2o3_amd/ops/tree_ops.py
@@ -145,8 +145,18 @@
                                          _c_void, _c_int, _c_void, _c_void, _c_void, _c_void, _c_void, _c_void,
                                          _c_void, _c_void]
         lib.h2o_fill_nid.argtypes = [_c_void, _c_void, _c_int, _c_void, _c_void]
+        lib.h2o_hist_bm_set_ragged.argtypes = [_c_int]
+        lib.h2o_hist_bm_set_ragged.restype = None
         lib._typed = True
     return lib
+
+
+def bm_ragged() -> int:
+    return int(env("H2O3_HIST_BM_RAGGED", "0"))
+
+
+def set_bm_ragged(lib, mode=None):
+    lib.h2o_hist_bm_set_ragged(bm_ragged() if mode is None else int(mode))
 
 
 def channels(mode: int) -> int:
@@ -338,6 +348,7 @@
             need = _need(fgw)
             if bm is not None:
                 part = bm_part(len(items), n_fg, bd.Bs, fgw, pack or mode == 2, dev)
+                set_bm_ragged(lib)
                 rc = lib.h2o_hist_bm(_ptr(bd.codes), bd.Fp, _ptr(ridx), _ptr(va), _ptr(vb), _ptr(work), len(items),
                                      bd.F, 0, bd.Bs, s0, s1, _ptr(hist), n_slots, mode, _ptr(wyy), 1 if posv else 0,
                                      bq, fgw, _ptr(need), None, _ptr(part), _stream())
@@ -809,6 +820,7 @@
         s1, bq = _pack_scale(vmax[1] if vb is None else max(vmax[1], 0.0), chunk)
     if bm is not None:
         part = bm_part(cap, n_fg, bd.Bs, fgw, pack or mode == 2, dev)
+        set_bm_ragged(lib)
         rc = lib.h2o_hist_bm(_ptr(bd.codes), bd.Fp, _ptr(ridx), _ptr(va), _ptr(vb), _ptr(work), cap, bd.F, 0, bd.Bs,
                              s0, s1, _ptr(Hb), n, mode, _ptr(wyy), 1 if posv else 0, bq, fgw, None, _ptr(cnts),
                              _ptr(part), _stream())
```
